# benanil/CLRayTracer

Hardware: AMD Instinct MI355X
Metric: Mrays/s (primary + traced secondary rays), ms/frame at 1920x1080 (higher is better)
Workload: dtype f32

## Files before the change

### clraytracer_amd/_lib.py

```python
import ctypes as C
import os

import numpy as np

os.environ.setdefault("GPU_MAX_HW_QUEUES", "8")

_HERE = os.path.dirname(os.path.abspath(__file__))
ROOT = os.path.dirname(_HERE)
HIP_SO = os.path.join(_HERE, "csrc", "libcrt_hip.so")
HOST_SO = os.path.join(_HERE, "host", "libcrt_host.so")


class CrtTraceArgs(C.Structure):
    _fields_ = [("cameraPos", C.c_float * 3), ("time", C.c_float), ("numMeshes", C.c_uint32), ("sunAngle", C.c_float)]


class CrtFrameStats(C.Structure):
    _fields_ = [("frames", C.c_uint64), ("sumMs", C.c_double * 4), ("extentMs", C.c_double), ("firstFrameMs", C.c_double)]


class CrtCounters(C.Structure):
    _fields_ = [(n, C.c_uint64) for n in ("rays", "primary", "secondary", "hits", "misses", "traversals", "pops",
                                          "innerVisits", "triTests", "capHits", "stackOverflows", "maxStack",
                                          "shadowRays", "shadowHits")]

    def as_dict(self):
        return {n: int(getattr(self, n)) for n, _ in self._fields_}


TRI_DTYPE = np.dtype([("v0", "<f4", 3), ("cx", "<f4"), ("v1", "<f4", 3), ("cy", "<f4"), ("v2", "<f4", 3), ("cz", "<f4"),
                      ("uv", "<u2", 6), ("mat", "<u2"), ("n", "<u2", 9)])
NODE_DTYPE = np.dtype([("min", "<f4", 3), ("leftFirst", "<u4"), ("max", "<f4", 3), ("triCount", "<u4")])
MATERIAL_DTYPE = np.dtype([("color", "<u4"), ("specularColor", "<u4"), ("albedo", "<u2"), ("specular", "<u2"),
                           ("shininess", "<u2"), ("roughness", "<u2")])
TEXTURE_DTYPE = np.dtype([("width", "<i4"), ("height", "<i4"), ("offset", "<i4"), ("padd", "<i4")])
INSTANCE_DTYPE = np.dtype([("inv", "<f4", (4, 4)), ("meshIndex", "<u2"), ("materialStart", "<u2"), ("pad", "u1", 12)])
RAYHIT_DTYPE = np.dtype([("t", "<f4"), ("u", "<f4"), ("v", "<f4"), ("tri", "<u4"), ("instance", "<i4")])
HITRECORD_DTYPE = np.dtype([("normal", "<f4", 3), ("uv", "<f4", 2), ("distance", "<f4"), ("color", "<u4"), ("index", "<u4")])
assert TRI_DTYPE.itemsize == 80 and NODE_DTYPE.itemsize == 32 and MATERIAL_DTYPE.itemsize == 16
assert TEXTURE_DTYPE.itemsize == 16 and INSTANCE_DTYPE.itemsize == 80 and RAYHIT_DTYPE.itemsize == 20
assert HITRECORD_DTYPE.itemsize == 32
CRT_RENDER_GBUFFER = 8192
CRT_GBUFFER_GEOMETRY, CRT_GBUFFER_IDS, CRT_GBUFFER_ALBEDO = 0, 1, 2
GBUFFER_GEOMETRY_DTYPE = np.dtype([("normal", "<f4", 3), ("t", "<f4")])
GBUFFER_IDS_DTYPE = np.dtype([("instance", "<i4"), ("tri", "<u4"), ("u", "<f4"), ("v", "<f4")])
GBUFFER_ALBEDO_DTYPE = np.dtype("<u4")
GBUFFER_PLANE_DTYPES = {"geometry": (CRT_GBUFFER_GEOMETRY, GBUFFER_GEOMETRY_DTYPE), "ids": (CRT_GBUFFER_IDS, GBUFFER_IDS_DTYPE),
                        "albedo": (CRT_GBUFFER_ALBEDO, GBUFFER_ALBEDO_DTYPE)}
GBUFFER_PIXEL_DTYPE = np.dtype([("normal", "<f4", 3), ("t", "<f4"), ("instance", "<i4"), ("tri", "<u4"), ("u", "<f4"), ("v", "<f4"),
                                ("albedo", "<u4")])
assert GBUFFER_GEOMETRY_DTYPE.itemsize == 16 and GBUFFER_IDS_DTYPE.itemsize == 16 and GBUFFER_PIXEL_DTYPE.itemsize == 36

_f = C.c_float
_fp = C.POINTER(C.c_float)
_vp = C.c_void_p
_sz = C.c_size_t

HIP_API = {
    "crt_init": (C.c_int, [C.c_int, C.c_int, C.c_int]),
    "crt_init_devices": (C.c_int, [C.POINTER(C.c_int), C.c_int, C.c_int, C.c_int]),
    "crt_init_gpus": (C.c_int, [C.c_int, C.c_int, C.c_int]),
    "crt_num_devices": (C.c_int, []),
    "crt_peer_access": (C.c_int, [C.c_int]),
    "crt_gather_path": (C.c_char_p, []),
    "crt_get_cull_range": (C.c_int, [_fp, C.c_int, _fp, _fp, C.POINTER(C.c_uint64)]),
    "crt_debug_staggered_frames": (C.c_int, [C.POINTER(C.c_uint64)]),
    "crt_debug_inject_failure": (C.c_int, [C.c_int]),
    "crt_debug_last_kernel": (C.c_int, [C.c_char_p, C.c_size_t]),
    "crt_debug_last_gather": (C.c_int, [C.POINTER(C.c_uint64), C.POINTER(C.c_int)]),
    "crt_debug_build_stats": (C.c_int, [C.POINTER(C.c_uint32), C.POINTER(C.c_uint32)]),
    "crt_debug_tlas_stats": (C.c_int, [C.POINTER(C.c_uint64), C.POINTER(C.c_uint32), C.POINTER(C.c_uint32)]),
    "crt_debug_measure_clock": (C.c_int, [C.c_int, C.POINTER(C.c_double)]),
    "crt_shutdown": (C.c_int, []),
    "crt_resize": (C.c_int, [C.c_int, C.c_int]),
    "crt_set_row_bands": (C.c_int, [C.c_int, C.c_int, C.c_int]),
    "crt_row_owner": (C.c_int, [C.c_int, C.c_int, C.c_int]),
    "crt_band_plan": (C.c_int, [C.c_int, C.c_int, C.c_int, C.c_int, C.POINTER(C.c_int)]),
    "crt_upload_triangles": (C.c_int, [_vp, _sz, _sz]),
    "crt_upload_bvh_nodes": (C.c_int, [_vp, _sz, _sz]),
    "crt_upload_bvh_roots": (C.c_int, [_vp, _sz, _sz]),
    "crt_upload_materials": (C.c_int, [_vp, _sz, _sz]),
    "crt_upload_texture_table": (C.c_int, [_vp, _sz]),
    "crt_upload_texels": (C.c_int, [_vp, _sz, _sz]),
    "crt_upload_instances": (C.c_int, [_vp, _sz, _sz]),
    "crt_build_bvh": (C.c_int, [_sz, _vp, C.c_int, _sz, _sz, C.POINTER(C.c_uint32)]),
    "crt_download_triangles": (C.c_int, [_vp, _sz, _sz]),
    "crt_download_bvh_nodes": (C.c_int, [_vp, _sz, _sz]),
    "crt_download_bvh_roots": (C.c_int, [_vp, _sz, _sz]),
    "crt_render": (C.c_int, [C.POINTER(CrtTraceArgs), _fp, _fp, C.c_int]),
    "crt_sync": (C.c_int, []),
    "crt_query_hits": (C.c_int, [_vp, _vp, C.c_int, C.c_uint32, _vp]),
    "crt_read_output": (C.c_int, [_vp, _sz]),
    "crt_read_output_rows": (C.c_int, [_vp, C.c_int, C.c_int]),
    "crt_read_output_rgba8": (C.c_int, [_vp, _sz]),
    "crt_map_host_frame": (C.c_int, [C.POINTER(C.c_void_p), C.POINTER(C.c_size_t)]),
    "crt_map_host_frame_back": (C.c_int, [C.c_int, C.POINTER(C.c_void_p), C.POINTER(C.c_size_t)]),
    "crt_read_rays": (C.c_int, [_vp, _sz]),
    "crt_output_device_ptr": (_vp, []),
    "crt_read_gbuffer": (C.c_int, [C.c_int, _vp, _sz]),
    "crt_gbuffer_device_ptr": (_vp, [C.c_int]),
    "crt_pick_pixel": (C.c_int, [C.c_int, C.c_int, _vp]),
    "crt_owned_rows": (C.c_int, []),
    "crt_last_kernel_ms": (C.c_float, [C.c_int]),
    "crt_frame_time_stats": (C.c_int, [C.POINTER(CrtFrameStats), C.c_int]),
    "crt_get_counters": (C.c_int, [C.POINTER(CrtCounters)]),
    "crt_get_culled_visits": (C.c_int, [C.POINTER(C.c_uint64)]),
    "crt_debug_read_stamps": (C.c_int, [_vp, _sz, C.POINTER(C.c_size_t)]),
    "crt_debug_read_frame_times": (C.c_int, [_vp, _sz, C.POINTER(C.c_size_t)]),
    "crt_error_string": (C.c_char_p, [C.c_int]),
    "crt_device_name": (C.c_char_p, []),
}

HOST_API = {
    "crth_initialize": (C.c_int, [C.c_int, C.c_int, C.c_int]),
    "crth_initialize_devices": (C.c_int, [C.POINTER(C.c_int), C.c_int, C.c_int, C.c_int]),
    "crth_initialize_host_only": (C.c_int, [C.c_int, C.c_int]),
    "crth_terminate": (None, []),
    "crth_last_error": (C.c_int, []),
    "crth_clear_error": (None, []),
    "crth_prepare_meshes": (None, []),
    "crth_import_texture": (C.c_int, [C.c_char_p]),
    "crth_import_texture_rgb8": (C.c_int, [C.c_char_p, C.c_int, C.c_int, _vp]),
    "crth_import_mesh": (C.c_int, [C.c_char_p]),
    "crth_push_meshes": (None, []),
    "crth_set_device_bvh_build": (None, [C.c_int]),
    "crth_set_mesh_cache": (None, [C.c_int]),
    "crth_qlz_decompress": (C.c_size_t, [_vp, _sz, _vp, _sz]),
    "crth_qlz_store": (C.c_size_t, [_vp, _sz, _vp]),
    "crth_qlz_compress": (C.c_size_t, [_vp, _sz, _vp]),
    "crth_jpeg_decode": (C.c_size_t, [_vp, _sz, _vp, _sz, C.POINTER(C.c_int), C.POINTER(C.c_char_p)]),
    "crth_set_asset_root": (None, [C.c_char_p]),
    "crth_push_textures": (None, []),
    "crth_push_materials": (None, []),
    "crth_create_material": (C.c_int, [C.c_int]),
    "crth_edit_material": (None, [C.c_int, _vp]),
    "crth_begin_instances": (None, []),
    "crth_register_instance": (C.c_uint, [C.c_int, C.c_int, _fp]),
    "crth_end_instances": (None, []),
    "crth_clear_instances": (None, []),
    "crth_set_mesh_matrix": (None, [C.c_uint, _fp]),
    "crth_set_mesh_position": (None, [C.c_uint, _fp]),
    "crth_set_instance_material": (None, [C.c_uint, C.c_int]),
    "crth_set_camera": (None, [_fp, _fp]),
    "crth_get_camera": (None, [_fp, _fp, _fp]),
    "crth_resize": (None, [C.c_int, C.c_int]),
    "crth_set_postprocess": (None, [C.c_int]),
    "crth_set_shadows": (None, [C.c_int]),
    "crth_set_refraction": (None, [C.c_int]),
    "crth_set_fxaa": (None, [C.c_int]),
    "crth_set_supersampling": (None, [C.c_int]),
    "crth_set_gbuffer": (None, [C.c_int]),
    "crth_map_gbuffer": (_vp, [C.c_int]),
    "crth_pick_pixel": (C.c_int, [C.c_int, C.c_int, _vp]),
    "crth_set_unorm8": (None, [C.c_int]),
    "crth_map_output_rgba8": (_vp, []),
    "crth_set_pipelined": (None, [C.c_int]),
    "crth_set_row_bands": (None, [C.c_int, C.c_int, C.c_int]),
    "crth_render": (C.c_uint, [_f]),
    "crth_map_output": (_vp, []),
    "crth_last_frame_ms": (C.c_float, []),
    "crth_cpu_raycast": (None, [_vp, _vp, C.c_int, _vp, C.c_int]),
    "crth_cpu_raycast_sse": (None, [_vp, _vp, C.c_int, _vp, C.c_int]),
    "crth_triangles": (_vp, []), "crth_num_triangles": (_sz, []),
    "crth_nodes": (_vp, []), "crth_num_nodes": (_sz, []),
    "crth_roots": (_vp, []), "crth_num_meshes": (C.c_int, []),
    "crth_materials": (_vp, []), "crth_num_materials": (C.c_int, []),
    "crth_textures": (_vp, []), "crth_num_textures": (C.c_int, []),
    "crth_texels": (_vp, []), "crth_texel_bytes": (_sz, []),
    "crth_instances": (_vp, []), "crth_num_instances": (C.c_uint, []),
    "crth_mesh_info": (None, [C.c_int, _vp]),
    "crth_build_bvh": (C.c_uint32, [_vp, _vp, C.c_int, _vp, _vp]),
    "crth_float_to_half": (C.c_uint16, [_f]),
    "crth_half_to_float": (_f, [C.c_uint16]),
    "crth_inverse_transform": (None, [_fp, _fp]),
    "crth_inverse": (None, [_fp, _fp]),
    "crth_perspective_fov_rh": (None, [_f, _f, _f, _f, _f, _fp]),
    "crth_look_at_rh": (None, [_fp, _fp, _fp, _fp]),
    "crth_write_obj": (C.c_int, [C.c_char_p, _vp, C.c_int, _vp, C.c_int, _vp, C.c_int, _vp, _vp, C.c_int, _vp, C.c_int]),
    "crth_shm_barrier_open": (_vp, [C.c_char_p, C.c_int, C.c_int]),
    "crth_shm_barrier_wait": (C.c_int, [_vp, C.c_int]),
    "crth_shm_barrier_close": (None, [_vp]),
}


def _bind(path, table):
    if not os.path.exists(path):
        raise ImportError(f"{path} has not been built (run `make` at {ROOT} or __graft_entry__.build()); "
                          "the ray-trace path has no fallback without it")
    lib = C.CDLL(path, mode=C.RTLD_GLOBAL)
    for name, (res, args) in table.items():
        fn = getattr(lib, name)
        fn.restype = res
        fn.argtypes = args
    return lib


_hip = None
_host = None


def hip():
    global _hip
    if _hip is None:
        _hip = _bind(HIP_SO, HIP_API)
    return _hip


def host():
    global _host
    if _host is None:
        hip()
        _host = _bind(HOST_SO, HOST_API)
    return _host


CRT_OK, CRT_E_NOT_INITIALIZED, CRT_E_BAD_ARGUMENT, CRT_E_OUT_OF_RANGE, CRT_E_NO_DEVICE, CRT_E_UNSUPPORTED = 0, -1, -2, -3, -4, -5


class CrtError(RuntimeError):
    pass


def check(rc, what="crt call"):
    if rc != 0:
        msg = hip().crt_error_string(rc)
        raise CrtError(f"{what} failed with {rc}: {msg.decode() if msg else '?'}")


def fptr(a):
    a = np.ascontiguousarray(a, dtype=np.float32)
    return a.ctypes.data_as(_fp), a


def as_array(ptr, count, dtype):
    if not ptr or count == 0:
        return np.zeros(0, dtype=dtype)
    nbytes = int(count) * np.dtype(dtype).itemsize
    buf = (C.c_char * nbytes).from_address(ptr)
    return np.frombuffer(buf, dtype=dtype, count=int(count)).copy()
```

### clraytracer_amd/csrc/crt_device.h

```cpp
#pragma once
#include <hip/hip_runtime.h>
#include <hip/hip_fp16.h>
#include <stdint.h>
#include <type_traits>
#include "../../include/crt_types.h"

#define CRT_LEAF_BIT 0x80000000u
#define CRT_TOP_BIT 0x40000000u
#define CRT_BLOCK 64
#ifndef CRT_WAVES_PER_SIMD
#define CRT_WAVES_PER_SIMD 8
#endif
#define CRT_WAVES_PER_SIMD_COUNT 6
typedef uint32_t __attribute__((address_space(3))) * crt_lds_u32_ptr;
typedef float crt_f32x4 __attribute__((ext_vector_type(4)));
typedef const crt_f32x4 __attribute__((address_space(4)))* crt_const_f32x4_ptr;
typedef const crt_f32x4 __attribute__((address_space(3)))* crt_lds_f32x4_ptr;
#ifndef CRT_LDS_SLOTS
#define CRT_LDS_SLOTS 20
#endif
#define CRT_MAX_PARK 5
#define CRT_OVF_SLOTS_MAX (CRT_STACK_DEPTH - (CRT_LDS_SLOTS - CRT_MAX_PARK))
#define CRT_OVF_WORDS_PER_BLOCK ((size_t)CRT_OVF_SLOTS_MAX * CRT_BLOCK)
template <int PARK, int SLOTS = CRT_LDS_SLOTS, bool TOP = false>
struct CrtStackT {
    static constexpr bool kTop = TOP;
    static constexpr int kLds = SLOTS - PARK;
    static_assert(PARK >= 0 && PARK <= CRT_MAX_PARK && kLds >= 1 && kLds <= CRT_STACK_DEPTH && CRT_STACK_DEPTH - kLds <= CRT_OVF_SLOTS_MAX, "LDS slots");
    crt_lds_u32_ptr lds;
    uint32_t* ovf;
    crt_lds_f32x4_ptr top;
    uint32_t vblock;
    __device__ __forceinline__ uint32_t* overflow_slot(int k) const
    {
        uint32_t lane = threadIdx.x & 63;
        asm volatile("" : "+v"(lane));
        return ovf + ((size_t)(TOP ? vblock : blockIdx.x) * CRT_OVF_SLOTS_MAX + (size_t)k) * CRT_BLOCK + lane;
    }
    __device__ __forceinline__ void write(int slot, uint32_t v) const
    {
        const int s = slot & (CRT_STACK_DEPTH - 1);
        if (kLds >= CRT_STACK_DEPTH || __ballot(s >= kLds) == 0) { lds[s * 64] = v; return; }
        if (kLds >= CRT_STACK_DEPTH || s < kLds) lds[s * 64] = v;
        else *overflow_slot(s - kLds) = v;
    }
    __device__ __forceinline__ uint32_t read(int slot) const
    {
        const int s = slot & (CRT_STACK_DEPTH - 1);
        if (kLds >= CRT_STACK_DEPTH || __ballot(s >= kLds) == 0) return lds[s * 64];
        if (kLds >= CRT_STACK_DEPTH || s < kLds) return lds[s * 64];
        return *overflow_slot(s - kLds);
    }
    __device__ __forceinline__ crt_lds_f32x4_ptr top_record(uint32_t k) const { return top + k * 4; }
    __device__ __forceinline__ void park(int k, uint32_t v) const { lds[(kLds + k) * 64] = v; }
    __device__ __forceinline__ uint32_t parked(int k) const { return lds[(kLds + k) * 64]; }
};
typedef CrtStackT<0> CrtStack;
#ifndef CRT_SPLIT_BETA
#define CRT_SPLIT_BETA 1.2f
#endif
#ifndef CRT_SPLIT_BETA_ASYNC
#define CRT_SPLIT_BETA_ASYNC 2.0f
#endif
#define CRT_MAX_SPLIT 96
#ifndef CRT_MAX_SPLIT_PIPELINED
#define CRT_MAX_SPLIT_PIPELINED 8
#endif
#define CRT_TILE 8

struct CrtTlasNode { float4 sphere; uint32_t left, right, pad0, pad1; };
#define CRT_TLAS_LEAF 0x80000000u
#define CRT_TLAS_MIN_INSTANCES 64
#define CRT_TLAS_LIST 8

struct CrtDevScene {
    const float4* __restrict__ pairs;
    const float* __restrict__ triHot;
    const uint4* __restrict__ triCold;
    const uint32_t* __restrict__ bigLeaf;
    const uint32_t* __restrict__ rootRefs;
    uint32_t* stackOverflow;
    const CrtMeshInstance* __restrict__ instances;
    const struct CrtDevInstance* __restrict__ devInstances;
    const float4* __restrict__ instBounds;
    const CrtMaterial* __restrict__ materials;
    const CrtTexture* __restrict__ textures;
    const uint32_t* __restrict__ texels;
    int numTexels;
    uint32_t numInstances;
    const CrtTlasNode* __restrict__ tlas;
    uint32_t tlasNodes;
    const uint32_t* __restrict__ alwaysList;
    uint32_t numAlways;
    const float4* __restrict__ topPairs;
};

struct CrtFrame {
    float invView[16];
    float invProj[16];
    float camPos[3];
    float lightY, lightZ;
    int width, height;
    int tilesX;
    int ownedTileRows;
    int gridBlocks;
    int tileRowsPerBand;
    int rank, nRanks;
    int slotsPerXcd;
    const uint32_t* order;
    const uint32_t* listLen;
    int listCap;
    uint32_t* cost;
    uint32_t epilogue;
    int ss;
    uint32_t* packOut;
};

struct CrtGBuffer {
    char* __restrict__ planes;
    __host__ __device__ char* geometry() const { return planes; }
    __host__ __device__ char* ids(size_t pixels) const { return planes + 16 * pixels; }
    __host__ __device__ char* albedo(size_t pixels) const { return planes + 32 * pixels; }
};

struct v3 { float x, y, z; };

__device__ __forceinline__ v3 mk3(float x, float y, float z) { v3 r; r.x = x; r.y = y; r.z = z; return r; }
__device__ __forceinline__ v3 add3(v3 a, v3 b) { return mk3(a.x + b.x, a.y + b.y, a.z + b.z); }
__device__ __forceinline__ v3 sub3(v3 a, v3 b) { return mk3(a.x - b.x, a.y - b.y, a.z - b.z); }
__device__ __forceinline__ v3 mul3(v3 a, v3 b) { return mk3(a.x * b.x, a.y * b.y, a.z * b.z); }
__device__ __forceinline__ v3 scale3(v3 a, float s) { return mk3(a.x * s, a.y * s, a.z * s); }
__device__ __forceinline__ v3 neg3(v3 a) { return mk3(-a.x, -a.y, -a.z); }
__device__ __forceinline__ float dot3(v3 a, v3 b) { return (a.x * b.x + a.y * b.y) + a.z * b.z; }
__device__ __forceinline__ v3 cross3(v3 a, v3 b)
{
    return mk3(a.y * b.z - a.z * b.y, a.z * b.x - a.x * b.z, a.x * b.y - a.y * b.x);
}
__device__ __forceinline__ v3 normalize3(v3 v)
{
    float inv = 1.0f / sqrtf(dot3(v, v));
    return scale3(v, inv);
}
__device__ __forceinline__ v3 reflect3(v3 v, v3 n)
{
    float d = dot3(n, v);
    return sub3(v, scale3(scale3(n, d), 2.0f));
}
__device__ __forceinline__ int f2i(float x)
{
    if (!(x == x)) return 0;
    if (x >= 2147483648.0f) return 2147483647;
    if (x <= -2147483648.0f) return (-2147483647 - 1);
    return (int)x;
}
__device__ __forceinline__ float h2f(uint32_t bits16) { return __half2float(__ushort_as_half((unsigned short)bits16)); }

struct CrtDevInstance;
struct Triout { float t, u, v; uint32_t tri; };

struct LaneCounters {
    uint32_t rays, primary, secondary, hits, misses;
    uint32_t traversals, pops, innerVisits, triTests, capHits, stackOverflows, maxStack;
    uint32_t shadowRays, shadowHits;
    uint32_t culled;
};
__device__ __forceinline__ void count_culled(LaneCounters& lc, uint32_t n) { lc.traversals += n; lc.pops += n; lc.innerVisits += n; lc.culled += n; }

__device__ __forceinline__ float intersect_aabb(v3 o, v3 inv, float4 bmin, float4 bmax, float minSoFar)
{
// ... 61 lines not shown
__device__ __forceinline__ v3 xform_xyz(const CrtDevInstance& m, float vx, float vy, float vz, float vw)
{
    v3 r;
    r.x = ((m.r0.x * vx + m.r1.x * vy) + m.r2.x * vz) + m.r3.x * vw;
    r.y = ((m.r0.y * vx + m.r1.y * vy) + m.r2.y * vz) + m.r3.y * vw;
    r.z = ((m.r0.z * vx + m.r1.z * vy) + m.r2.z * vz) + m.r3.z * vw;
    return r;
}

__device__ __forceinline__ v3 mat3mul(const CrtDevInstance& m, v3 v)
{
    v3 r;
    r.x = (m.r0.x * v.x + m.r1.x * v.y) + m.r2.x * v.z;
    r.y = (m.r0.y * v.x + m.r1.y * v.y) + m.r2.y * v.z;
    r.z = (m.r0.z * v.x + m.r1.z * v.y) + m.r2.z * v.z;
    return r;
}

__device__ __forceinline__ CrtDevInstance load_instance(const CrtDevInstance* __restrict__ table, uint32_t inst)
{
    CrtDevInstance I;
    const uint32_t inst0 = (uint32_t)__builtin_amdgcn_readfirstlane((int)inst);
    if (__ballot(inst != inst0) == 0) {
        const crt_const_f32x4_ptr p = (crt_const_f32x4_ptr)(table + inst0);
        const crt_f32x4 a = p[0], b = p[1], c = p[2], e = p[3];
        I.r0 = make_float4(a.x, a.y, a.z, a.w); I.r1 = make_float4(b.x, b.y, b.z, b.w);
        I.r2 = make_float4(c.x, c.y, c.z, c.w); I.r3 = make_float4(e.x, e.y, e.z, e.w);
    } else {
        const CrtDevInstance* ip = table + inst;
        I.r0 = ip->r0; I.r1 = ip->r1; I.r2 = ip->r2; I.r3 = ip->r3;
    }
    return I;
}

template <bool COUNT>
struct Traversal {
    v3 mo, md, inv;
    Triout tr;
    int sp, prot, inters;
    uint32_t ref, curInst;
    bool active;

    __device__ __forceinline__ void reset()
    {
        mo = mk3(0.f, 0.f, 0.f); md = mo; inv = mo;
        tr.t = 0.f; tr.u = 0.f; tr.v = 0.f; tr.tri = 0;
        sp = 0; prot = 0; inters = 0; ref = 0; curInst = 0; active = false;
    }
    __device__ __forceinline__ bool at_inner() const { return active && !(ref & CRT_LEAF_BIT); }
    __device__ __forceinline__ bool at_leaf() const { return active && (ref & CRT_LEAF_BIT); }

    __device__ __forceinline__ void finish(Closest& c)
    {
        if (inters) { c.hitInstance = (int)curInst; c.hit = tr; c.distance = tr.t; c.anyHit = 1; }
        active = false;
    }
    template <class STK>
    __device__ __forceinline__ void pop_next(const STK& stack, Closest& c, LaneCounters& lc)
    {
        const bool nonEmpty = sp > 0, canPop = nonEmpty && prot < CRT_MAX_POPS;
        prot += nonEmpty ? 1 : 0;
        if (COUNT) { if (nonEmpty && !canPop) lc.capHits++; if (canPop) lc.pops++; }
        if (canPop) { --sp; ref = stack.read(sp); }
        else {
            const bool keep = inters != 0;
            c.hitInstance = keep ? (int)curInst : c.hitInstance; c.distance = keep ? tr.t : c.distance; c.anyHit = keep ? 1 : c.anyHit;
            c.hit.t = keep ? tr.t : c.hit.t; c.hit.u = keep ? tr.u : c.hit.u; c.hit.v = keep ? tr.v : c.hit.v; c.hit.tri = keep ? tr.tri : c.hit.tri;
            active = false;
        }
    }
    template <bool TOP = false>
    __device__ __forceinline__ void enter(const CrtDevScene& S, uint32_t inst, v3 o, v3 d, float bestSoFar, LaneCounters& lc)
    {
        curInst = inst;
        const CrtDevInstance I = load_instance(S.devInstances, inst);
        mo = xform_xyz(I, o.x, o.y, o.z, 1.0f);
        md = xform_xyz(I, d.x, d.y, d.z, 0.0f);
        inv = mk3(1.0f / md.x, 1.0f / md.y, 1.0f / md.z);
        tr.t = bestSoFar; tr.tri = 0; tr.u = 0.0f; tr.v = 0.0f;
        ref = __float_as_uint(TOP ? I.r2.w : I.r0.w);
        sp = 0; prot = 1; inters = 0; active = true;
        if (COUNT) { lc.traversals++; lc.pops++; }
    }
    template <class STK>
    __device__ __forceinline__ void inner(const CrtDevScene& S, const STK& stack, Closest& c, LaneCounters& lc)
    {
        float dist1, dist2;
        uint32_t nearRef, farRef;
        const uint32_t ref0 = (uint32_t)__builtin_amdgcn_readfirstlane((int)ref);
        if (__ballot(ref != ref0) == 0) {
            const crt_const_f32x4_ptr q = (STK::kTop && (ref0 & CRT_TOP_BIT)) ? (crt_const_f32x4_ptr)(S.topPairs + (size_t)(ref0 & 0xFFFFu) * 4)
                                                                             : (crt_const_f32x4_ptr)(S.pairs + (size_t)ref0 * 4);
            const crt_f32x4 a = q[0], b = q[1], c4 = q[2], e = q[3];
            dist1 = intersect_aabb(mo, inv, make_float4(a.x, a.y, a.z, a.w), make_float4(b.x, b.y, b.z, b.w), tr.t);
            dist2 = intersect_aabb(mo, inv, make_float4(c4.x, c4.y, c4.z, c4.w), make_float4(e.x, e.y, e.z, e.w), tr.t);
            nearRef = __float_as_uint(a.w); farRef = __float_as_uint(c4.w);
#ifndef CRT_TOP_NO_LDS_PATH
#define CRT_TOP_NO_LDS_PATH 0
#endif
        } else if (STK::kTop && !CRT_TOP_NO_LDS_PATH && __ballot(!(ref & CRT_TOP_BIT)) == 0) {
            const auto q = stack.top_record(ref & 0xFFFFu);
            const crt_f32x4 a = q[0], b = q[1], c4 = q[2], e = q[3];
            dist1 = intersect_aabb(mo, inv, make_float4(a.x, a.y, a.z, a.w), make_float4(b.x, b.y, b.z, b.w), tr.t);
            dist2 = intersect_aabb(mo, inv, make_float4(c4.x, c4.y, c4.z, c4.w), make_float4(e.x, e.y, e.z, e.w), tr.t);
            nearRef = __float_as_uint(a.w); farRef = __float_as_uint(c4.w);
        } else {
            const float4* p = (STK::kTop && (ref & CRT_TOP_BIT)) ? S.topPairs + (size_t)(ref & 0xFFFFu) * 4 : S.pairs + (size_t)ref * 4;
            const float4 lmin = p[0], lmax = p[1], rmin = p[2], rmax = p[3];
            dist1 = intersect_aabb(mo, inv, lmin, lmax, tr.t);
            dist2 = intersect_aabb(mo, inv, rmin, rmax, tr.t);
            nearRef = __float_as_uint(lmin.w); farRef = __float_as_uint(rmin.w);
        }
        if (COUNT) lc.innerVisits++;
        {
            const bool sw = dist1 > dist2;
            const float d1 = sw ? dist2 : dist1, d2 = sw ? dist1 : dist2;
            const uint32_t r1 = sw ? farRef : nearRef, r2 = sw ? nearRef : farRef;
            dist1 = d1; dist2 = d2; nearRef = r1; farRef = r2;
        }
        if (dist2 != 1e30f) {
            if (COUNT) { if (sp >= CRT_STACK_DEPTH) lc.stackOverflows++; }
            stack.write(sp, farRef);
            sp++;
            if (COUNT) { if ((uint32_t)sp > lc.maxStack) lc.maxStack = (uint32_t)sp; }
        }
        if (dist1 == 1e30f) pop_next(stack, c, lc);
        else ref = nearRef;
    }
    template <bool ANYHIT, class STK>
    __device__ __forceinline__ void leaf(const CrtDevScene& S, const STK& stack, Closest& c, LaneCounters& lc)
    {
        const uint32_t first = ref & 0x00FFFFFFu;
        uint32_t n = (ref >> 24) & 0x7Fu;
        if (n == 0) n = S.bigLeaf[first];
        for (uint32_t i = first, end = first + n; i < end; ++i) {
            if (COUNT) lc.triTests++;
            const float* __restrict__ hot = S.triHot + (size_t)i * 9;
            inters |= intersect_triangle(mo, md, mk3(hot[0], hot[1], hot[2]), mk3(hot[3], hot[4], hot[5]), mk3(hot[6], hot[7], hot[8]), tr, i);
            if (ANYHIT) { if (inters) break; }
        }
        if (ANYHIT && inters) finish(c);
        else pop_next(stack, c, lc);
    }
};

__device__ __forceinline__ bool sphere_culls(const float4 bs, v3 o, v3 d, float dd)
{
    const v3 oc = mk3(bs.x - o.x, bs.y - o.y, bs.z - o.z);
    const float oc2 = dot3(oc, oc), b = dot3(oc, d);
    const float r2 = bs.w * bs.w * 1.0201f + 4e-6f * oc2;
    return (bs.w >= 0.0f) & ((oc2 * dd - b * b > r2 * dd) | ((b < 0.0f) & (oc2 > r2)));
}

template <bool COUNT, bool DEFER_COUNT = false>
__device__ __forceinline__ unsigned long long candidate_mask(const CrtDevScene& S, v3 o, v3 d, uint32_t base, uint32_t cnt, LaneCounters& lc)
{
    const float dd = dot3(d, d);
    unsigned long long cand = 0;
    const crt_const_f32x4_ptr bounds = (crt_const_f32x4_ptr)S.instBounds;
    for (uint32_t k = 0; k < cnt; ++k) {
        const crt_f32x4 bs = bounds[base + k];
        const v3 oc = mk3(bs.x - o.x, bs.y - o.y, bs.z - o.z);
        const float oc2 = dot3(oc, oc), b = dot3(oc, d);
        const float r2 = bs.w * bs.w * 1.0201f + 4e-6f * oc2;
        const bool cull = (bs.w >= 0.0f) && ((oc2 * dd - b * b > r2 * dd) || (b < 0.0f && oc2 > r2));
        if (!cull) cand |= 1ull << k;
    }
    if (COUNT && !DEFER_COUNT) { const uint32_t culled = cnt - (uint32_t)__popcll(cand); count_culled(lc, culled); }
    return cand;
}

#define CRT_TLAS_PARK (CRT_TLAS_LIST / 2)
template <class STK>
__device__ __forceinline__ bool candidate_list_add(const STK& stack, uint32_t& n, uint32_t idx)
{
    if (n >= (uint32_t)CRT_TLAS_LIST) return false;
    const uint32_t sh = (n & 1u) * 16u, m = ~(0xFFFFu << sh), v = idx << sh;
    const int k = (int)(n >> 1);
    stack.park(k, (stack.parked(k) & m) | v);
    n++;
    return true;
}
template <class STK>
__device__ __forceinline__ uint32_t candidate_list_next(const STK& stack, int after)
{
    uint32_t best = 0xFFFFu;
#pragma unroll
    for (int k = 0; k < CRT_TLAS_PARK; ++k) {
        const uint32_t w = stack.parked(k);
        const uint32_t lo = w & 0xFFFFu, hi = w >> 16;
        if ((int)lo > after && lo < best) best = lo;
        if ((int)hi > after && hi < best) best = hi;
    }
    return best;
}
template <class STK>
__device__ __forceinline__ bool tlas_candidates(const CrtDevScene& S, v3 o, v3 d, const STK& stack, uint32_t& n)
{
#pragma unroll
    for (int k = 0; k < CRT_TLAS_PARK; ++k) stack.park(k, 0xFFFFFFFFu);
    n = 0;
    bool ok = true;
    for (uint32_t k = 0; k < S.numAlways; ++k) { const uint32_t i = S.alwaysList[k]; if (i < S.numInstances) ok = candidate_list_add(stack, n, i) && ok; }
    if (S.tlasNodes == 0) return ok;
    const float dd = dot3(d, d);
    uint32_t node = 0; int sp = 0;
    for (;;) {
        const CrtTlasNode nd = S.tlas[node];
        bool descend = false;
        if (!sphere_culls(nd.sphere, o, d, dd)) {
            if (nd.left & CRT_TLAS_LEAF) {
                const uint32_t i = nd.left & 0xFFFFu;
                if (i < S.numInstances) ok = candidate_list_add(stack, n, i) && ok;
            } else { stack.write(sp, nd.right); sp++; node = nd.left; descend = true; }
        }
        if (!descend) { if (sp == 0) break; --sp; node = stack.read(sp); }
    }
    return ok;
}

template <bool COUNT, bool ITERS, bool ANYHIT, class STK>
__device__ __forceinline__ void trip_steps(const CrtDevScene& S, const STK& stack, Traversal<COUNT>& T, Closest& c, LaneCounters& lc, bool done)
{
    if (!done && T.at_inner()) {
        if (ITERS) { lc.rays++; if (first_active_lane()) lc.innerVisits++; }
        T.inner(S, stack, c, lc);
    }
    if (!done && T.at_leaf()) {
        if (ITERS) {
            if (first_active_lane()) lc.triTests++;
            uint32_t n = (T.ref >> 24) & 0x7Fu; if (n == 0) n = S.bigLeaf[T.ref & 0x00FFFFFFu];
            for (int off = 32; off > 0; off >>= 1) { const uint32_t o2 = (uint32_t)__shfl_xor((int)n, off, 64); n = o2 > n ? o2 : n; }
            if (first_active_lane()) lc.misses += n;
        }
        T.template leaf<ANYHIT>(S, stack, c, lc);
    }
    if (!done && T.at_inner()) {
        if (ITERS) { if (first_active_lane()) lc.hits++; }
        T.inner(S, stack, c, lc);
    }
}

template <bool COUNT, bool ITERS = false, bool ANYHIT = false, bool TLAS = false, class STK = CrtStack>
__device__ __forceinline__ Closest closest_hit(const CrtDevScene& S, v3 o, v3 d, const STK& stack, LaneCounters& lc)
{
    Closest c = no_hit();
    Traversal<COUNT> T; T.reset();

    if constexpr (TLAS) {
        static_assert(!TLAS || STK::kLds <= CRT_LDS_SLOTS - CRT_TLAS_PARK, "the candidate list needs CRT_TLAS_PARK parked slots");
        uint32_t listed = 0;
        const bool fits = tlas_candidates(S, o, d, stack, listed);
        if (__ballot(!fits) == 0) {
            int prev = -1;
            if (COUNT && !ANYHIT) { const uint32_t culled = S.numInstances - listed; count_culled(lc, culled); }
            bool done = false;
            for (;;) {
                const bool wEnter = !done && !T.active;
                const bool wInner = !done && T.at_inner();
                const bool wLeaf = !done && T.at_leaf();
                if (__ballot(wEnter || wInner || wLeaf) == 0) break;
                if (wEnter) {
                    const uint32_t k = (ANYHIT && c.anyHit) ? 0xFFFFu : candidate_list_next(stack, prev);
                    if (k == 0xFFFFu) {
                        done = true;
                        if (COUNT && ANYHIT && !c.anyHit) { const uint32_t n = S.numInstances - (uint32_t)(prev + 1); count_culled(lc, n); }
                    } else {
                        if (COUNT && ANYHIT) { const uint32_t n = k - (uint32_t)(prev + 1); count_culled(lc, n); }
                        prev = (int)k;
                        T.template enter<STK::kTop>(S, k, o, d, c.distance, lc);
                    }
                }
                trip_steps<COUNT, false, ANYHIT>(S, stack, T, c, lc, done);
            }
            return c;
        }
    }

    for (uint32_t base = 0; base < S.numInstances; base += 64) {
        const uint32_t cnt = (S.numInstances - base) < 64u ? (S.numInstances - base) : 64u;
        unsigned long long cand = candidate_mask<COUNT, ANYHIT>(S, o, d, base, cnt, lc);
        unsigned long long culledLeft = (COUNT && ANYHIT) ? (~cand & (cnt == 64u ? ~0ull : ((1ull << cnt) - 1ull))) : 0ull;
        bool done = ANYHIT && c.anyHit;
        for (;;) {
            const bool wEnter = !done && !T.active;
            const bool wInner = !done && T.at_inner();
            const bool wLeaf = !done && T.at_leaf();
            if (__ballot(wEnter || wInner || wLeaf) == 0) break;
            if (ITERS) { if (first_active_lane()) lc.pops++; }
            if (wEnter) {
                if (ANYHIT && c.anyHit) done = true;
                else if (cand == 0) {
                    done = true;
                    if (COUNT && ANYHIT) { const uint32_t n = (uint32_t)__popcll(culledLeft); count_culled(lc, n); culledLeft = 0; }
                } else {
                    if (ITERS) { if (first_active_lane()) lc.traversals++; }
                    const uint32_t k = (uint32_t)__ffsll((long long)cand) - 1u;
                    cand &= cand - 1;
                    if (COUNT && ANYHIT) {
                        const unsigned long long below = culledLeft & ((1ull << k) - 1ull);
                        const uint32_t n = (uint32_t)__popcll(below);
                        count_culled(lc, n); culledLeft &= ~below;
                    }
                    T.template enter<STK::kTop>(S, base + k, o, d, c.distance, lc);
                }
            }
            trip_steps<COUNT, ITERS, ANYHIT>(S, stack, T, c, lc, done);
        }
    }
    return c;
}

__device__ __forceinline__ int clamp_texel(int idx, int n) { return idx < 0 ? 0 : (idx >= n ? n - 1 : idx); }

__device__ __noinline__ int sample_skybox(v3 d, int texW, int texH)
{
    const double PI = 3.14159265358979323846;
    float at = (float)(atan2((double)d.x, (double)(-d.z)) / PI);
    float ac = (float)(acos((double)d.y) / PI);
    int theta = f2i((at * 0.5f) * (float)texW);
    int phi = f2i(ac * (float)texH);
    return (int)((uint32_t)phi * (uint32_t)texW + (uint32_t)(theta + 2));
}

__device__ __forceinline__ int sample_texture(const CrtTexture& tex, float u, float v)
{
    u = u - floorf(u);
    v = v - floorf(v);
    int uS = f2i((float)tex.width * u);
    int vS = f2i((float)tex.height * v);
    return (int)((uint32_t)vS * (uint32_t)tex.width + (uint32_t)tex.offset + (uint32_t)uS);
}

__device__ __forceinline__ v3 raygen_dir(const CrtFrame& F, int i, int j, int width, int height)
{
    float cx = (float)i / (float)width, cy = (float)j / (float)height;
    cx = cx * 2.0f - 1.0f;
    cy = cy * 2.0f - 1.0f;
    v3 t = matmul_xyz(F.invProj, cx, cy, 1.0f, 1.0f);
    float w = matmul_w(F.invProj, cx, cy, 1.0f, 1.0f);
    float tx = t.x / w, ty = t.y / w, tz = t.z / w, tw = w / w;
    v3 wv = matmul_xyz(F.invView, tx, ty, tz, tw);
    return normalize3(wv);
}

__device__ __forceinline__ v3 raygen_dir(const CrtFrame& F, int i, int j) { return raygen_dir(F, i, j, F.width, F.height); }

struct PathState { v3 o, d, result; float energy; };
__device__ __forceinline__ PathState camera_path(const CrtFrame& F, v3 d)
{
    PathState ps;
    ps.o = mk3(F.camPos[0], F.camPos[1], F.camPos[2]);
    ps.d = d;
    ps.result = mk3(0.0f, 0.0f, 0.0f);
    ps.energy = 1.0f;
    return ps;
}

__device__ __forceinline__ float specular_x(float ndl, float shadow)
{
    const float sp = ((1.0f - 0.5f) * ndl) * shadow;
    return (sp * 0.2f) * ndl;
}

struct NoSink { };
template <bool DEFER_ENERGY = false, bool REFRACT = false, class SINK = NoSink>
__device__ __forceinline__ int shade_bounce(const CrtDevScene& S, const Closest& c, PathState& ps, int bounce, float lightY, float lightZ,
                                            float* ndlOut = nullptr, const SINK* sink = nullptr)
{
    constexpr bool kSink = !std::is_same<SINK, NoSink>::value;
    const float UcharToFloat01 = 1.0f / 255.0f;
    if (c.distance > 99998.0f) {
        if constexpr (kSink) { if (bounce == 0) sink->miss(c); }
        const crt_f32x4 skyHdr = ((crt_const_f32x4_ptr)S.textures)[2];
        int idx = clamp_texel(sample_skybox(ps.d, __float_as_int(skyHdr.x), __float_as_int(skyHdr.y)), S.numTexels);
        uint32_t px = S.texels[idx];
        v3 skyc = scale3(mk3((float)(px & 0xffu), (float)((px >> 8) & 0xffu), (float)((px >> 16) & 0xffu)), UcharToFloat01);
        ps.result = add3(ps.result, scale3(skyc, ps.energy));
        return 0;
    }
    const v3 light = bounce == 0 ? mk3(0.0f, lightY, lightZ) : ps.d;
    const v3 atm0 = scale3(mk3(0.255f, 0.25f, 0.27f), 1.0f);
    const v3 atm = bounce == 0 ? atm0 : scale3(atm0, 0.4f);
    const CrtDevInstance I = load_instance(S.devInstances, (uint32_t)c.hitInstance);
    const v3 mo = xform_xyz(I, ps.o.x, ps.o.y, ps.o.z, 1.0f);
    const v3 md = xform_xyz(I, ps.d.x, ps.d.y, ps.d.z, 0.0f);

    const uint4 c0 = S.triCold[(size_t)c.hit.tri * 2], c1 = S.triCold[(size_t)c.hit.tri * 2 + 1];
    const uint32_t matIndex = c0.w & 0xffffu;
    uint32_t mi = __float_as_uint(I.r1.w) + matIndex;
    mi = mi < (uint32_t)CRT_MAX_MATERIALS ? mi : (uint32_t)CRT_MAX_MATERIALS - 1;
    const CrtMaterial mat = S.materials[mi];
    const float bx = (1.0f - c.hit.u) - c.hit.v, by = c.hit.u, bz = c.hit.v;

    const v3 n0 = mat3mul(I, mk3(h2f(c0.w >> 16), h2f(c1.x & 0xffffu), h2f(c1.x >> 16)));
    const v3 n1 = mat3mul(I, mk3(h2f(c1.y & 0xffffu), h2f(c1.y >> 16), h2f(c1.z & 0xffffu)));
    const v3 n2 = mat3mul(I, mk3(h2f(c1.z >> 16), h2f(c1.w & 0xffffu), h2f(c1.w >> 16)));
    const v3 normal = normalize3(add3(add3(scale3(n0, bx), scale3(n1, by)), scale3(n2, bz)));

    const float uvx = (h2f(c0.x & 0xffffu) * bx + h2f(c0.y & 0xffffu) * by) + h2f(c0.z & 0xffffu) * bz;
    const float uvy = (h2f(c0.x >> 16) * bx + h2f(c0.y >> 16) * by) + h2f(c0.z >> 16) * bz;

    uint32_t ti = mat.albedoTextureIndex;
    ti = ti < (uint32_t)CRT_MAX_TEXTURES ? ti : (uint32_t)CRT_MAX_TEXTURES - 1;
    const CrtTexture tex = S.textures[ti];
    const uint32_t px = S.texels[clamp_texel(sample_texture(tex, uvx, uvy), S.numTexels)];
    const uint32_t a = mat.color;
    const uint32_t cr = (((a & 0xffu) * (px & 0xffu)) >> 8) & 0xffu;
    const uint32_t cg = ((((a >> 8) & 0xffu) * ((px >> 8) & 0xffu)) >> 8) & 0xffu;
    const uint32_t cb = ((((a >> 16) & 0xffu) * ((px >> 16) & 0xffu)) >> 8) & 0xffu;
    const v3 color = scale3(mk3((float)cr, (float)cg, (float)cb), UcharToFloat01);
    if constexpr (kSink) { if (bounce == 0) sink->hit(c, normal, 0xFF000000u | (cb << 16) | (cg << 8) | cr); }
    const v3 point = add3(mo, scale3(md, c.hit.t));


    bool transmitted = false;
    float opacity = 1.0f;
    if (REFRACT) {
        if (bounce == 0) {
            opacity = h2f(mat.roughness);
            if (opacity < 1.0f) {
                const float dn = dot3(normal, ps.d);
                const bool entering = dn < 0.0f;
                const v3 nf = entering ? normal : neg3(normal);
                const float cosi = entering ? (0.0f - dn) : dn;
                const float eta = entering ? 0.6666667f : 1.5f;
                const float k = 1.0f - (eta * eta) * (1.0f - cosi * cosi);
                if (k >= 0.0f) {
                    const float w = eta * cosi - sqrtf(k);
                    const v3 refr = add3(scale3(ps.d, eta), scale3(nf, w));
                    ps.o = sub3(point, scale3(nf, 0.01f));
                    ps.d = refr;
                    transmitted = true;
                }
            }
        }
    }
    if (!transmitted) {
        ps.o = add3(point, scale3(normal, 0.01f));
        ps.d = reflect3(ps.d, normal);
    }

    float ndl = dot3(normal, neg3(light));
    const v3 ambient = mul3(scale3(atm, fmaxf(0.0f - ndl, 0.1f)), color);
    ndl = fmaxf(ndl, 0.0f);
    const float sl = (ndl * fmaxf(dot3(reflect3(neg3(light), normal), md), 0.0f)) * 0.2f;

    ps.result = add3(ps.result, add3(add3(scale3(scale3(color, ndl), ps.energy), ambient), mk3(sl, sl, sl)));
    if (REFRACT && transmitted) { ps.energy = ps.energy * (1.0f - opacity); return 2; }
    if (DEFER_ENERGY) *ndlOut = ndl;
    else ps.energy = ps.energy * specular_x(ndl, 1.0f);
    return 1;
}
```

### clraytracer_amd/csrc/crt_frame.h

```cpp
#pragma once
namespace {

static void unpack_counters(const unsigned long long c[CRT_NUM_COUNTERS])
{
    CrtCounters& o = g.lastCounters;
    o.rays = c[0]; o.primary = c[1]; o.secondary = c[2]; o.hits = c[3]; o.misses = c[4]; o.traversals = c[5];
    o.pops = c[6]; o.innerVisits = c[7]; o.triTests = c[8]; o.capHits = c[9]; o.stackOverflows = c[10]; o.maxStack = c[11];
    o.shadowRays = c[12]; o.shadowHits = c[13]; g.lastCulled = c[14];
}

int collect_set(EventSet& es)
{
    if (!es.pending) return CRT_OK;
    hipEvent_t* ev = es.ev;
    hipEvent_t traceStart = es.evRaygen ? ev[1] : ev[0], frameEnd = es.evPost ? ev[3] : ev[2];
    HIPCHK(hipEventSynchronize(frameEnd));
    float ms[4] = { 0, 0, 0, 0 };
    HIPCHK(hipEventElapsedTime(&ms[0], ev[0], frameEnd));
    if (es.evRaygen) HIPCHK(hipEventElapsedTime(&ms[1], ev[0], ev[1]));
    HIPCHK(hipEventElapsedTime(&ms[2], traceStart, ev[2]));
    if (es.evPost) HIPCHK(hipEventElapsedTime(&ms[3], ev[2], ev[3]));
    for (int k = 0; k < 4; ++k) g.msSum[k] += (double)ms[k];
    g.framesTimed++;
    if (g.statStartValid && es.seq >= g.statStartSeq) {
// ... 352 lines not shown

static int launch_passes(FrameCtx& c)
{
    FrameSlot& fs = *c.fs; EventSet& es = *c.es; CrtFrame& F = c.F;
    const bool unorm = (c.flags & CRT_RENDER_UNORM8) != 0, post = (c.flags & CRT_RENDER_POSTPROCESS) != 0, fxaa = (c.flags & CRT_RENDER_FXAA) != 0;
    const bool fxaaLocal = fxaa && g.groupSize <= 1;
    const size_t framePixels = (size_t)g.width * (size_t)g.height;
    if (fxaa && !is_secondary()) RCCHK(grow(fs.aux, fs.auxPixels, framePixels, fs.stream));
    if (c.flags & CRT_RENDER_GBUFFER) RCCHK(grow(fs.gbuf, fs.gbufBytes, framePixels * CRT_GBUFFER_PIXEL_BYTES, fs.stream));
    if (!fxaa) F.epilogue = (unorm ? CRT_EPILOGUE_QUANTIZE : 0u) | (post ? CRT_EPILOGUE_POST : 0u);
    else if (fxaaLocal) F.epilogue = unorm ? CRT_EPILOGUE_QUANTIZE : 0u;
    c.gather8 = frame_gathers_rgba8(c.flags);
    c.packInKernel = unorm && (((c.flags & CRT_RENDER_READBACK) && g.groupSize <= 1) || c.gather8);
    if (c.packInKernel) RCCHK(grow(fs.packBuf, fs.packCap, framePixels, fs.stream));
    if (c.packInKernel && !fxaa) F.packOut = fs.packBuf;
    c.T.epilogue = F.epilogue; c.T.packOut = F.packOut;
    RCCHK(launch_trace(c, fxaaLocal ? fs.aux : fs.out));
    if (is_primary() && !es.evPost) RCCHK(wait_for_parts(c));
    HIPCHK(hipEventRecord(es.ev[2], fs.stream));
    if (!es.evPost) return CRT_OK;
    if (!fxaa) {
        if (!c.fused) {
            if (unorm) crt_quantize_kernel<<<c.grid, CRT_BLOCK, 0, fs.stream>>>(F, fs.out);
            if (post) crt_postprocess_kernel<<<c.grid, CRT_BLOCK, 0, fs.stream>>>(F, fs.out);
            if (unorm && post) crt_quantize_kernel<<<c.grid, CRT_BLOCK, 0, fs.stream>>>(F, fs.out);
            if (c.gather8) crt_pack_owned_kernel<<<(unsigned)F.gridBlocks, CRT_BLOCK, 0, fs.stream>>>(plain_frame(F, false), fs.out, fs.packBuf);
            HIPCHK(hipGetLastError());
        }
        if (is_primary()) RCCHK(wait_for_parts(c));
    } else if (!is_secondary()) {
        if (is_primary()) RCCHK(wait_for_parts(c));
        CrtFrame FF = plain_frame(F, true);
        const unsigned gridAll = (unsigned)FF.gridBlocks;
        if (fxaaLocal) {
            if (unorm && !c.fused) crt_quantize_kernel<<<gridAll, CRT_BLOCK, 0, fs.stream>>>(FF, fs.aux);
        } else {
            if (unorm) crt_quantize_kernel<<<gridAll, CRT_BLOCK, 0, fs.stream>>>(FF, fs.out);
            HIPCHK(hipMemcpyAsync(fs.aux, fs.out, framePixels * sizeof(float4), hipMemcpyDeviceToDevice, fs.stream));
        }
        FF.epilogue = (unorm ? CRT_EPILOGUE_QUANTIZE : 0u) | (post ? CRT_EPILOGUE_POST : 0u);
        FF.packOut = c.packInKernel ? fs.packBuf : nullptr;
        crt_fxaa_kernel<<<gridAll, CRT_BLOCK, 0, fs.stream>>>(FF, fs.aux, fs.out);
        HIPCHK(hipGetLastError());
    }
    HIPCHK(hipEventRecord(es.ev[3], fs.stream));
    return CRT_OK;
}

static int gather_to_primary(const FrameCtx& c)
{
    FrameSlot& fs = *c.fs; FrameSlot& pfs = g.primary->slot[c.slot];
    HIPCHK(hipStreamWaitEvent(fs.stream, pfs.slotDone, 0));
    if (c.gather8) RCCHK(copy_owned_rows_async(pfs.packBuf, fs.packBuf, 4, hipMemcpyDeviceToDevice, fs.stream));
    else RCCHK(copy_owned_rows_async(pfs.out, fs.out, 16, hipMemcpyDeviceToDevice, fs.stream));
    HIPCHK(hipEventRecord(fs.partDone, fs.stream));
    return CRT_OK;
}

static int finish_frame(const FrameCtx& c)
{
    FrameSlot& fs = *c.fs; EventSet& es = *c.es;
    fs.frameIs8 = c.gather8;
    g.cur = c.slot;
    if (c.flags & CRT_RENDER_GBUFFER) g.gbufSlot = c.slot;
    es.pending = true; es.flags = c.flags; es.seq = ++g.frameSeq; fs.frames++;
    if (c.T.order != nullptr && !(c.flags & CRT_RENDER_DIAG_MIX3)) {
        float view[35];
        memcpy(view, c.F.invView, 64); memcpy(view + 16, c.F.invProj, 64); memcpy(view + 32, c.F.camPos, 12);
        g.viewMoved = memcmp(view, g.lastView, sizeof view) != 0 || g.lastViewInst != g.instVersion;
        memcpy(g.lastView, view, sizeof view); g.lastViewInst = g.instVersion;
        RCCHK(sort_for_next_frame(c.T, fs, c.pipelined, g.form != Form::Mega));
    }
    if (c.flags & CRT_RENDER_READBACK) {
        const size_t pixels = (size_t)g.width * (size_t)g.height;
        const bool bytes8 = (c.flags & CRT_RENDER_UNORM8) != 0;
        const size_t bytes = pixels * (bytes8 ? 4 : 16);
        if (bytes > fs.hostCap) {
            if (fs.hostBuf) (void)hipHostFree(fs.hostBuf);
            fs.hostBuf = nullptr; fs.hostCap = 0;
            HIPCHK(hipHostMalloc(&fs.hostBuf, bytes, hipHostMallocDefault));
            fs.hostCap = bytes;
        }
        if (!fs.copied) HIPCHK(hipEventCreateWithFlags(&fs.copied, hipEventDisableTiming));
        const void* src = fs.out;
        if (bytes8) {
            RCCHK(grow(fs.packBuf, fs.packCap, pixels, fs.stream));
            const bool packed = (c.packInKernel && ((c.flags & CRT_RENDER_FXAA) || c.fused)) || c.gather8;
            if (!packed) crt_pack_unorm8_kernel<<<(unsigned)((pixels + 255) / 256), 256, 0, fs.stream>>>(fs.out, fs.packBuf, pixels);
            HIPCHK(hipGetLastError());
            src = fs.packBuf;
        }
        RCCHK(copy_owned_rows_async(fs.hostBuf, src, bytes8 ? 4 : 16, hipMemcpyDeviceToHost, fs.stream, is_primary()));
        HIPCHK(hipEventRecord(fs.copied, fs.stream));
        fs.hostBytes = bytes; g.readbackRing[g.readbackCount++ % CRT_MAX_FRAMES_IN_FLIGHT] = c.slot;
    }
    if (is_primary()) HIPCHK(hipEventRecord(fs.slotDone, fs.stream));
    if (!(c.flags & CRT_RENDER_ASYNC) && !(c.plan && c.plan->noHostWait)) HIPCHK(hipEventSynchronize(es.evPost ? es.ev[3] : es.ev[2]));
    return CRT_OK;
}

int crt1_render(const CrtTraceArgs* args, const float invView[16], const float invProj[16], int flags, const RenderPlan* plan = nullptr)
{
    if (!g.initialized) return CRT_E_NOT_INITIALIZED;
    if (!args || !invView || !invProj) return CRT_E_BAD_ARGUMENT;
    if (args->numMeshes > CRT_MAX_INSTANCES) return CRT_E_OUT_OF_RANGE;
    if (!g.sceneValid) return CRT_E_BAD_ARGUMENT;
    if ((flags & CRT_RENDER_SSAA2) && (flags & CRT_RENDER_SSAA4)) return CRT_E_BAD_ARGUMENT;
    FrameCtx c;
    c.flags = flags; c.plan = plan;
    fill_frame(c.F, args, invView, invProj, ssaa_factor(flags));
    if (c.F.gridBlocks == 0) return record_empty_share(plan);
    RCCHK(refuse_unsupported(flags, args->numMeshes));
    RCCHK(choose_slot(c));
    RCCHK(prepare_lists(c));
    RCCHK(begin_frame(c, args));
    RCCHK(launch_passes(c));
    if (is_secondary()) RCCHK(gather_to_primary(c));
    return finish_frame(c);
}

__global__ void crt_clock_probe_kernel(unsigned long long ticks, double* __restrict__ out)
{
    const unsigned long long r0 = __builtin_amdgcn_s_memrealtime(), c0 = __builtin_amdgcn_s_memtime();
    unsigned long long r1 = r0, guard = 0;
    while (r1 - r0 < ticks && guard < (1ull << 24)) { __builtin_amdgcn_s_sleep(8); r1 = __builtin_amdgcn_s_memrealtime(); ++guard; }
    const unsigned long long c1 = __builtin_amdgcn_s_memtime();
    r1 = __builtin_amdgcn_s_memrealtime();
    if (threadIdx.x == 0) out[blockIdx.x] = r1 > r0 ? (double)(c1 - c0) / (double)(r1 - r0) * 0.1 : 0.0;
}

int crt1_debug_measure_clock(int micros, double* ghz)
{
    if (!g.initialized) return CRT_E_NOT_INITIALIZED;
    if (!ghz || micros < 1 || micros > 100000) return CRT_E_BAD_ARGUMENT;
    double* d = nullptr; hipStream_t st = nullptr;
    HIPCHK(hipMalloc(&d, 8 * sizeof(double)));
    hipError_t e = hipStreamCreateWithFlags(&st, hipStreamNonBlocking);
    double h[8] = { 0 };
    if (e == hipSuccess) {
        crt_clock_probe_kernel<<<8, 64, 0, st>>>((unsigned long long)micros * 100ull, d);
        e = hipGetLastError();
        if (e == hipSuccess) e = hipMemcpyAsync(h, d, sizeof h, hipMemcpyDeviceToHost, st);
        if (e == hipSuccess) e = hipStreamSynchronize(st);
    }
    if (st) (void)hipStreamDestroy(st);
    (void)hipFree(d);
    if (e != hipSuccess) return (int)e;
    double sum = 0; int n = 0;
    for (double v : h) if (v > 0.0) { sum += v; ++n; }
    *ghz = n ? sum / n : 0.0;
    return CRT_OK;
}

int crt1_sync(void)
{
    if (!g.initialized) return CRT_E_NOT_INITIALIZED;
    return sync_all();
}

int crt1_query_hits(const float* origins, const float* dirs, int n, uint32_t numInstances, CrtRayHit* out)
{
    if (!g.initialized) return CRT_E_NOT_INITIALIZED;
    if (n <= 0) return CRT_OK;
    if (!origins || !dirs || !out || numInstances > CRT_MAX_INSTANCES) return CRT_E_BAD_ARGUMENT;
    if (!g.sceneValid) return CRT_E_BAD_ARGUMENT;
    RCCHK(collect_timing());
    RCCHK(quiesce());
    const size_t rayBytes = sizeof(float) * 3 * (size_t)n, need = rayBytes * 2 + sizeof(CrtRayHit) * (size_t)n;
    RCCHK(grow(g.queryBuf, g.queryBytes, need, g.stream));
    float* dO = reinterpret_cast<float*>(g.queryBuf);
    float* dD = dO + 3 * (size_t)n;
    CrtRayHit* dH = reinterpret_cast<CrtRayHit*>(dD + 3 * (size_t)n);
    HIPCHK(hipMemcpyAsync(dO, origins, rayBytes, hipMemcpyHostToDevice, g.stream));
    HIPCHK(hipMemcpyAsync(dD, dirs, rayBytes, hipMemcpyHostToDevice, g.stream));
    HIPCHK(hipMemsetAsync(g.counters, 0, CRT_NUM_COUNTERS * sizeof(unsigned long long), g.stream));
    FrameSlot& fs = g.slot[0];
    RCCHK(ensure_slot_instances(fs));
    RCCHK(ensure_overflow(fs, (size_t)((n + CRT_BLOCK - 1) / CRT_BLOCK)));
    double farthest2 = 0.0;
    for (int k = 0; k < n; ++k) {
        const double x = origins[3 * k], y = origins[3 * k + 1], z = origins[3 * k + 2], d2 = x * x + y * y + z * z;
        if (!(d2 <= farthest2)) farthest2 = d2;
    }
    CrtDevScene S; fill_scene(S, numInstances, fs, beyond_cull_range(sqrt(farthest2)));
    with_bools([&](auto Tl) { crt_query_kernel<decltype(Tl)::value><<<(unsigned)((n + CRT_BLOCK - 1) / CRT_BLOCK), CRT_BLOCK, 0, g.stream>>>(S, dO, dD, n, dH, g.counters); }, use_tlas(S));
    HIPCHK(hipGetLastError());
    HIPCHK(hipMemcpyAsync(out, dH, sizeof(CrtRayHit) * (size_t)n, hipMemcpyDeviceToHost, g.stream));
    unsigned long long c[CRT_NUM_COUNTERS];
    HIPCHK(hipMemcpyAsync(c, g.counters, sizeof c, hipMemcpyDeviceToHost, g.stream));
    HIPCHK(hipStreamSynchronize(g.stream));
    unpack_counters(c);
    return CRT_OK;
}

int crt1_read_output(float* dst, size_t floats)
{
    if (!g.initialized) return CRT_E_NOT_INITIALIZED;
    if (!dst || floats != (size_t)g.width * (size_t)g.height * 4) return CRT_E_BAD_ARGUMENT;
    RCCHK(sync_all());
    RCCHK(expand_rgba8_frame(g.slot[g.cur]));
    HIPCHK(hipMemcpy(dst, g.slot[g.cur].out, floats * sizeof(float), hipMemcpyDeviceToHost));
    return CRT_OK;
}

int crt1_read_output_rows(float* dst, int row0, int rows)
{
    if (!g.initialized) return CRT_E_NOT_INITIALIZED;
    if (!dst || row0 < 0 || rows < 0 || row0 + rows > g.height) return CRT_E_BAD_ARGUMENT;
    RCCHK(sync_all());
    RCCHK(expand_rgba8_frame(g.slot[g.cur]));
    HIPCHK(hipMemcpy(dst, g.slot[g.cur].out + (size_t)row0 * (size_t)g.width, (size_t)rows * (size_t)g.width * sizeof(float4), hipMemcpyDeviceToHost));
    return CRT_OK;
}

int crt1_read_output_rgba8(uint8_t* dst, size_t bytes)
{
    if (!g.initialized) return CRT_E_NOT_INITIALIZED;
    const size_t pixels = (size_t)g.width * (size_t)g.height;
    if (!dst || bytes != pixels * 4) return CRT_E_BAD_ARGUMENT;
    RCCHK(sync_all());
    if (g.slot[g.cur].frameIs8) {
        HIPCHK(hipMemcpy(dst, g.slot[g.cur].packBuf, pixels * 4, hipMemcpyDeviceToHost));
        return CRT_OK;
    }
    RCCHK(grow(g.queryBuf, g.queryBytes, pixels * 4, g.stream));
    crt_pack_unorm8_kernel<<<(unsigned)((pixels + 255) / 256), 256, 0, g.stream>>>(g.slot[g.cur].out, reinterpret_cast<uint32_t*>(g.queryBuf), pixels);
    HIPCHK(hipGetLastError());
    HIPCHK(hipMemcpyAsync(dst, g.queryBuf, pixels * 4, hipMemcpyDeviceToHost, g.stream));
    HIPCHK(hipStreamSynchronize(g.stream));
    return CRT_OK;
}

int crt1_map_host_frame_back(int framesBack, const void** ptr, size_t* bytes)
{
    if (!g.initialized) return CRT_E_NOT_INITIALIZED;
    if (!ptr || framesBack < 0 || (unsigned)framesBack >= g.readbackCount || framesBack >= g.nSlots) return CRT_E_BAD_ARGUMENT;
    const int slot = g.readbackRing[(g.readbackCount - 1u - (unsigned)framesBack) % CRT_MAX_FRAMES_IN_FLIGHT];
    for (int k = 0; k < framesBack; ++k)
        if (g.readbackRing[(g.readbackCount - 1u - (unsigned)k) % CRT_MAX_FRAMES_IN_FLIGHT] == slot) return CRT_E_BAD_ARGUMENT;
    FrameSlot& fs = g.slot[slot];
    HIPCHK(hipEventSynchronize(fs.copied));
    *ptr = fs.hostBuf;
    if (bytes) *bytes = fs.hostBytes;
    return CRT_OK;
}

int crt1_map_host_frame(const void** ptr, size_t* bytes) { return crt1_map_host_frame_back(0, ptr, bytes); }

int crt1_read_rays(float* dst, size_t floats)
{
    if (!g.initialized) return CRT_E_NOT_INITIALIZED;
    if (!dst || floats != (size_t)g.width * (size_t)g.height * 3) return CRT_E_BAD_ARGUMENT;
    RCCHK(sync_all());
    HIPCHK(hipMemcpy(dst, g.rays, floats * sizeof(float), hipMemcpyDeviceToHost));
    return CRT_OK;
}

static char* gbuffer_plane(int plane)
{
    if (g.gbufSlot < 0 || !g.slot[g.gbufSlot].gbuf || gbuffer_plane_pixel_bytes(plane) == 0) return nullptr;
    const CrtGBuffer gb = slot_gbuffer(g.slot[g.gbufSlot]);
    const size_t pixels = (size_t)g.width * (size_t)g.height;
    return plane == CRT_GBUFFER_GEOMETRY ? gb.geometry() : plane == CRT_GBUFFER_IDS ? gb.ids(pixels) : gb.albedo(pixels);
}

int crt1_read_gbuffer(int plane, void* dst, size_t bytes)
{
    if (!g.initialized) return CRT_E_NOT_INITIALIZED;
    const char* src = gbuffer_plane(plane);
    if (!dst || !src || bytes != (size_t)g.width * (size_t)g.height * gbuffer_plane_pixel_bytes(plane)) return CRT_E_BAD_ARGUMENT;
    RCCHK(sync_all());
    HIPCHK(hipMemcpy(dst, src, bytes, hipMemcpyDeviceToHost));
    return CRT_OK;
}

void* crt1_gbuffer_device_ptr(int plane) { return g.initialized ? (void*)gbuffer_plane(plane) : nullptr; }

int crt1_pick_pixel(int x, int y, CrtGBufferPixel* out)
{
    if (!g.initialized) return CRT_E_NOT_INITIALIZED;
    if (!out || !gbuffer_plane(CRT_GBUFFER_GEOMETRY)) return CRT_E_BAD_ARGUMENT;
    if (x < 0 || y < 0 || x >= g.width || y >= g.height) return CRT_E_OUT_OF_RANGE;
    RCCHK(sync_all());
    const size_t idx = (size_t)y * (size_t)g.width + (size_t)x;
    HIPCHK(hipMemcpy(out->normal, gbuffer_plane(CRT_GBUFFER_GEOMETRY) + idx * 16, 16, hipMemcpyDeviceToHost));
    HIPCHK(hipMemcpy(&out->instance, gbuffer_plane(CRT_GBUFFER_IDS) + idx * 16, 16, hipMemcpyDeviceToHost));
    HIPCHK(hipMemcpy(&out->albedo, gbuffer_plane(CRT_GBUFFER_ALBEDO) + idx * 4, 4, hipMemcpyDeviceToHost));
    return CRT_OK;
}

void* crt1_output_device_ptr(void)
{
    if (!g.initialized) return nullptr;
    if (g.slot[g.cur].frameIs8 && (sync_all() != CRT_OK || expand_rgba8_frame(g.slot[g.cur]) != CRT_OK)) return nullptr;
    return (void*)g.slot[g.cur].out;
}

float crt1_last_kernel_ms(int which)
{
    if (!g.initialized || which < 0 || which > 3) return -1.0f;
    if (collect_timing() != CRT_OK) return -1.0f;
    return g.ms[which];
}

int crt1_frame_time_stats(CrtFrameStats* out, int reset)
{
    if (!g.initialized) return CRT_E_NOT_INITIALIZED;
    RCCHK(collect_timing());
    if (out) {
        out->frames = g.framesTimed;
        for (int k = 0; k < 4; ++k) out->sumMs[k] = g.msSum[k];
        out->extentMs = g.statExtent;
        out->firstFrameMs = g.statFirstMs;
    }
    if (reset) {
        for (int k = 0; k < 4; ++k) g.msSum[k] = 0.0;
        g.framesTimed = 0; g.statExtent = 0; g.statFirstMs = 0; g.statStartArmed = true; g.statStartValid = false;
    }
    return CRT_OK;
}

int crt1_debug_read_frame_times(double* dst, size_t maxFrames, size_t* numFrames)
{
    if (!g.initialized) return CRT_E_NOT_INITIALIZED;
    if (!numFrames) return CRT_E_BAD_ARGUMENT;
    RCCHK(collect_timing());
    *numFrames = g.frameLogN;
    if (dst) memcpy(dst, g.frameLog, sizeof(double) * 2 * (maxFrames < g.frameLogN ? maxFrames : g.frameLogN));
    return CRT_OK;
}

int crt1_debug_read_stamps(uint64_t* dst, size_t maxWaves, size_t* numWaves)
{
    if (!g.initialized) return CRT_E_NOT_INITIALIZED;
    if (!numWaves) return CRT_E_BAD_ARGUMENT;
    *numWaves = g.stampWaves;
    if (!dst || !g.stamps) return CRT_OK;
    const size_t n = maxWaves < g.stampWaves ? maxWaves : g.stampWaves;
    RCCHK(sync_all());
    HIPCHK(hipMemcpy(dst, g.stamps + 16, n * 8 * sizeof(unsigned long long), hipMemcpyDeviceToHost));
    return CRT_OK;
}

int crt1_get_culled_visits(uint64_t* out)
{
    if (!g.initialized) return CRT_E_NOT_INITIALIZED;
    if (!out) return CRT_E_BAD_ARGUMENT;
    RCCHK(collect_timing());
    *out = g.lastCulled;
    return CRT_OK;
}

int crt1_get_cull_range(float* limits, int n, float* sceneLimit, float* bounceReach, uint64_t* noCullFrames)
{
    if (!g.initialized) return CRT_E_NOT_INITIALIZED;
    if (n < 0 || n > CRT_MAX_INSTANCES || (n > 0 && !limits)) return CRT_E_BAD_ARGUMENT;
    for (int i = 0; i < n; ++i) limits[i] = g.hCullOriginLimit[i];
    if (sceneLimit) *sceneLimit = g.cullOriginLimit;
    if (bounceReach) *bounceReach = g.bounceOriginReach;
    if (noCullFrames) *noCullFrames = g.noCullFrames;
    return CRT_OK;
}

int crt1_get_counters(CrtCounters* out)
{
    if (!g.initialized) return CRT_E_NOT_INITIALIZED;
    if (!out) return CRT_E_BAD_ARGUMENT;
    RCCHK(collect_timing());
    *out = g.lastCounters;
    return CRT_OK;
}

}
```

### clraytracer_amd/csrc/crt_instances.h

```cpp
#pragma once
namespace {

bool invert4(const double m[16], double out[16])
{
    double a[4][8];
    for (int r = 0; r < 4; ++r) for (int c = 0; c < 4; ++c) { a[r][c] = m[r * 4 + c]; a[r][4 + c] = (r == c) ? 1.0 : 0.0; }
    for (int col = 0; col < 4; ++col) {
        int piv = col;
        for (int r = col + 1; r < 4; ++r) if (fabs(a[r][col]) > fabs(a[piv][col])) piv = r;
        if (!(fabs(a[piv][col]) > 1e-300)) return false;
        if (piv != col) for (int c = 0; c < 8; ++c) { double t = a[col][c]; a[col][c] = a[piv][c]; a[piv][c] = t; }
        const double inv = 1.0 / a[col][col];
        for (int c = 0; c < 8; ++c) a[col][c] *= inv;
        for (int r = 0; r < 4; ++r) if (r != col) { const double f = a[r][col]; if (f != 0.0) for (int c = 0; c < 8; ++c) a[r][c] -= f * a[col][c]; }
    }
    for (int r = 0; r < 4; ++r) for (int c = 0; c < 4; ++c) out[r * 4 + c] = a[r][4 + c];
    return true;
}

int cache_root_nodes()
{
    for (uint32_t m = 0; m < CRT_MAX_MESHES; ++m) {
        g.hHaveRoot[m] = m < g.numRoots && g.hRoots[m] < g.nodeCount;
        if (g.hHaveRoot[m]) HIPCHK(hipMemcpyAsync(&g.hRootNodes[m], g.rawNodes + g.hRoots[m], sizeof(CrtBVHNode), hipMemcpyDeviceToHost, g.stream));
// ... 79 lines not shown
    for (int a = 0; a < 3; ++a) { lo[a] = c[a] - b.w; hi[a] = c[a] + b.w; }
}

double debug_cull_range_scale()
{
    const char* h = getenv("CRT_DEBUG_HOOKS"); const char* k = getenv("CRT_DEBUG_CULL_RANGE_SCALE");
    return (h && atoi(h) != 0 && k && atof(k) > 0.0) ? atof(k) : 1.0;
}


void update_bounce_reach()
{
    g.hReach = 0.0;
    auto widen = [](double far) { if (far > g.hReach || !(far == far)) g.hReach = far; };
    for (uint32_t m = 0; m < CRT_MAX_MESHES; ++m) {
        if (!g.hHaveRoot[m]) continue;
        widen(box_reach(g.hRootNodes[m]));
        if (g.hHaveKids[m]) { widen(box_reach(g.hRootKids[m][0])); widen(box_reach(g.hRootKids[m][1])); }
    }
    widen(reach_of(g.triReach2));
    g.bounceOriginReach = g.hReach < 3.0e38 ? (float)g.hReach : 3.0e38f;
}

void recompute_cull_records(uint32_t first, uint32_t count)
{
    const uint32_t end = first + count < (uint32_t)CRT_MAX_INSTANCES ? first + count : (uint32_t)CRT_MAX_INSTANCES;
    const double rangeScale = debug_cull_range_scale();
    for (uint32_t i = first; i < end; ++i) {
        g.hBounds[i] = make_float4(0.f, 0.f, 0.f, -1.0f);
        g.hCullOriginLimit[i] = 0.0f;
        if (i >= g.instHigh) continue;
        const CrtMeshInstance& inst = g.hInstances[i];
        if (inst.meshIndex >= CRT_MAX_MESHES || !g.hHaveRoot[inst.meshIndex] || g.hRootNodes[inst.meshIndex].triCount > 0 || !g.hHaveKids[inst.meshIndex]) continue;
        double inv[16], fwd[16], lo[3], hi[3], cw[3];
        if (!forward_transform(inst, inv, fwd)) continue;
        const CrtBVHNode* kid = g.hRootKids[inst.meshIndex];
        for (int a = 0; a < 3; ++a) { lo[a] = fmin((double)kid[0].aabbMin[a], (double)kid[1].aabbMin[a]); hi[a] = fmax((double)kid[0].aabbMax[a], (double)kid[1].aabbMax[a]); }
        const double r = image_sphere(lo, hi, fwd, cw);
        const float4 b = fp32_sphere(cw, r, 1.0 + 1e-4);
        if (!(isfinite(b.x) && isfinite(b.y) && isfinite(b.z) && isfinite(b.w)) || !(b.w < 1e18f) || !(b.w > 1e-18f)) continue;
        const double limit = cull_origin_limit(inv, fwd, b.w) * rangeScale;
        if (!(limit >= g.hReach)) continue;
        g.hCullOriginLimit[i] = (float)fmin(limit * (1.0 - 1e-6), 3e38);
        g.hBounds[i] = b;
    }
}

void recompute_scene_limit()
{
    float lo = (float)fmin(1e30 * (1.0 - 1e-6), 3e38);
    for (uint32_t i = 0; i < g.instHigh; ++i) if (g.hBounds[i].w >= 0.0f && g.hCullOriginLimit[i] < lo) lo = g.hCullOriginLimit[i];
    g.cullOriginLimit = lo;
}

bool tlas_refit()
{
    bool sameSet = g.hTlasBuilt && g.hTlasBuiltHigh == g.instHigh && g.hTlasRefits < 256u;
    for (uint32_t k = 0; sameSet && k < g.instHigh; ++k) sameSet = g.hTlasMember[k] == (uint8_t)(g.hBounds[k].w >= 0.0f);
    if (!sameSet) return false;
    if (g.hTlasNodes == 0) return true;
    double blo[2 * CRT_MAX_INSTANCES][3], bhi[2 * CRT_MAX_INSTANCES][3], sumR = 0.0;
    for (uint32_t n = g.hTlasNodes; n-- > 0;) {
        CrtTlasNode& nd = g.hTlas[n];
        if (nd.left & CRT_TLAS_LEAF) {
            nd.sphere = g.hBounds[nd.left & 0xFFFFu];
            sphere_box(blo[n], bhi[n], nd.sphere);
        } else {
            for (int a = 0; a < 3; ++a) { blo[n][a] = fmin(blo[nd.left][a], blo[nd.right][a]); bhi[n][a] = fmax(bhi[nd.left][a], bhi[nd.right][a]); }
            nd.sphere = node_sphere(blo[n], bhi[n]);
            sumR += (double)nd.sphere.w;
        }
    }
    if (!(sumR <= 1.25 * g.hTlasBuiltRadii)) return false;
    g.hTlasRefits++;
    return true;
}

void tlas_build()
{
    uint32_t nAlways = 0, nLeaves = 0, nNodes = 0, leaves[CRT_MAX_INSTANCES];
    for (uint32_t k = 0; k < g.instHigh; ++k) { const bool cullable = g.hBounds[k].w >= 0.0f; g.hTlasMember[k] = (uint8_t)cullable; if (!cullable) g.hAlways[nAlways++] = k; else leaves[nLeaves++] = k; }
    struct Range { uint32_t lo, hi, node; };
    double sumR = 0.0;
    Range stack[64]; int sp = 0;
    if (nLeaves) stack[sp++] = Range{ 0, nLeaves, nNodes++ };
    while (sp) {
        const Range r = stack[--sp];
        double lo[3] = { 1e300, 1e300, 1e300 }, hi[3] = { -1e300, -1e300, -1e300 }, clo[3] = { 1e300, 1e300, 1e300 }, chi[3] = { -1e300, -1e300, -1e300 };
        for (uint32_t k = r.lo; k < r.hi; ++k) {
            const float4 b = g.hBounds[leaves[k]]; const double c[3] = { b.x, b.y, b.z };
            double slo[3], shi[3];
            sphere_box(slo, shi, b);
            for (int a = 0; a < 3; ++a) {
                if (slo[a] < lo[a]) lo[a] = slo[a];
                if (shi[a] > hi[a]) hi[a] = shi[a];
                if (c[a] < clo[a]) clo[a] = c[a];
                if (c[a] > chi[a]) chi[a] = c[a];
            }
        }
        CrtTlasNode& n = g.hTlas[r.node];
        n.pad0 = n.pad1 = 0;
        if (r.hi - r.lo == 1) { n.sphere = g.hBounds[leaves[r.lo]]; n.left = CRT_TLAS_LEAF | leaves[r.lo]; n.right = 0; continue; }
        n.sphere = node_sphere(lo, hi);
        sumR += (double)n.sphere.w;
        int axis = 0;
        if (chi[1] - clo[1] > chi[axis] - clo[axis]) axis = 1;
        if (chi[2] - clo[2] > chi[axis] - clo[axis]) axis = 2;
        const uint32_t mid = (r.lo + r.hi) / 2;
        auto key = [&](uint32_t idx) { const float4 b = g.hBounds[idx]; return axis == 0 ? b.x : (axis == 1 ? b.y : b.z); };
        std::nth_element(leaves + r.lo, leaves + mid, leaves + r.hi, [&](uint32_t p, uint32_t q) { return key(p) < key(q) || (key(p) == key(q) && p < q); });
        n.left = nNodes++; n.right = nNodes++;
        stack[sp++] = Range{ mid, r.hi, n.right };
        stack[sp++] = Range{ r.lo, mid, n.left };
    }
    g.hTlasNodes = nNodes; g.hNumAlways = nAlways;
    g.hTlasBuilt = true; g.hTlasBuiltHigh = g.instHigh; g.hTlasBuiltRadii = sumR; g.hTlasRefits = 0; g.hTlasBuilds++;
}

void rebuild_instance_master(uint32_t dirtyFirst = 0, uint32_t dirtyCount = CRT_MAX_INSTANCES, bool everything = true)
{
    if (everything) update_bounce_reach();
    recompute_cull_records(everything ? 0u : dirtyFirst, everything ? (uint32_t)CRT_MAX_INSTANCES : dirtyCount);
    recompute_scene_limit();
    if (!tlas_refit()) tlas_build();
    g.instVersion++;
}

int rebuild_bvh_layout()
{
    HIPCHK(hipMemsetAsync(g.err, 0, sizeof(int), g.stream));
    if (g.nodeCount) {
        crt_relayout_nodes<<<(g.nodeCount + 255) / 256, 256, 0, g.stream>>>(g.rawNodes, g.nodeCount, (uint32_t)g.triCap, g.pairs, g.bigLeaf, g.err);
        HIPCHK(hipGetLastError());
    }
    crt_make_root_refs<<<(CRT_MAX_MESHES + 255) / 256, 256, 0, g.stream>>>(g.rawNodes, g.nodeCount, (uint32_t)g.triCap, g.roots, g.numRoots, g.rootRefs, g.bigLeaf, g.err);
    HIPCHK(hipGetLastError());
    {
        const uint32_t perMesh = g.numRoots ? (uint32_t)CRT_TOP_PAIRS / g.numRoots : 0u;
        crt_build_top_kernel<<<1, CRT_MAX_MESHES, 0, g.stream>>>(g.pairs, g.rootRefs, g.numRoots, perMesh, g.topPairs, g.topRootRefs);
        HIPCHK(hipGetLastError());
    }
    int err = 0;
    HIPCHK(hipMemcpyAsync(&err, g.err, sizeof(int), hipMemcpyDeviceToHost, g.stream));
    HIPCHK(hipStreamSynchronize(g.stream));
    g.sceneValid = (err == 0);
    if (err) return CRT_E_BAD_ARGUMENT;
    RCCHK(cache_root_nodes());
    rebuild_instance_master();
    return CRT_OK;
}

constexpr size_t kStageInst = 0;
constexpr size_t kStageBounds = (kStageInst + CRT_MAX_INSTANCES * sizeof(CrtMeshInstance) + 255) & ~(size_t)255;
constexpr size_t kStageAlways = (kStageBounds + CRT_MAX_INSTANCES * sizeof(float4) + 255) & ~(size_t)255;
constexpr size_t kStageTlas = (kStageAlways + CRT_MAX_INSTANCES * sizeof(uint32_t) + 255) & ~(size_t)255;
constexpr size_t kStageBytes = kStageTlas + 2 * CRT_MAX_INSTANCES * sizeof(CrtTlasNode);

int ensure_slot_instances(FrameSlot& fs)
{
    if (fs.instVersion == g.instVersion) return CRT_OK;
    HIPCHK(hipEventSynchronize(fs.staged));
    memcpy(fs.staging + kStageInst, g.hInstances, CRT_MAX_INSTANCES * sizeof(CrtMeshInstance));
    memcpy(fs.staging + kStageBounds, g.hBounds, CRT_MAX_INSTANCES * sizeof(float4));
    if (g.hNumAlways) memcpy(fs.staging + kStageAlways, g.hAlways, g.hNumAlways * sizeof(uint32_t));
    if (g.hTlasNodes) memcpy(fs.staging + kStageTlas, g.hTlas, g.hTlasNodes * sizeof(CrtTlasNode));
    static_assert(kStageInst == 0 && kStageBytes % 16 == 0 && kStageTlas % 16 == 0 && sizeof(CrtTlasNode) % 16 == 0, "copied as 16-byte words");
    const uint32_t words16 = (uint32_t)((kStageTlas + g.hTlasNodes * sizeof(CrtTlasNode)) / 16);
    crt_refresh_instances_kernel<<<16, 256, 0, fs.stream>>>(reinterpret_cast<const uint4*>(fs.stagingDev), reinterpret_cast<uint4*>(fs.instBlock), words16,
                                                             g.rootRefs, g.topRootRefs, CRT_MAX_INSTANCES, fs.devInstances);
    HIPCHK(hipGetLastError());
    HIPCHK(hipEventRecord(fs.staged, fs.stream));
    fs.tlasNodes = g.hTlasNodes; fs.numAlways = g.hNumAlways; fs.instVersion = g.instVersion;
    return CRT_OK;
}

}
```

### clraytracer_amd/csrc/crt_kernels.h

```cpp
#pragma once
#include "crt_device.h"

__device__ __forceinline__ uint32_t wave_sum(uint32_t v)
{
    for (int off = 32; off > 0; off >>= 1) v += __shfl_xor(v, off, 64);
    return v;
}
__device__ __forceinline__ uint32_t wave_max(uint32_t v)
{
    for (int off = 32; off > 0; off >>= 1) { uint32_t o = __shfl_xor(v, off, 64); v = o > v ? o : v; }
    return v;
}

__device__ __forceinline__ void flush_counters(const LaneCounters& lc, unsigned long long* g)
{
    uint32_t s[14] = { lc.rays, lc.primary, lc.secondary, lc.hits, lc.misses, lc.traversals, lc.pops,
                       lc.innerVisits, lc.triTests, lc.capHits, lc.stackOverflows, lc.shadowRays, lc.shadowHits, lc.culled };
    uint32_t mx = wave_max(lc.maxStack);
#pragma unroll
    for (int k = 0; k < 14; ++k) {
        uint32_t t = wave_sum(s[k]);
        if ((threadIdx.x & 63) == 0 && t) atomicAdd(&g[k < 11 ? k : k + 1], (unsigned long long)t);
    }
    if ((threadIdx.x & 63) == 0) atomicMax(&g[11], (unsigned long long)mx);
// ... 113 lines not shown
    __syncthreads();
    const uint32_t nSplit = s_nSplit;
    for (int i = tid; i < slotsPerXcd; i += 1024) {
        int bin = 1023 - (int)((float)c[i] * scale);
        bin = bin < 0 ? 0 : (bin > 1023 ? 1023 : bin);
        const uint32_t pos = atomicAdd(&s_bins[bin], 1u);
        if (pos < nSplit) { for (uint32_t q = 0; q < 4; ++q) o[4 * pos + q] = (uint32_t)i | (q << 28) | 0x80000000u; }
        else o[3 * nSplit + pos] = (uint32_t)i;
    }
    __syncthreads();
    for (int i = tid; i < slotsPerXcd; i += 1024) cost[(size_t)x * slotsPerXcd + i] = 0;
}

__global__ void crt_identity_order_kernel(uint32_t* __restrict__ order, uint32_t* __restrict__ listLen, int slotsPerXcd, int listCap)
{
    const int i = blockIdx.x * blockDim.x + threadIdx.x;
    if (i < 8) listLen[i] = (uint32_t)slotsPerXcd;
    if (i < 8 * slotsPerXcd) order[(i / slotsPerXcd) * listCap + (i % slotsPerXcd)] = (uint32_t)(i % slotsPerXcd);
}

__device__ __forceinline__ v3 post_pixel(v3 rgb, int px, int py, int width, int height)
{
    const float uvx = (float)px / (float)width, uvy = (float)py / (float)height;
    const float P = sqrtf((rgb.x * rgb.x) * 0.299f + ((rgb.y * rgb.y) * 0.587f) + ((rgb.z * rgb.z) * 0.114f));
    const v3 Pv = mk3(P, P, P);
    rgb = add3(Pv, scale3(sub3(rgb, Pv), 1.2f));
    const v3 lw = mk3(0.2126f, 0.7152f, 0.0722f);
    const float max_white_l = 0.8f;
    const float l_old = dot3(rgb, lw);
    const float numerator = l_old * (1.0f + (l_old / (max_white_l * max_white_l)));
    const float l_new = numerator / (1.0f + l_old);
    const float l_in = dot3(rgb, lw);
    rgb = scale3(rgb, l_new / l_in);
    const float ig = 1.0f / 1.55f;
    rgb = mk3(powf(rgb.x, ig), powf(rgb.y, ig), powf(rgb.z, ig));
    const float oneDivGamma = 1.0f / 1.2f;
    rgb = mk3(powf(rgb.x, oneDivGamma), powf(rgb.y, oneDivGamma), powf(rgb.z, oneDivGamma));
    const float vx = uvx * (1.0f - uvy), vy = uvy * (1.0f - uvx);
    float vig = (vx * vy) * 15.0f;
    vig = powf(vig, 0.15f);
    return scale3(rgb, vig);
}
__device__ __forceinline__ uint32_t unorm8(float x)
{
    const float v = x * 255.0f;
    if (!(v == v) || v <= 0.0f) return 0u;
    if (v >= 255.0f) return 255u;
    return (uint32_t)rintf(v);
}
__device__ __forceinline__ float quantize1(float x) { return (float)unorm8(x) / 255.0f; }
#define CRT_EPILOGUE_QUANTIZE 1
#define CRT_EPILOGUE_POST 2

__device__ __forceinline__ v3 quantize3(v3 c) { return mk3(quantize1(c.x), quantize1(c.y), quantize1(c.z)); }
__device__ __forceinline__ uint32_t pack_rgba8(float4 p) { return unorm8(p.x) | (unorm8(p.y) << 8) | (unorm8(p.z) << 16) | (unorm8(p.w) << 24); }
__device__ __forceinline__ uint32_t pack_rgba8(v3 c) { return unorm8(c.x) | (unorm8(c.y) << 8) | (unorm8(c.z) << 16) | 0xFF000000u; }

__device__ __forceinline__ void finish_pixel(const CrtFrame& F, v3 rgb, int x, int y, int width, int height, float4* __restrict__ out, bool always = true)
{
    if (F.epilogue & CRT_EPILOGUE_QUANTIZE) rgb = quantize3(rgb);
    if (F.epilogue & CRT_EPILOGUE_POST) {
        rgb = post_pixel(rgb, x, y, width, height);
        if (F.epilogue & CRT_EPILOGUE_QUANTIZE) rgb = quantize3(rgb);
    }
    const size_t idx = (size_t)y * (size_t)width + (size_t)x;
    if (always || F.epilogue != 0) out[idx] = make_float4(rgb.x, rgb.y, rgb.z, 1.0f);
    if (F.packOut) F.packOut[idx] = pack_rgba8(rgb);
}
__device__ __forceinline__ void finish_block_pixels(const CrtFrame& F, int tx0, int tileRow, uint32_t pixels, float4* __restrict__ out)
{
    if (F.epilogue == 0 && F.packOut == nullptr) return;
    __builtin_amdgcn_fence(__ATOMIC_RELEASE, "workgroup");
    __builtin_amdgcn_fence(__ATOMIC_ACQUIRE, "workgroup");
    for (uint32_t p = threadIdx.x & 63u; p < pixels; p += 64u) {
        int qx, qy;
        tile_pixel(tx0 + (int)(p >> 6), tileRow, (int)(p & 63u), qx, qy);
        if (qx >= F.width || qy >= F.height) continue;
        const float4 v = out[(size_t)qy * (size_t)F.width + (size_t)qx];
        finish_pixel(F, mk3(v.x, v.y, v.z), qx, qy, F.width, F.height, out, false);
    }
}

__device__ __forceinline__ unsigned long long tile_cost_start(const CrtFrame& F) { return F.cost ? __builtin_amdgcn_s_memtime() : 0ull; }
__device__ __forceinline__ void add_tile_cost(const CrtFrame& F, int costSlot, unsigned long long tc0, bool halve = false)
{
    if (F.cost && costSlot >= 0) {
        unsigned long long dt = __builtin_amdgcn_s_memtime() - tc0;
        if (halve) dt >>= 1;
        if ((threadIdx.x & 63) == 0) atomicAdd(&F.cost[costSlot], dt > 0x0FFFFFFFull ? 0x0FFFFFFFu : (uint32_t)dt);
    }
}

struct WaveStampStart { unsigned long long rt, c; };
__device__ __forceinline__ WaveStampStart wave_stamp_start() { return { __builtin_amdgcn_s_memrealtime(), __builtin_amdgcn_s_memtime() }; }
__device__ __forceinline__ void write_wave_stamp(unsigned long long* __restrict__ counters, const LaneCounters& lc, WaveStampStart t0, uint32_t wService = 0)
{
    const unsigned long long t1c = __builtin_amdgcn_s_memtime(), t1rt = __builtin_amdgcn_s_memrealtime();
    const uint32_t wOuter = wave_sum(lc.pops), wEnter = wave_sum(lc.traversals), wDescent = wave_sum(lc.innerVisits),
                   wLeaf = wave_sum(lc.triTests), laneVisits = wave_sum(lc.rays), wInner2 = wave_sum(lc.hits), wLeafIters = wave_sum(lc.misses);
    if ((threadIdx.x & 63) == 0) {
        unsigned long long* st = counters + 16 + (size_t)blockIdx.x * 8;
        st[4] = wOuter | ((unsigned long long)wInner2 << 32); st[5] = wEnter | ((unsigned long long)wLeafIters << 32);
        st[6] = wDescent | ((unsigned long long)wService << 32); st[7] = ((unsigned long long)wLeaf << 32) | laneVisits;
        st[0] = t0.rt; st[1] = t1rt; st[2] = t1c - t0.c;
        st[3] = (unsigned long long)__builtin_amdgcn_s_getreg((31 << 11) | 20) | ((unsigned long long)__builtin_amdgcn_s_getreg((31 << 11) | 4) << 32);
    }
}

template <int M> __device__ __forceinline__ float xor_add(float v) { return v + __int_as_float(__builtin_amdgcn_ds_swizzle(__float_as_int(v), 0x1F | (M << 10))); }
template <int M> __device__ __forceinline__ v3 xor_add3(v3 v) { return mk3(xor_add<M>(v.x), xor_add<M>(v.y), xor_add<M>(v.z)); }

__device__ __forceinline__ void lane_pixel_again(const CrtFrame& F, int b, int lane, int& qx, int& qy)
{
    asm volatile("" : "+s"(b), "+v"(lane));
    (void)lane_pixel(F, qx, qy, nullptr, nullptr, b, lane);
}

struct GBufferSink {
    const CrtGBuffer* gb; const CrtFrame* F; int b, lane;
    __device__ __forceinline__ uint32_t pixel_offset() const
    {
        int gx, gy;
        lane_pixel_again(*F, b, lane, gx, gy);
        return ((uint32_t)gy * (uint32_t)F->width + (uint32_t)gx) << 2;
    }
    template <class T> static __device__ __forceinline__ void store(char* plane, uint32_t byteOffset, T v) { *reinterpret_cast<T*>(plane + byteOffset) = v; }
    __device__ __forceinline__ size_t pixels() const { return (size_t)((uint32_t)F->width * (uint32_t)F->height); }
    __device__ __forceinline__ void hit(const Closest& c, v3 normal, uint32_t albedo) const
    {
        const uint32_t off = pixel_offset();
        store(gb->geometry(), off << 2, make_float4(normal.x, normal.y, normal.z, c.hit.t));
        store(gb->ids(pixels()), off << 2, make_uint4((uint32_t)c.hitInstance, c.hit.tri, __float_as_uint(c.hit.u), __float_as_uint(c.hit.v)));
        store(gb->albedo(pixels()), off, albedo);
    }
    __device__ __forceinline__ void miss(const Closest& c) const
    {
        const uint32_t off = pixel_offset();
        const bool anyHit = c.distance < no_hit().distance;
        store(gb->geometry(), off << 2, make_float4(0.0f, 0.0f, 0.0f, c.distance));
        store(gb->ids(pixels()), off << 2, anyHit ? make_uint4((uint32_t)c.hitInstance, c.hit.tri, __float_as_uint(c.hit.u), __float_as_uint(c.hit.v)) : make_uint4(0xFFFFFFFFu, 0u, 0u, 0u));
        store(gb->albedo(pixels()), off, 0u);
    }
};
#define CRT_TRACE_PLAIN 0
#define CRT_TRACE_SSAA 1
#define CRT_TRACE_GBUFFER 2
template <bool SHADOW, bool TLAS> using CrtTraceStack = CrtStackT<(TLAS ? CRT_TLAS_PARK : 0) + (SHADOW ? 1 : 0)>;
template <bool COUNT, bool STAMP, bool SHADOW, bool TLAS, bool REFRACT, int CASE, class STK>
__device__ __forceinline__ void trace_body(const CrtDevScene& S, const CrtFrame& F, float4* __restrict__ out, unsigned long long* __restrict__ counters,
                                           const STK& stack, int b, int lane, const CrtGBuffer* gb = nullptr)
{
    constexpr bool SSAA = CASE == CRT_TRACE_SSAA, GBUFFER = CASE == CRT_TRACE_GBUFFER;
    constexpr int kParkNdl = TLAS ? CRT_TLAS_PARK : 0;
    LaneCounters lc; zero_counters(lc);
    WaveStampStart t0 = { 0, 0 };
    if (STAMP) t0 = wave_stamp_start();
    int px, py, costSlot = -1;
    bool isQuadrant = false;
    const unsigned long long tc0 = tile_cost_start(F);
    const bool active = lane_pixel(F, px, py, &costSlot, &isQuadrant, b, lane);
    if (active) {
        PathState ps = camera_path(F, raygen_dir(F, px, py));
        for (int bounce = 0; bounce < 2; ++bounce) {
            if (COUNT) { lc.rays++; if (bounce == 0) lc.primary++; else lc.secondary++; }
            if (SHADOW || GBUFFER) stack.park(kParkNdl, __float_as_uint(ps.energy));
            Closest c = closest_hit<COUNT, STAMP, false, TLAS>(S, ps.o, ps.d, stack, lc);
            if (SHADOW || GBUFFER) ps.energy = __uint_as_float(stack.parked(kParkNdl));
            float ndl = 0.0f;
            int cont;
            if constexpr (!GBUFFER) cont = shade_bounce<SHADOW, REFRACT>(S, c, ps, bounce, F.lightY, F.lightZ, &ndl);
            else {
                const GBufferSink sink = { gb, &F, b, lane };
                cont = shade_bounce<SHADOW, REFRACT, GBufferSink>(S, c, ps, bounce, F.lightY, F.lightZ, &ndl, &sink);
            }
            if (COUNT) { if (cont) lc.hits++; else lc.misses++; }
            if (!cont) break;
            if (SHADOW && cont == 1) {
                if (bounce == 0) {
                    float shadow = 1.0f;
                    if (ndl > 0.0f) {
                        if (COUNT) { lc.rays++; lc.shadowRays++; }
                        stack.park(kParkNdl, __float_as_uint(ndl));
                        const Closest sc = closest_hit<COUNT, false, true, TLAS>(S, ps.o, neg3(mk3(0.0f, F.lightY, F.lightZ)), stack, lc);
                        if (sc.anyHit) { shadow = 0.0f; if (COUNT) lc.shadowHits++; }
                        ndl = __uint_as_float(stack.parked(kParkNdl));
                    }
                    ps.energy = specular_x(ndl, shadow);
                } else ps.energy = ps.energy * specular_x(ndl, 1.0f);
            }
        }
        int qx, qy;
        if constexpr (SSAA) {
            const int k = F.ss;
            v3 rgb = xor_add3<2>(xor_add3<1>(ps.result));
            if (k == 4) rgb = xor_add3<8>(xor_add3<4>(rgb));
            rgb = scale3(rgb, k == 4 ? 1.0f / 16.0f : 0.25f);
            lane_pixel_again(F, b, lane, qx, qy);
            if ((lane & (k * k - 1)) == 0) {
                const int sh = k == 4 ? 2 : 1;
                int w2 = F.width >> sh, h2 = F.height >> sh;
                asm volatile("" : "+s"(w2), "+s"(h2));
                finish_pixel(F, rgb, qx >> sh, qy >> sh, w2, h2, out);
            }
        } else {
            lane_pixel_again(F, b, lane, qx, qy);
            int w2 = F.width, h2 = F.height;
            asm volatile("" : "+s"(w2), "+s"(h2));
            finish_pixel(F, ps.result, qx, qy, w2, h2, out);
        }
    }
    add_tile_cost(F, costSlot, tc0, isQuadrant);
    if (COUNT) flush_counters(lc, counters);
    if (STAMP) write_wave_stamp(counters, lc, t0);
}

template <bool COUNT, bool STAMP = false, bool SHADOW = false, bool TLAS = false, bool REFRACT = false>
__global__ __launch_bounds__(CRT_BLOCK, (COUNT || STAMP) ? CRT_WAVES_PER_SIMD_COUNT : CRT_WAVES_PER_SIMD)
void crt_trace_kernel(CrtDevScene S, CrtFrame F, float4* __restrict__ out, unsigned long long* __restrict__ counters)
{
    __shared__ uint32_t s_stack[CRT_LDS_SLOTS * CRT_BLOCK];
    const CrtTraceStack<SHADOW, TLAS> stack = { (crt_lds_u32_ptr)s_stack + threadIdx.x, S.stackOverflow };
    trace_body<COUNT, STAMP, SHADOW, TLAS, REFRACT, CRT_TRACE_PLAIN>(S, F, out, counters, stack, blockIdx.x, (int)(threadIdx.x & 63));
}

template <bool COUNT, bool SHADOW, bool TLAS, bool REFRACT>
__global__ __launch_bounds__(CRT_BLOCK, COUNT ? CRT_WAVES_PER_SIMD_COUNT - 1 : CRT_WAVES_PER_SIMD)
void crt_trace_ssaa_kernel(CrtDevScene S, CrtFrame F, float4* __restrict__ out, unsigned long long* __restrict__ counters)
{
    __shared__ uint32_t s_stack[CRT_LDS_SLOTS * CRT_BLOCK];
    const CrtTraceStack<SHADOW, TLAS> stack = { (crt_lds_u32_ptr)s_stack + threadIdx.x, S.stackOverflow };
    trace_body<COUNT, false, SHADOW, TLAS, REFRACT, CRT_TRACE_SSAA>(S, F, out, counters, stack, blockIdx.x, (int)(threadIdx.x & 63));
}

template <bool SHADOW, bool TLAS, bool REFRACT>
__global__ __launch_bounds__(CRT_BLOCK, (SHADOW && TLAS && REFRACT) ? CRT_WAVES_PER_SIMD - 1 : CRT_WAVES_PER_SIMD)
void crt_trace_gbuffer_kernel(CrtDevScene S, CrtFrame F, float4* __restrict__ out, CrtGBuffer gb)
{
    __shared__ uint32_t s_stack[CRT_LDS_SLOTS * CRT_BLOCK];
    const CrtTraceStack<true, TLAS> stack = { (crt_lds_u32_ptr)s_stack + threadIdx.x, S.stackOverflow };
    trace_body<false, false, SHADOW, TLAS, REFRACT, CRT_TRACE_GBUFFER>(S, F, out, nullptr, stack, blockIdx.x, (int)(threadIdx.x & 63), &gb);
}

struct CrtBounceRay { float ox, oy, oz, energy, dx, dy, dz; uint32_t pixel; };
__device__ __forceinline__ CrtBounceRay pack_bounce(const PathState& ps, uint32_t pixel)
{
    CrtBounceRay r;
    r.ox = ps.o.x; r.oy = ps.o.y; r.oz = ps.o.z; r.energy = ps.energy;
    r.dx = ps.d.x; r.dy = ps.d.y; r.dz = ps.d.z; r.pixel = pixel;
    return r;
}
__device__ __forceinline__ PathState unpack_bounce(const CrtBounceRay& r, v3 result = mk3(0.0f, 0.0f, 0.0f))
{
    PathState ps;
    ps.o = mk3(r.ox, r.oy, r.oz); ps.d = mk3(r.dx, r.dy, r.dz); ps.result = result; ps.energy = r.energy;
    return ps;
}

template <bool COUNT>
__global__ __launch_bounds__(CRT_BLOCK, COUNT ? CRT_WAVES_PER_SIMD_COUNT : CRT_WAVES_PER_SIMD) void crt_primary_kernel(CrtDevScene S, CrtFrame F, float4* __restrict__ out,
                                                                unsigned long long* __restrict__ counters,
                                                                CrtBounceRay* __restrict__ queue, uint32_t* __restrict__ waveCount)
{
    __shared__ uint32_t s_stack[CRT_LDS_SLOTS * CRT_BLOCK];
    const CrtStack stack = { (crt_lds_u32_ptr)s_stack + threadIdx.x, S.stackOverflow };
    LaneCounters lc; zero_counters(lc);
    int px, py;
    const bool active = lane_pixel(F, px, py);
    bool cont = false;
    PathState ps = camera_path(F, mk3(0.f, 0.f, 0.f));
    if (active) {
        ps.d = raygen_dir(F, px, py);
        if (COUNT) { lc.rays++; lc.primary++; }
        Closest c = closest_hit<COUNT>(S, ps.o, ps.d, stack, lc);
        cont = shade_bounce(S, c, ps, 0, F.lightY, F.lightZ) != 0;
        if (COUNT) { if (cont) lc.hits++; else lc.misses++; }
        out[(size_t)py * (size_t)F.width + (size_t)px] = make_float4(ps.result.x, ps.result.y, ps.result.z, 1.0f);
    }
    const uint32_t entry = (blockIdx.x & 7u) * (uint32_t)F.slotsPerXcd + (blockIdx.x >> 3);
    const unsigned long long m = __ballot(cont);
    if (cont) {
        const uint32_t rank = __builtin_amdgcn_mbcnt_hi((uint32_t)(m >> 32), __builtin_amdgcn_mbcnt_lo((uint32_t)m, 0u));
        queue[(size_t)entry * 64 + rank] = pack_bounce(ps, (uint32_t)py * (uint32_t)F.width + (uint32_t)px);
    }
    if ((threadIdx.x & 63) == 0) waveCount[entry] = (uint32_t)__popcll(m);
    if (COUNT) flush_counters(lc, counters);
}

__global__ __launch_bounds__(1024) void crt_wavefront_scan_kernel(const uint32_t* __restrict__ waveCount, uint32_t* __restrict__ offs, uint32_t* __restrict__ total, int slotsPerXcd)
{
    __shared__ uint32_t s_wave[16];
    const int x = blockIdx.x, tid = threadIdx.x;
    const uint32_t* c = waveCount + (size_t)x * slotsPerXcd;
    uint32_t* o = offs + (size_t)x * slotsPerXcd;
    const int per = (slotsPerXcd + 1023) / 1024, i0 = tid * per, i1 = (i0 + per < slotsPerXcd) ? i0 + per : slotsPerXcd;
    uint32_t sum = 0;
    for (int i = i0; i < i1; ++i) sum += c[i];
    uint32_t incl = sum;
    for (int off = 1; off < 64; off <<= 1) { const uint32_t v = (uint32_t)__shfl_up((int)incl, off, 64); if ((tid & 63) >= off) incl += v; }
    if ((tid & 63) == 63) s_wave[tid >> 6] = incl;
    __syncthreads();
    uint32_t base = incl - sum;
    for (int w = 0; w < (tid >> 6); ++w) base += s_wave[w];
    for (int i = i0; i < i1; ++i) { o[i] = base; base += c[i]; }
    if (tid == 1023) total[x] = base;
}

template <bool COUNT>
__global__ __launch_bounds__(CRT_BLOCK, COUNT ? CRT_WAVES_PER_SIMD_COUNT : CRT_WAVES_PER_SIMD) void crt_bounce_kernel(CrtDevScene S, CrtFrame F, float4* __restrict__ out,
                                                               unsigned long long* __restrict__ counters,
                                                               const CrtBounceRay* __restrict__ queue, const uint32_t* __restrict__ offs,
                                                               const uint32_t* __restrict__ total)
{
    __shared__ uint32_t s_stack[CRT_LDS_SLOTS * CRT_BLOCK];
    const CrtStack stack = { (crt_lds_u32_ptr)s_stack + threadIdx.x, S.stackOverflow };
    LaneCounters lc; zero_counters(lc);
    const uint32_t xcd = blockIdx.x & 7u;
    const uint32_t n = total[xcd];
    const uint32_t k = (blockIdx.x >> 3) * CRT_BLOCK + threadIdx.x;
    if (k < n) {
        const uint32_t* o = offs + (size_t)xcd * (uint32_t)F.slotsPerXcd;
        uint32_t lo = 0, hi = (uint32_t)F.slotsPerXcd;
        while (hi - lo > 1) { const uint32_t mid = (lo + hi) >> 1; if (o[mid] <= k) lo = mid; else hi = mid; }
        const CrtBounceRay r = queue[((size_t)xcd * (uint32_t)F.slotsPerXcd + lo) * 64 + (k - o[lo])];
        const float4 partial = out[r.pixel];
        PathState ps = unpack_bounce(r, mk3(partial.x, partial.y, partial.z));
        if (COUNT) { lc.rays++; lc.secondary++; }
        Closest c = closest_hit<COUNT>(S, ps.o, ps.d, stack, lc);
        const bool cont = shade_bounce(S, c, ps, 1, F.lightY, F.lightZ) != 0;
        if (COUNT) { if (cont) lc.hits++; else lc.misses++; }
        out[r.pixel] = make_float4(ps.result.x, ps.result.y, ps.result.z, 1.0f);
    }
    if (COUNT) flush_counters(lc, counters);
}

__global__ __launch_bounds__(CRT_BLOCK) void crt_raygen_kernel(CrtFrame F, float* __restrict__ rays)
{
    int px, py;
    if (!lane_pixel(F, px, py)) return;
    v3 d = raygen_dir(F, px, py);
    float* o = rays + 3 * ((size_t)px + (size_t)py * (size_t)F.width);
    o[0] = d.x; o[1] = d.y; o[2] = d.z;
}

// ... 118 lines not shown
```

### clraytracer_amd/csrc/crt_shim.hip

```cpp
#include <hip/hip_runtime.h>
#include <math.h>
#include <stdio.h>
#include <string.h>
#include <stdlib.h>
#include "../../include/crt_api.h"
#include "../../include/crt_debug.h"
#include "crt_kernels.h"
#include "crt_refill.h"
#include "crt_ldstop.h"
#include "crt_relayout.h"
#include "crt_bvh_build.h"
#include <vector>
#include <algorithm>
#include <utility>
#include <thread>
#include <mutex>
#include <condition_variable>
#include <functional>
#include <atomic>
#include "crt_state.h"
#include "crt_instances.h"
#include "crt_upload.h"
#include "crt_bvh_driver.h"
#include "crt_frame.h"

#include "crt_multidev.h"

extern "C" {

const char* crt_error_string(int code)
{
    switch (code) {
    case CRT_OK: return "ok";
    case CRT_E_NOT_INITIALIZED: return "crt: not initialized (crt_init failed or was not called)";
    case CRT_E_BAD_ARGUMENT: return "crt: bad argument or invalid scene data";
    case CRT_E_OUT_OF_RANGE: return "crt: out of range (an upload beyond a fixed device pool, a pixel outside the frame)";
    case CRT_E_NO_DEVICE: return "crt: no usable HIP device";
    case CRT_E_UNSUPPORTED: return "crt: unsupported";
    default: return code > 0 ? hipGetErrorString((hipError_t)code) : "crt: unknown error";
    }
}

int crt_row_owner(int row, int bandRows, int nRanks)
{
    if (row < 0 || !valid_bands(bandRows, 0, nRanks)) return CRT_E_BAD_ARGUMENT;
    return (row / bandRows) % nRanks;
}

int crt_band_plan(int height, int bandRows, int rank, int nRanks, int out[4])
{
    if (!out || height < 0 || !valid_bands(bandRows, rank, nRanks)) return CRT_E_BAD_ARGUMENT;
    const BandPlan p = band_plan(height, bandRows, rank, nRanks);
    out[0] = p.firstRow; out[1] = p.fullBands; out[2] = p.tailRow; out[3] = p.tailRows;
    return CRT_OK;
}

static void raise_hw_queues()
{
    (void)setenv("GPU_MAX_HW_QUEUES", "8", 0);
}

int crt_init_devices(const int* devices, int numDevices, int width, int height)
{
    if (M.n != 0) return CRT_E_BAD_ARGUMENT;
    if (!devices || numDevices < 1 || numDevices > CRT_MAX_DEVICES) return CRT_E_BAD_ARGUMENT;
    raise_hw_queues();
    int rc = CRT_OK;
    M.n = numDevices;
    for (int d = 0; d < numDevices && rc == CRT_OK; ++d) {
        M.hipDevice[d] = devices[d];
        M.dev[d] = new State();
        G = M.dev[d];
        rc = init_impl(devices[d], width, height);
        M.peer[d] = 2;
        if (rc == CRT_OK && numDevices > 1) {
            g.bandRows = 16; g.rank = d; g.nRanks = numDevices;
            g.primary = M.dev[0]; g.groupSize = numDevices;
            if (d > 0 && devices[d] != devices[0]) {
                int can = 0;
                (void)hipDeviceCanAccessPeer(&can, devices[d], devices[0]);
                M.peer[d] = 0;
                if (can) {
                    const hipError_t e = hipDeviceEnablePeerAccess(devices[0], 0);
                    if (e == hipSuccess || e == hipErrorPeerAccessAlreadyEnabled) M.peer[d] = 1; else rc = (int)e;
                    (void)hipGetLastError();
                }
                if (M.peer[d] == 0 && rc == CRT_OK)
                    fprintf(stderr, "crt_init_devices: device %d has no peer access to device %d: its bands are gathered through host memory\n", devices[d], devices[0]);
            }
        }
    }
    if (rc == CRT_OK && numDevices > 1) {
        for (int d = 0; d < numDevices; ++d) for (int k = 0; k < numDevices; ++k) M.dev[d]->group[k] = M.dev[k];
        for (int d = 1; d < numDevices; ++d) { M.worker[d] = new Worker(); M.worker[d]->start(M.dev[d], devices[d]); }
    }
    if (rc != CRT_OK) { destroy_group(); return rc; }
    Use::select(0);
    return CRT_OK;
}

int crt_init(int device, int width, int height) { return crt_init_devices(&device, 1, width, height); }

int crt_init_gpus(int numGpus, int width, int height)
{
    raise_hw_queues();
    int have = 0;
    if (hipGetDeviceCount(&have) != hipSuccess || have <= 0) return CRT_E_NO_DEVICE;
    if (numGpus < 1 || numGpus > have || numGpus > CRT_MAX_DEVICES) return CRT_E_BAD_ARGUMENT;
    int ids[CRT_MAX_DEVICES];
    for (int d = 0; d < numGpus; ++d) ids[d] = d;
    return crt_init_devices(ids, numGpus, width, height);
}

int crt_num_devices(void) { return M.n; }
int crt_peer_access(int device) { if (M.n == 0) return CRT_E_NOT_INITIALIZED; if (device < 0 || device >= M.n) return CRT_E_BAD_ARGUMENT; return M.peer[device]; }
const char* crt_gather_path(void)
{
    if (M.n <= 1) return "none (one device)";
    int lo = 2;
    for (int d = 1; d < M.n; ++d) if (M.peer[d] < lo) lo = M.peer[d];
    return lo == 2 ? "same-device copies (rehearsal: one GPU listed several times)" : (lo == 1 ? "xgmi-peer" : "host-staged");
}
int crt_debug_inject_failure(int device)
{
    NEED_SESSION();
    { const char* e = getenv("CRT_DEBUG_HOOKS"); if (!e || atoi(e) == 0) return CRT_E_UNSUPPORTED; }
    if (device < 0 || device >= M.n) return CRT_E_BAD_ARGUMENT;
    M.injectFailure = device;
    return CRT_OK;
}
int crt_debug_staggered_frames(uint64_t* out) { NEED_SESSION(); if (!out) return CRT_E_BAD_ARGUMENT; Use u_(0); *out = g.staggeredFrames; return CRT_OK; }
int crt_debug_tlas_stats(uint64_t* builds, uint32_t* refitsSinceBuild, uint32_t* nodes)
{
    NEED_SESSION();
    Use u_(0);
    if (builds) *builds = g.hTlasBuilds;
    if (refitsSinceBuild) *refitsSinceBuild = g.hTlasRefits;
    if (nodes) *nodes = g.hTlasNodes;
    return CRT_OK;
}
int crt_debug_build_stats(uint32_t* levels, uint32_t* launches)
{
    NEED_SESSION();
    Use u_(0);
    if (levels) *levels = g.buildLevels;
    if (launches) *launches = g.buildLaunches;
    return CRT_OK;
}
int crt_debug_last_gather(uint64_t* bytes, int* bytesPerPixel)
{
    NEED_SESSION();
    if (bytes) *bytes = M.n > 1 ? M.lastGatherBytes : 0;
    if (bytesPerPixel) *bytesPerPixel = M.n > 1 ? M.lastGatherBpp : 0;
    return CRT_OK;
}
int crt_debug_last_kernel(char* dst, size_t cap)
{
    NEED_SESSION();
    if (!dst || cap == 0) return CRT_E_BAD_ARGUMENT;
    Use u_(0);
    snprintf(dst, cap, "%s", g.lastKernel);
    return CRT_OK;
}
int crt_debug_measure_clock(int micros, double* ghz) { ON_PRIMARY(crt1_debug_measure_clock(micros, ghz)); }

int crt_shutdown(void)
{
    NEED_SESSION();
    destroy_group();
    return CRT_OK;
}

const char* crt_device_name(void) { if (M.n == 0) return ""; Use u(0); return crt1_device_name(); }

int crt_resize(int width, int height)
{
    NEED_SESSION();
    if (M.n == 1) { Use u(0); return crt1_resize(width, height); }
    int oldW, oldH;
    { Use u(0); oldW = g.width; oldH = g.height; }
    int rc = CRT_OK, done = 0;
    for (; done < M.n && rc == CRT_OK; ++done) { Use u(done); rc = (done == M.injectFailure) ? (int)CRT_E_UNSUPPORTED : crt1_resize(width, height); }
    if (M.injectFailure >= 0) M.injectFailure = -1;
    if (rc == CRT_OK) return CRT_OK;
    for (int d = 0; d < done - 1; ++d) { Use u(d); if (crt1_resize(oldW, oldH) != CRT_OK) M.broken = true; }
    return rc;
}
int crt_set_row_bands(int bandRows, int rank, int nRanks)
{
    NEED_SESSION();
    if (M.n > 1) return CRT_E_UNSUPPORTED;
    ON_PRIMARY(crt1_set_row_bands(bandRows, rank, nRanks));
}
int crt_owned_rows(void) { if (M.n == 0) return 0; Use u(0); return M.n > 1 ? g.height : crt1_owned_rows(); }

int crt_upload_triangles(const void* tris, size_t byteOffset, size_t bytes) { ON_ALL(crt1_upload_triangles(tris, byteOffset, bytes)); }
int crt_upload_bvh_nodes(const void* nodes, size_t byteOffset, size_t bytes) { ON_ALL(crt1_upload_bvh_nodes(nodes, byteOffset, bytes)); }
int crt_upload_bvh_roots(const uint32_t* roots, size_t firstMesh, size_t count) { ON_ALL(crt1_upload_bvh_roots(roots, firstMesh, count)); }
int crt_upload_materials(const void* materials, size_t first, size_t count) { ON_ALL(crt1_upload_materials(materials, first, count)); }
int crt_upload_texture_table(const void* textures, size_t count) { ON_ALL(crt1_upload_texture_table(textures, count)); }
int crt_upload_texels(const void* rgb8, size_t byteOffset, size_t bytes) { ON_ALL(crt1_upload_texels(rgb8, byteOffset, bytes)); }
int crt_upload_instances(const void* instances, size_t first, size_t count) { ON_ALL(crt1_upload_instances(instances, first, count)); }
int crt_build_bvh(size_t firstTri, const uint32_t* meshTriCounts, int numMeshes, size_t firstNode, size_t firstMesh, uint32_t* nodesUsedOut)
{ ON_ALL(crt1_build_bvh(firstTri, meshTriCounts, numMeshes, firstNode, firstMesh, nodesUsedOut)); }
int crt_download_triangles(void* dst, size_t byteOffset, size_t bytes) { ON_PRIMARY(crt1_download_triangles(dst, byteOffset, bytes)); }
int crt_download_bvh_nodes(void* dst, size_t byteOffset, size_t bytes) { ON_PRIMARY(crt1_download_bvh_nodes(dst, byteOffset, bytes)); }
int crt_download_bvh_roots(uint32_t* dst, size_t firstMesh, size_t count) { ON_PRIMARY(crt1_download_bvh_roots(dst, firstMesh, count)); }

int crt_render(const CrtTraceArgs* args, const float invView[16], const float invProj[16], int flags)
{
    NEED_SESSION();
    if (M.n == 1) { Use u(0); return crt1_render(args, invView, invProj, flags); }
    if (M.broken) return CRT_E_BAD_ARGUMENT;
    if (!args || !invView || !invProj) return CRT_E_BAD_ARGUMENT;
    if (flags & (CRT_RENDER_WRITE_RAYS | CRT_RENDER_STAMPS)) return CRT_E_UNSUPPORTED;
    if ((flags & CRT_RENDER_SSAA2) && (flags & CRT_RENDER_SSAA4)) return CRT_E_BAD_ARGUMENT;
    { Use u(0); RCCHK(refuse_ssaa(flags)); RCCHK(refuse_gbuffer(flags)); }
    RenderPlan plan;
    { Use u(0); plan.slot = frame_is_pipelined(flags) ? (int)(M.seq++ % (unsigned)g.nSlots) : 0; }
    plan.noHostWait = true;
    bool gather8 = false;
    { Use u(0); gather8 = frame_gathers_rgba8(flags); }
    if (gather8) {
        int w, h;
        { Use u(0); w = g.width; h = g.height; }
        if (M.pack8W != w || M.pack8H != h) {
            for (int d = 0; d < M.n; ++d) { Use u(d); RCCHK(crt1_prepare_gather8()); }
            M.pack8W = w; M.pack8H = h;
        }
    }
    {
        Use u(0);
        unsigned long long rows = 0;
        for (int d = 1; d < M.n; ++d) { const BandPlan p = band_plan(g.height, g.bandRows, d, M.n); rows += (unsigned long long)p.fullBands * (unsigned)g.bandRows + (unsigned)p.tailRows; }
        M.lastGatherBpp = gather8 ? 4 : 16; M.lastGatherBytes = rows * (unsigned long long)g.width * (unsigned)M.lastGatherBpp;
    }
    struct Job { CrtTraceArgs a; float iv[16], ip[16]; int flags; RenderPlan plan; } job;
    job.a = *args; memcpy(job.iv, invView, 64); memcpy(job.ip, invProj, 64); job.flags = flags & ~CRT_RENDER_READBACK; job.plan = plan;
    const int failDevice = M.injectFailure;
    M.injectFailure = -1;
    for (int d = 1; d < M.n; ++d) {
        if (d == failDevice) M.worker[d]->post([]() { return (int)CRT_E_UNSUPPORTED; });
        else M.worker[d]->post([job]() { return crt1_render(&job.a, job.iv, job.ip, job.flags, &job.plan); });
    }
    int rc = CRT_OK;
    for (int d = 1; d < M.n; ++d) { const int r = M.worker[d]->wait(); if (r != CRT_OK && rc == CRT_OK) rc = r; }
    if (rc != CRT_OK) return rc;
    if (failDevice == 0) return CRT_E_UNSUPPORTED;
    Use u(0);
    plan.noHostWait = false;
    return crt1_render(args, invView, invProj, flags, &plan);
}

int crt_sync(void) { ON_ALL(crt1_sync()); }

static int drain_secondaries() { for (int d = 1; d < M.n; ++d) { Use u(d); const int r = crt1_sync(); if (r != CRT_OK) return r; } return CRT_OK; }
int crt_query_hits(const float* origins, const float* dirs, int n, uint32_t numInstances, CrtRayHit* out) { ON_PRIMARY(crt1_query_hits(origins, dirs, n, numInstances, out)); }
int crt_read_output(float* dst, size_t floats) { NEED_SESSION(); RCCHK(drain_secondaries()); ON_PRIMARY(crt1_read_output(dst, floats)); }
int crt_read_output_rows(float* dst, int row0, int rows) { NEED_SESSION(); RCCHK(drain_secondaries()); ON_PRIMARY(crt1_read_output_rows(dst, row0, rows)); }
int crt_read_output_rgba8(uint8_t* dst, size_t bytes) { NEED_SESSION(); RCCHK(drain_secondaries()); ON_PRIMARY(crt1_read_output_rgba8(dst, bytes)); }
int crt_map_host_frame_back(int framesBack, const void** ptr, size_t* bytes) { ON_PRIMARY(crt1_map_host_frame_back(framesBack, ptr, bytes)); }
int crt_map_host_frame(const void** ptr, size_t* bytes) { return crt_map_host_frame_back(0, ptr, bytes); }
int crt_read_rays(float* dst, size_t floats) { NEED_SESSION(); if (M.n > 1) return CRT_E_UNSUPPORTED; ON_PRIMARY(crt1_read_rays(dst, floats)); }
int crt_read_gbuffer(int plane, void* dst, size_t bytes) { ON_PRIMARY(crt1_read_gbuffer(plane, dst, bytes)); }
void* crt_gbuffer_device_ptr(int plane) { if (M.n == 0) return nullptr; Use u(0); return crt1_gbuffer_device_ptr(plane); }
int crt_pick_pixel(int x, int y, CrtGBufferPixel* out) { ON_PRIMARY(crt1_pick_pixel(x, y, out)); }
void* crt_output_device_ptr(void) { if (M.n == 0) return nullptr; Use u(0); return crt1_output_device_ptr(); }
float crt_last_kernel_ms(int which) { if (M.n == 0) return -1.0f; Use u(0); return crt1_last_kernel_ms(which); }
int crt_frame_time_stats(CrtFrameStats* out, int reset)
{
    NEED_SESSION();
    for (int d = 1; d < M.n; ++d) { Use u(d); RCCHK(crt1_frame_time_stats(nullptr, reset)); }
    ON_PRIMARY(crt1_frame_time_stats(out, reset));
}
int crt_debug_read_stamps(uint64_t* dst, size_t maxWaves, size_t* numWaves) { ON_PRIMARY(crt1_debug_read_stamps(dst, maxWaves, numWaves)); }
int crt_debug_read_frame_times(double* dst, size_t maxFrames, size_t* numFrames) { ON_PRIMARY(crt1_debug_read_frame_times(dst, maxFrames, numFrames)); }

int crt_get_counters(CrtCounters* out)
{
    NEED_SESSION();
    if (!out) return CRT_E_BAD_ARGUMENT;
    CrtCounters total; memset(&total, 0, sizeof total);
    unsigned long long maxStack = 0;
    for (int d = 0; d < M.n; ++d) {
        Use u(d);
        CrtCounters c;
        RCCHK(crt1_get_counters(&c));
        const unsigned long long* src = reinterpret_cast<const unsigned long long*>(&c);
        unsigned long long* dst = reinterpret_cast<unsigned long long*>(&total);
        for (size_t k = 0; k < sizeof(CrtCounters) / sizeof(unsigned long long); ++k) dst[k] += src[k];
        if (c.maxStack > maxStack) maxStack = c.maxStack;
    }
    total.maxStack = maxStack;
    *out = total;
    return CRT_OK;
}
int crt_get_cull_range(float* limits, int n, float* sceneLimit, float* bounceReach, uint64_t* noCullFrames) { ON_PRIMARY(crt1_get_cull_range(limits, n, sceneLimit, bounceReach, noCullFrames)); }
int crt_get_culled_visits(uint64_t* out)
{
    NEED_SESSION();
    if (!out) return CRT_E_BAD_ARGUMENT;
    uint64_t total = 0;
    for (int d = 0; d < M.n; ++d) { Use u(d); uint64_t c = 0; RCCHK(crt1_get_culled_visits(&c)); total += c; }
    *out = total;
    return CRT_OK;
}
}
```

### clraytracer_amd/csrc/crt_upload.h

```cpp
#pragma once
namespace {


const char* crt1_device_name(void) { return g.deviceName; }

int crt1_upload_texels(const void* rgb8, size_t byteOffset, size_t bytes);

int env_int(const char* name, int dflt) { const char* e = getenv(name); return e ? atoi(e) : dflt; }
float env_float(const char* name, float dflt) { const char* e = getenv(name); return e ? (float)atof(e) : dflt; }
bool env_on(const char* name, bool dflt) { const char* e = getenv(name); return e ? atoi(e) != 0 : dflt; }

const struct { const char* name; Form form; } kKernelForms[] = {
    { "default", Form::Mega }, { "wavefront", Form::Wavefront }, { "refill", Form::Refill }, { "block", Form::Block }, { "ldstop", Form::LdsTop } };


int open_device(int device)
{
    int n = 0;
    if (hipGetDeviceCount(&n) != hipSuccess || n <= 0) return CRT_E_NO_DEVICE;
    if (device < 0 || device >= n) return CRT_E_BAD_ARGUMENT;
    HIPCHK(hipSetDevice(device));
    hipDeviceProp_t prop;
    HIPCHK(hipGetDeviceProperties(&prop, device));
    snprintf(g.deviceName, sizeof g.deviceName, "%s (%s, %d CUs)", prop.name, prop.gcnArchName, prop.multiProcessorCount);
    g.device = device;
    g.numCUs = prop.multiProcessorCount;
    return CRT_OK;
}

int create_frame_slots()
{
    g.nSlots = std::min(std::max(env_int("CRT_FRAMES_IN_FLIGHT", 3), 1), CRT_MAX_FRAMES_IN_FLIGHT);
    for (int si = 0; si < g.nSlots; ++si) {
        FrameSlot& fs = g.slot[si];
        HIPCHK(hipStreamCreateWithFlags(&fs.stream, hipStreamNonBlocking));
        for (EventSet& es : fs.es) for (int i = 0; i < 4; ++i) HIPCHK(hipEventCreate(&es.ev[i]));
        HIPCHK(hipMalloc(&fs.instBlock, kStageBytes));
        fs.instances = reinterpret_cast<CrtMeshInstance*>(fs.instBlock + kStageInst); fs.instBounds = reinterpret_cast<float4*>(fs.instBlock + kStageBounds);
        fs.alwaysList = reinterpret_cast<uint32_t*>(fs.instBlock + kStageAlways); fs.tlas = reinterpret_cast<CrtTlasNode*>(fs.instBlock + kStageTlas);
        HIPCHK(hipMalloc(&fs.devInstances, CRT_MAX_INSTANCES * sizeof(CrtDevInstance)));
        HIPCHK(hipHostMalloc(reinterpret_cast<void**>(&fs.staging), kStageBytes, hipHostMallocDefault));
        HIPCHK(hipHostGetDevicePointer(reinterpret_cast<void**>(&fs.stagingDev), fs.staging, 0));
        for (hipEvent_t* ev : { &fs.staged, &fs.partDone, &fs.slotDone }) HIPCHK(hipEventCreateWithFlags(ev, hipEventDisableTiming));
        HIPCHK(hipEventRecord(fs.staged, fs.stream));
        fs.instVersion = 0;
    }
    HIPCHK(hipEventCreate(&g.statStart));
    g.stream = g.slot[0].stream; g.cur = 0; g.asyncSeq = 0; g.othersBusy = false;
    return CRT_OK;
}

int alloc_pools()
{
    g.triCap = (size_t)CRT_MAX_TRIANGLES * 2;
    g.nodeCap = (size_t)CRT_MAX_TRIANGLES * 2;
    g.texelByteCap = CRT_MAX_TEXTURE_BYTES * 2;
    HIPCHK(hipMalloc(&g.rawTris, g.triCap * sizeof(CrtTri)));
    HIPCHK(hipMemsetAsync(g.rawTris, 0, g.triCap * sizeof(CrtTri), g.stream));
    HIPCHK(hipMalloc(&g.rawNodes, g.nodeCap * sizeof(CrtBVHNode)));
    HIPCHK(hipMalloc(&g.roots, CRT_MAX_MESHES * sizeof(uint32_t)));
    HIPCHK(hipMalloc(&g.rawTexels, g.texelByteCap + 16));
    HIPCHK(hipMalloc(&g.pairs, (g.nodeCap / 2 + 1) * 4 * sizeof(float4)));
    HIPCHK(hipMalloc(&g.triHot, g.triCap * 9 * sizeof(float)));
    HIPCHK(hipMalloc(&g.triCold, g.triCap * 2 * sizeof(uint4)));
    HIPCHK(hipMalloc(&g.bigLeaf, (g.triCap + 1) * sizeof(uint32_t)));
    HIPCHK(hipMemset(g.bigLeaf + g.triCap, 0, sizeof(uint32_t)));
    HIPCHK(hipMalloc(&g.rootRefs, CRT_MAX_MESHES * sizeof(uint32_t)));
    HIPCHK(hipMalloc(&g.topRootRefs, CRT_MAX_MESHES * sizeof(uint32_t)));
    HIPCHK(hipMalloc(&g.topPairs, CRT_TOP_PAIRS * 4 * sizeof(float4)));
    HIPCHK(hipMemset(g.topPairs, 0, CRT_TOP_PAIRS * 4 * sizeof(float4)));
    HIPCHK(hipMalloc(&g.texels, (g.texelByteCap / 3 + 2) * sizeof(uint32_t)));
    HIPCHK(hipMalloc(&g.materials, CRT_MAX_MATERIALS * sizeof(CrtMaterial)));
    HIPCHK(hipMalloc(&g.textures, CRT_MAX_TEXTURES * sizeof(CrtTexture)));
    HIPCHK(hipMalloc(&g.counters, CRT_NUM_COUNTERS * sizeof(unsigned long long)));
    HIPCHK(hipMalloc(&g.err, sizeof(int)));
    HIPCHK(hipMalloc(&g.triReachBits, sizeof(uint32_t)));
    HIPCHK(hipMemset(g.triReachBits, 0, sizeof(uint32_t)));
    static float4 never[CRT_MAX_INSTANCES];
    for (float4& b : never) b = make_float4(0.f, 0.f, 0.f, -1.0f);
    HIPCHK(hipMalloc(&g.noCullBounds, sizeof never));
    HIPCHK(hipMemcpy(g.noCullBounds, never, sizeof never, hipMemcpyHostToDevice));
    return CRT_OK;
}

int read_environment()
{
    const char* e = getenv("CRT_KERNEL");
    const auto* form = std::begin(kKernelForms);
    while (e && *e && form != std::end(kKernelForms) && strcmp(e, form->name) != 0) ++form;
    if (form == std::end(kKernelForms)) {
        fprintf(stderr, "crt_init: CRT_KERNEL=%s is not one of ", e);
        for (const auto& k : kKernelForms) fprintf(stderr, "%s%s", k.name, &k + 1 == std::end(kKernelForms) ? "\n" : ", ");
        return CRT_E_BAD_ARGUMENT;
    }
    g.form = form->form;
    g.splitBeta = env_float("CRT_SPLIT_BETA", CRT_SPLIT_BETA);
    g.splitBetaAsync = env_float("CRT_SPLIT_BETA_ASYNC", CRT_SPLIT_BETA_ASYNC);
    g.costSpread = env_float("CRT_COST_SPREAD", 0.8f);
    const char* split = getenv("CRT_SPLIT");
    g.maxSplit = split ? std::min(std::max(atoi(split), 0), CRT_MAX_SPLIT) : CRT_MAX_SPLIT; g.maxSplitPipelined = split ? g.maxSplit : CRT_MAX_SPLIT_PIPELINED;
    g.gather8 = env_on("CRT_GATHER_RGBA8", true);
    { const char* e = getenv("CRT_TLAS"); g.forceTlas = e ? (atoi(e) != 0 ? 1 : 0) : -1; }
    g.staggerUs = env_int("CRT_STAGGER_US", -1);
    g.feedback = env_on("CRT_FEEDBACK", true);
    g.feedbackAsync = env_on("CRT_FEEDBACK_ASYNC", false);
    return CRT_OK;
}

int reset_scene()
{
    HIPCHK(hipMemset(g.roots, 0, CRT_MAX_MESHES * sizeof(uint32_t)));
    { std::vector<uint32_t> e(CRT_MAX_MESHES, crt_empty_ref((uint32_t)g.triCap)); HIPCHK(hipMemcpy(g.rootRefs, e.data(), e.size() * sizeof(uint32_t), hipMemcpyHostToDevice));
      HIPCHK(hipMemcpy(g.topRootRefs, e.data(), e.size() * sizeof(uint32_t), hipMemcpyHostToDevice)); }
    HIPCHK(hipMemset(g.materials, 0, CRT_MAX_MATERIALS * sizeof(CrtMaterial)));
    HIPCHK(hipMemset(g.textures, 0, CRT_MAX_TEXTURES * sizeof(CrtTexture)));
    HIPCHK(hipMemset(g.texels, 0, 64));
    g.nodeCount = 0; g.numRoots = 0; g.texelBytesHigh = 0; g.trisHigh = 0; g.sceneValid = true; g.instHigh = 0;
    memset(g.hInstances, 0, sizeof g.hInstances); memset(g.hRoots, 0, sizeof g.hRoots);
    memset(g.hHaveRoot, 0, sizeof g.hHaveRoot); g.instVersion = 1;
    rebuild_instance_master();
    return CRT_OK;
}

static int init_impl(int device, int width, int height)
{
    if (g.initialized) return CRT_E_BAD_ARGUMENT;
    if (width < 16 || height < 16) return CRT_E_BAD_ARGUMENT;
    RCCHK(open_device(device));
    RCCHK(create_frame_slots());
    RCCHK(alloc_pools());
    RCCHK(read_environment());
    RCCHK(reset_scene());
    g.bandRows = 16; g.rank = 0; g.nRanks = 1;
    RCCHK(alloc_frame_buffers(width, height));
    g.initialized = true;
    const unsigned char def[6] = { 0xFF, 0xFF, 0xFF, 0, 0, 0 };
    return crt1_upload_texels(def, 0, 6);
}

static void release_all()
{
    for (FrameSlot& fs : g.slot) if (fs.stream) (void)hipStreamSynchronize(fs.stream);
    void* ptrs[] = { g.rawTris, g.rawNodes, g.roots, g.rawTexels, g.pairs, g.triHot, g.triCold, g.bigLeaf, g.rootRefs,
                     g.texels, g.materials, g.textures, g.rays, g.counters, g.err, g.triReachBits, g.topPairs, g.topRootRefs,
                     g.queryBuf, g.buildBuf, g.buildTris, g.stamps, g.noCullBounds };
    for (FrameSlot& fs : g.slot) {
        void* q[] = { fs.out, fs.aux, fs.blockQueue, fs.wfCount, fs.ovf, fs.lists, fs.mixOrder, fs.packBuf, fs.instBlock, fs.devInstances, fs.gbuf };
        for (void* p : q) if (p) (void)hipFree(p);
        if (fs.staging) (void)hipHostFree(fs.staging);
        if (fs.staged) (void)hipEventDestroy(fs.staged);
        if (fs.partDone) (void)hipEventDestroy(fs.partDone);
        if (fs.slotDone) (void)hipEventDestroy(fs.slotDone);
        if (fs.hostBuf) (void)hipHostFree(fs.hostBuf);
        if (fs.copied) (void)hipEventDestroy(fs.copied);
    }
    for (void* p : ptrs) if (p) (void)hipFree(p);
    if (g.statStart) (void)hipEventDestroy(g.statStart);
    if (g.buildCtlHost) (void)hipHostFree(g.buildCtlHost);
    for (FrameSlot& fs : g.slot) {
        for (EventSet& es : fs.es) for (int i = 0; i < 4; ++i) if (es.ev[i]) (void)hipEventDestroy(es.ev[i]);
        if (fs.stream) (void)hipStreamDestroy(fs.stream);
    }
    { State* me = G; *me = State(); }
}

int crt1_resize(int width, int height)
{
    if (!g.initialized) return CRT_E_NOT_INITIALIZED;
    if (width < 16 || height < 16) return CRT_OK;
    RCCHK(sync_all());
    return alloc_frame_buffers(width, height);
}

int crt1_set_row_bands(int bandRows, int rank, int nRanks)
{
    if (!g.initialized) return CRT_E_NOT_INITIALIZED;
    if (!valid_bands(bandRows, rank, nRanks)) return CRT_E_BAD_ARGUMENT;
    RCCHK(sync_all());
    g.bandRows = bandRows; g.rank = rank; g.nRanks = nRanks;
    return CRT_OK;
}

int crt1_owned_rows(void)
{
    if (!g.initialized) return 0;
    const BandPlan p = band_plan(g.height, g.bandRows, g.rank, g.nRanks);
    return p.fullBands * g.bandRows + p.tailRows;
}

#define SPANCHK(p, first, count, unit, cap) do { \
    if (!g.initialized) return CRT_E_NOT_INITIALIZED; \
    if ((count) == 0) return CRT_OK; \
    if (!(p) || (first) % (unit) || (count) % (unit)) return CRT_E_BAD_ARGUMENT; \
    if ((first) + (count) > (cap)) return CRT_E_OUT_OF_RANGE; } while (0)

int crt1_upload_triangles(const void* tris, size_t byteOffset, size_t bytes)
{
    SPANCHK(tris, byteOffset, bytes, sizeof(CrtTri), g.triCap * sizeof(CrtTri));
    RCCHK(quiesce());
    HIPCHK(hipMemcpyAsync(reinterpret_cast<char*>(g.rawTris) + byteOffset, tris, bytes, hipMemcpyHostToDevice, g.stream));
    const size_t first = byteOffset / sizeof(CrtTri), count = bytes / sizeof(CrtTri);
    crt_relayout_tris<<<(unsigned)((count + 255) / 256), 256, 0, g.stream>>>(g.rawTris, first, count, g.triHot, g.triCold);
    HIPCHK(hipGetLastError());
    HIPCHK(hipStreamSynchronize(g.stream));
    const bool overwrites = first < g.trisHigh;
    if (first + count > g.trisHigh) g.trisHigh = first + count;
    if (overwrites) HIPCHK(hipMemsetAsync(g.triReachBits, 0, sizeof(uint32_t), g.stream));
    {
        const size_t f0 = overwrites ? 0 : first, n0 = overwrites ? g.trisHigh : count;
        crt_tri_reach_kernel<<<(unsigned)((n0 + 255) / 256), 256, 0, g.stream>>>(g.rawTris, f0, n0, g.triReachBits);
        HIPCHK(hipGetLastError());
    }
    uint32_t bitsHost = 0;
    HIPCHK(hipMemcpyAsync(&bitsHost, g.triReachBits, sizeof bitsHost, hipMemcpyDeviceToHost, g.stream));
    HIPCHK(hipStreamSynchronize(g.stream));
    {
        float f; memcpy(&f, &bitsHost, sizeof f);
        const double far2 = (f == f && f < 3.0e38f) ? (double)f * (1.0 + 1e-6) : 1e300;
        if (far2 != g.triReach2) { g.triReach2 = far2; rebuild_instance_master(); }
    }
    return CRT_OK;
}

int crt1_upload_bvh_nodes(const void* nodes, size_t byteOffset, size_t bytes)
{
    SPANCHK(nodes, byteOffset, bytes, sizeof(CrtBVHNode), g.nodeCap * sizeof(CrtBVHNode));
    RCCHK(quiesce());
    HIPCHK(hipMemcpyAsync(reinterpret_cast<char*>(g.rawNodes) + byteOffset, nodes, bytes, hipMemcpyHostToDevice, g.stream));
    const uint32_t high = (uint32_t)((byteOffset + bytes) / sizeof(CrtBVHNode));
    if (high > g.nodeCount) g.nodeCount = high;
    return rebuild_bvh_layout();
// ... 71 lines not shown
```

### clraytracer_amd/host/crt_host_c.cpp

```cpp
#include "../../include/crt_host.h"
#include "../../include/crt_api.h"
#include "AssetManager.hpp"
#include "CPURayTrace.hpp"
#include "JpegDecode.hpp"
#include "Renderer.hpp"
#include <cstdio>
#include <cstring>
#include <thread>
#include <vector>

namespace ResourceManager { size_t TexelBytesUsed(); int NumMaterials(); int NumTextures(); size_t NumTriangles(); size_t NumNodes(); }

namespace { bool hostOnly = false; int hostOnlyError = 0; }

extern "C" {

int crth_initialize(int device, int width, int height) { hostOnly = false; hostOnlyError = 0; return Renderer::Initialize(device, width, height); }
int crth_initialize_devices(const int* devices, int numDevices, int width, int height) { hostOnly = false; hostOnlyError = 0; return Renderer::InitializeDevices(devices, numDevices, width, height); }

int crth_initialize_host_only(int width, int height)
{
    hostOnly = true; hostOnlyError = 0;
    ResourceManager::Initialize(false);
    g_NumMeshInstances = 0;
    Renderer::ClearAllInstances();
    Camera& cam = Renderer::EditCamera();
    cam = Camera();
    cam.RecalculateProjection(width, height);
    cam.RecalculateView();
    return 1;
}

void crth_terminate(void) { if (hostOnly) ResourceManager::Finalize(); else Renderer::Terminate(); hostOnly = false; }
int crth_last_error(void) { return hostOnlyError ? hostOnlyError : Renderer::LastError(); }
void crth_clear_error(void) { hostOnlyError = 0; Renderer::ClearError(); }

void crth_prepare_meshes(void) { ResourceManager::PrepareMeshes(); }
int crth_import_texture(const char* path) { return ResourceManager::ImportTexture(path); }
int crth_import_texture_rgb8(const char* name, int w, int h, const unsigned char* rgb) { return ResourceManager::ImportTextureRGB8(name, w, h, rgb); }
int crth_import_mesh(const char* path) { return ResourceManager::ImportMesh(path); }
void crth_push_meshes(void) { ResourceManager::PushMeshesToGPU(); }
void crth_set_mesh_cache(int enabled) { AssetManager_SetMeshCache(enabled != 0); }
size_t crth_qlz_decompress(const unsigned char* src, size_t srcLen, unsigned char* dst, size_t dstCap) { return MeshCache_QlzDecompress(src, srcLen, dst, dstCap); }
size_t crth_jpeg_decode(const unsigned char* data, size_t size, unsigned char* dst, size_t dstCap, int info[4], const char** error)
{
    std::vector<unsigned char> rgb;
    JpegInfo ji;
    if (!JpegDecodeRGB8(data, size, &ji, rgb, error)) return 0;
    if (info) { info[0] = ji.width; info[1] = ji.height; info[2] = ji.components; info[3] = ji.progressive ? 1 : 0; }
    if (dst) { if (dstCap < rgb.size()) return 0; std::memcpy(dst, rgb.data(), rgb.size()); }
    return rgb.size();
}
void crth_set_asset_root(const char* dir) { ResourceManager::SetAssetRoot(dir); }
size_t crth_qlz_store(const unsigned char* src, size_t size, unsigned char* dst) { return MeshCache_QlzStore(src, size, dst); }
size_t crth_qlz_compress(const unsigned char* src, size_t size, unsigned char* dst) { return MeshCache_QlzCompress(src, size, dst); }
void crth_set_device_bvh_build(int enabled) { ResourceManager::SetDeviceBVHBuild(enabled != 0); }
void crth_push_textures(void) { ResourceManager::PushTexturesToGPU(); }
void crth_push_materials(void) { ResourceManager::PushMaterialsToGPU(); }
int crth_create_material(int count) { MaterialHandle h = 0; return ResourceManager::CreateMaterial(&h, count) ? (int)h : -1; }
void crth_edit_material(int handle, const CrtMaterial* value) { if (value && handle >= 0 && handle < CRT_MAX_MATERIALS) ResourceManager::EditMaterial((MaterialHandle)handle) = *value; }

void crth_begin_instances(void) { Renderer::BeginInstanceRegister(); }
unsigned crth_register_instance(int mesh, int material, const float matrix[16])
{
    Matrix4 m; std::memcpy(&m, matrix, 64);
    return Renderer::RegisterMeshInstance((MeshHandle)mesh, (MaterialHandle)material, m);
}
void crth_end_instances(void) { Renderer::EndInstanceRegister(); }
void crth_clear_instances(void) { Renderer::ClearAllInstances(); }
void crth_set_mesh_matrix(unsigned instance, const float matrix[16]) { Matrix4 m; std::memcpy(&m, matrix, 64); Renderer::SetMeshMatrix(instance, m); }
void crth_set_mesh_position(unsigned instance, const float p[3]) { Renderer::SetMeshPosition(instance, float3(p[0], p[1], p[2])); }
void crth_set_instance_material(unsigned instance, int material) { Renderer::SetMeshInstanceMaterial(instance, (MaterialHandle)material); }

void crth_set_camera(const float position[3], const float front[3])
{
    Camera& cam = Renderer::EditCamera();
    cam.position = Vector3f(position[0], position[1], position[2]);
    cam.Front = Vector3f(front[0], front[1], front[2]);
    cam.RecalculateView();
}
void crth_get_camera(float invView[16], float invProj[16], float position[3])
{
    const Camera& cam = Renderer::GetCamera();
    std::memcpy(invView, &cam.inverseView, 64);
    std::memcpy(invProj, &cam.inverseProjection, 64);
    position[0] = cam.position.x; position[1] = cam.position.y; position[2] = cam.position.z;
}
void crth_resize(int width, int height)
{
    if (hostOnly) { if (width >= 16 && height >= 16) Renderer::EditCamera().RecalculateProjection(width, height); }
    else Renderer::OnWindowResize(width, height);
}
void crth_set_postprocess(int enabled) { Renderer::SetPostProcess(enabled != 0); }
void crth_set_shadows(int enabled) { Renderer::SetShadows(enabled != 0); }
void crth_set_refraction(int enabled) { Renderer::SetRefraction(enabled != 0); }
void crth_set_fxaa(int enabled) { Renderer::SetFXAA(enabled != 0); }
void crth_set_supersampling(int factor) { Renderer::SetSupersampling(factor); }
void crth_set_gbuffer(int enabled) { Renderer::SetGBuffer(enabled != 0); }
const void* crth_map_gbuffer(int plane) { if (hostOnly) { hostOnlyError = CRT_E_NOT_INITIALIZED; return nullptr; } return Renderer::MapGBuffer(plane); }
int crth_pick_pixel(int x, int y, CrtGBufferPixel* out)
{
    if (hostOnly) { hostOnlyError = CRT_E_NOT_INITIALIZED; return 0; }
    return (out && Renderer::PickPixel(x, y, *out)) ? 1 : 0;
}
void crth_set_unorm8(int enabled) { Renderer::SetUnorm8(enabled != 0); }
const unsigned char* crth_map_output_rgba8(void) { return hostOnly ? nullptr : Renderer::MapOutputRGBA8(); }
void crth_set_pipelined(int enabled) { Renderer::SetPipelined(enabled != 0); }
void crth_set_row_bands(int bandRows, int rank, int nRanks) { Renderer::SetRowBands(bandRows, rank, nRanks); }
unsigned crth_render(float sunAngle)
{
    if (hostOnly) { hostOnlyError = CRT_E_NOT_INITIALIZED; std::fprintf(stderr, "[crth] render requested in a host-only session: there is no CPU render path\n"); return 0; }
    return Renderer::Render(sunAngle);
}
const float* crth_map_output(void) { return hostOnly ? nullptr : Renderer::MapOutput(); }
float crth_last_frame_ms(void) { return hostOnly ? -1.0f : Renderer::LastFrameMs(); }

static void cpu_raycast_many(HitRecord (*cast)(RaySSE), const float* origins, const float* dirs, int n, CrtHitRecord* out, int nthreads)
{
    if (nthreads < 1) nthreads = 1;
    auto work = [&](int t) {
        for (int base = t * 4096; base < n; base += nthreads * 4096) {
            const int end = base + 4096 < n ? base + 4096 : n;
            for (int k = base; k < end; ++k) {
                RaySSE r;
                r.origin[0] = origins[3 * k]; r.origin[1] = origins[3 * k + 1]; r.origin[2] = origins[3 * k + 2]; r.origin[3] = 1.0f;
                r.direction[0] = dirs[3 * k]; r.direction[1] = dirs[3 * k + 1]; r.direction[2] = dirs[3 * k + 2]; r.direction[3] = 0.0f;
                out[k] = cast(r);
            }
        }
    };
    if (nthreads == 1) { work(0); return; }
    std::vector<std::thread> pool;
    for (int t = 0; t < nthreads; ++t) pool.emplace_back(work, t);
    for (auto& th : pool) th.join();
}
void crth_cpu_raycast(const float* origins, const float* dirs, int n, CrtHitRecord* out, int nthreads) { cpu_raycast_many(CPU_RayCast, origins, dirs, n, out, nthreads); }
void crth_cpu_raycast_sse(const float* origins, const float* dirs, int n, CrtHitRecord* out, int nthreads) { cpu_raycast_many(CPU_RayCastSSE, origins, dirs, n, out, nthreads); }

const CrtTri* crth_triangles(void) { return g_Triangles; }
size_t crth_num_triangles(void) { return ResourceManager::NumTriangles(); }
const CrtBVHNode* crth_nodes(void) { return g_BVHNodes; }
size_t crth_num_nodes(void) { return ResourceManager::NumNodes(); }
const uint32_t* crth_roots(void) { return g_BVHIndices; }
int crth_num_meshes(void) { return ResourceManager::GetNumMeshes(); }
const CrtMaterial* crth_materials(void) { return g_Materials; }
int crth_num_materials(void) { return ResourceManager::NumMaterials(); }
const CrtTexture* crth_textures(void) { return g_Textures; }
int crth_num_textures(void) { return ResourceManager::NumTextures(); }
const CrtRGB8* crth_texels(void) { return g_TexturePixels; }
size_t crth_texel_bytes(void) { return ResourceManager::TexelBytesUsed(); }
const CrtMeshInstance* crth_instances(void) { return g_MeshInstances; }
unsigned crth_num_instances(void) { return g_NumMeshInstances; }
void crth_mesh_info(int mesh, uint32_t out[4])
{
    MeshInfo mi = ResourceManager::GetMeshInfo((MeshHandle)mesh);
    out[0] = mi.numTriangles; out[1] = mi.triangleStart; out[2] = mi.materialStart; out[3] = mi.numMaterials;
}

uint32_t crth_build_bvh(CrtTri* tris, const uint32_t* meshTriCounts, int numMeshes, CrtBVHNode* nodes, uint32_t* roots)
{
    std::vector<MeshInfo> infos((size_t)numMeshes);
    uint32_t start = 0;
    for (int i = 0; i < numMeshes; ++i) { infos[i] = MeshInfo{ meshTriCounts[i], start, 0, 0, nullptr }; start += meshTriCounts[i]; }
    ResetBVHNodeCounter();
    uint32_t n = BuildBVH(tris, infos.data(), numMeshes, nodes, roots);
    ResetBVHNodeCounter();
    return n;
}
uint16_t crth_float_to_half(float v) { return crtmath::ConvertFloatToHalf(v); }
float crth_half_to_float(uint16_t h) { return crtmath::ConvertHalfToFloat(h); }
void crth_inverse_transform(const float in[16], float out[16]) { Matrix4 m; std::memcpy(&m, in, 64); m = Matrix4::InverseTransform(m); std::memcpy(out, &m, 64); }
void crth_inverse(const float in[16], float out[16]) { Matrix4 m; std::memcpy(&m, in, 64); m = Matrix4::Inverse(m); std::memcpy(out, &m, 64); }
void crth_perspective_fov_rh(float fov, float w, float h, float zn, float zf, float out[16]) { Matrix4 m = Matrix4::PerspectiveFovRH(fov, w, h, zn, zf); std::memcpy(out, &m, 64); }
void crth_look_at_rh(const float eye[3], const float front[3], const float up[3], float out[16])
{
    Matrix4 m = Matrix4::LookAtRH(Vector3f(eye[0], eye[1], eye[2]), Vector3f(front[0], front[1], front[2]), Vector3f(up[0], up[1], up[2]));
    std::memcpy(out, &m, 64);
}
int crth_write_obj(const char* path, const float* positions, int numPositions, const float* uvs, int numUvs,
                   const float* normals, int numNormals, const int* faces, const int* faceMaterial, int numFaces,
                   const char* const* materialNames, int numMaterials)
{
    return AssetManager_WriteObj(path, positions, numPositions, uvs, numUvs, normals, numNormals, faces, faceMaterial, numFaces, materialNames, numMaterials);
}

}
```

### include/crt_debug.h

```cpp
#ifndef CRT_DEBUG_H
#define CRT_DEBUG_H
#include "crt_api.h"
#ifdef __cplusplus
extern "C" {
#endif

int crt_debug_read_stamps(uint64_t* dst, size_t maxWaves, size_t* numWaves);
int crt_debug_read_frame_times(double* dst, size_t maxFrames, size_t* numFrames);
int crt_debug_measure_clock(int micros, double* ghz);
int crt_debug_inject_failure(int device);
int crt_debug_staggered_frames(uint64_t* out);

int crt_debug_last_kernel(char* dst, size_t cap);
int crt_debug_last_gather(uint64_t* bytes, int* bytesPerPixel);
int crt_debug_build_stats(uint32_t* levels, uint32_t* launches);
int crt_debug_tlas_stats(uint64_t* builds, uint32_t* refitsSinceBuild, uint32_t* nodes);

#ifdef __cplusplus
}
#endif
#endif
```

### include/crt_host.h

```cpp
#ifndef CRT_HOST_H
#define CRT_HOST_H
#include <stddef.h>
#include <stdint.h>
#include "crt_types.h"
#ifdef __cplusplus
extern "C" {
#endif

int crth_initialize(int device, int width, int height);
int crth_initialize_devices(const int* devices, int numDevices, int width, int height);
int crth_initialize_host_only(int width, int height);
void crth_terminate(void);
int crth_last_error(void);
void crth_clear_error(void);

void crth_prepare_meshes(void);
int crth_import_texture(const char* path);
int crth_import_texture_rgb8(const char* name, int width, int height, const unsigned char* rgb);
int crth_import_mesh(const char* path);
void crth_push_meshes(void);
void crth_set_device_bvh_build(int enabled);
void crth_set_mesh_cache(int enabled);
size_t crth_qlz_decompress(const unsigned char* src, size_t srcLen, unsigned char* dst, size_t dstCap);
size_t crth_qlz_store(const unsigned char* src, size_t size, unsigned char* dst);
size_t crth_qlz_compress(const unsigned char* src, size_t size, unsigned char* dst);
size_t crth_jpeg_decode(const unsigned char* data, size_t size, unsigned char* dst, size_t dstCap, int info[4], const char** error);
void crth_set_asset_root(const char* dir);
void crth_push_textures(void);
void crth_push_materials(void);
int crth_create_material(int count);
void crth_edit_material(int handle, const CrtMaterial* value);

void crth_begin_instances(void);
unsigned crth_register_instance(int mesh, int material, const float matrix[16]);
void crth_end_instances(void);
void crth_clear_instances(void);
void crth_set_mesh_matrix(unsigned instance, const float matrix[16]);
void crth_set_mesh_position(unsigned instance, const float position[3]);
void crth_set_instance_material(unsigned instance, int material);

void crth_set_camera(const float position[3], const float front[3]);
void crth_get_camera(float invView[16], float invProj[16], float position[3]);
void crth_resize(int width, int height);
void crth_set_postprocess(int enabled);
void crth_set_shadows(int enabled);
void crth_set_fxaa(int enabled);
void crth_set_supersampling(int factor);
void crth_set_gbuffer(int enabled);
const void* crth_map_gbuffer(int plane);
int crth_pick_pixel(int x, int y, CrtGBufferPixel* out);
void crth_set_refraction(int enabled);
void crth_set_unorm8(int enabled);
const unsigned char* crth_map_output_rgba8(void);
void crth_set_pipelined(int enabled);
void crth_set_row_bands(int bandRows, int rank, int nRanks);
unsigned crth_render(float sunAngle);
const float* crth_map_output(void);
float crth_last_frame_ms(void);

void crth_cpu_raycast(const float* origins, const float* dirs, int n, CrtHitRecord* out, int nthreads);
void crth_cpu_raycast_sse(const float* origins, const float* dirs, int n, CrtHitRecord* out, int nthreads);

const CrtTri* crth_triangles(void);         size_t crth_num_triangles(void);
const CrtBVHNode* crth_nodes(void);         size_t crth_num_nodes(void);
const uint32_t* crth_roots(void);           int crth_num_meshes(void);
const CrtMaterial* crth_materials(void);    int crth_num_materials(void);
const CrtTexture* crth_textures(void);      int crth_num_textures(void);
const CrtRGB8* crth_texels(void);           size_t crth_texel_bytes(void);
const CrtMeshInstance* crth_instances(void); unsigned crth_num_instances(void);
void crth_mesh_info(int mesh, uint32_t out[4]);

uint32_t crth_build_bvh(CrtTri* tris, const uint32_t* meshTriCounts, int numMeshes, CrtBVHNode* nodes, uint32_t* roots);
uint16_t crth_float_to_half(float v);
float crth_half_to_float(uint16_t h);
void crth_inverse_transform(const float in[16], float out[16]);
void crth_inverse(const float in[16], float out[16]);
void crth_perspective_fov_rh(float fovRad, float width, float height, float zNear, float zFar, float out[16]);
void crth_look_at_rh(const float eye[3], const float front[3], const float up[3], float out[16]);
int crth_write_obj(const char* path, const float* positions, int numPositions, const float* uvs, int numUvs,
                   const float* normals, int numNormals, const int* faces, const int* faceMaterial, int numFaces,
                   const char* const* materialNames, int numMaterials);

void* crth_shm_barrier_open(const char* name, int nRanks, int create);
int crth_shm_barrier_wait(void* handle, int timeoutMs);
void crth_shm_barrier_close(void* handle);

#ifdef __cplusplus
}
#endif
#endif
```

Before: 10600.

## Add fast float skybox indexing, deferred sky merge, and paired-bounds culling

Result: faster. 10840, median of 6 (+2.3%).

```diff
diff --git a/clraytracer_amd/_lib.py b/clraytracer_amd/_lib.py
--- a/clraytracer_amd/_lib.py
+++ b/clraytracer_amd/_lib.py
@@ -71,6 +71,9 @@
     "crt_debug_build_stats": (C.c_int, [C.POINTER(C.c_uint32), C.POINTER(C.c_uint32)]),
     "crt_debug_tlas_stats": (C.c_int, [C.POINTER(C.c_uint64), C.POINTER(C.c_uint32), C.POINTER(C.c_uint32)]),
     "crt_debug_measure_clock": (C.c_int, [C.c_int, C.POINTER(C.c_double)]),
+    "crt_debug_cull_counts": (C.c_int, [_fp, _fp, C.c_int, C.c_uint32, _vp]),
+    "crt_debug_instance_bounds": (C.c_int, [_fp, C.c_int]),
+    "crt_debug_skybox_indices": (C.c_int, [_fp, C.c_int, C.c_int, C.c_int, _vp, _vp, _vp, _vp]),
     "crt_shutdown": (C.c_int, []),
     "crt_resize": (C.c_int, [C.c_int, C.c_int]),
     "crt_set_row_bands": (C.c_int, [C.c_int, C.c_int, C.c_int]),
@@ -173,6 +176,8 @@
     "crth_float_to_half": (C.c_uint16, [_f]),
     "crth_half_to_float": (_f, [C.c_uint16]),
     "crth_inverse_transform": (None, [_fp, _fp]),
+    "crth_skybox_indices": (None, [_fp, _sz, C.c_int, C.c_int, _vp, _vp, _vp, _vp, _vp, _vp]),
+    "crth_skybox_bounds": (None, [_fp]),
     "crth_inverse": (None, [_fp, _fp]),
     "crth_perspective_fov_rh": (None, [_f, _f, _f, _f, _f, _fp]),
     "crth_look_at_rh": (None, [_fp, _fp, _fp, _fp]),
diff --git a/clraytracer_amd/csrc/crt_debug_kernels.hip b/clraytracer_amd/csrc/crt_debug_kernels.hip
--- /dev/null
+++ b/clraytracer_amd/csrc/crt_debug_kernels.hip
@@ -0,0 +1,74 @@
+#include <hip/hip_runtime.h>
+#include "crt_device.h"
+
+__global__ void crt_skybox_indices_kernel(const float* __restrict__ dirs, int n, int texW, int texH, int* __restrict__ idxFinal,
+                                          int* __restrict__ idxDouble, int* __restrict__ decided, int* __restrict__ idxFast)
+{
+    const int i = (int)(blockIdx.x * blockDim.x + threadIdx.x);
+    if (i >= n) return;
+    const v3 d = mk3(dirs[3 * (size_t)i], dirs[3 * (size_t)i + 1], dirs[3 * (size_t)i + 2]);
+    const CrtSkyIndex f = crt_skybox_index_fast(d.x, d.y, d.z, texW, texH);
+    idxFinal[i] = skybox_index(d, texW, texH);
+    idxDouble[i] = sample_skybox(d, texW, texH);
+    decided[i] = f.decided;
+    idxFast[i] = f.index;
+}
+
+int crt_skybox_indices_on_device(const float* dirs, int n, int texW, int texH, int* idxFinal, int* idxDouble, int* decided, int* idxFast)
+{
+    const size_t dirBytes = sizeof(float) * 3 * (size_t)n, outBytes = sizeof(int) * (size_t)n;
+    char* d = nullptr;
+    hipError_t e = hipMalloc(&d, dirBytes + 4 * outBytes);
+    if (e != hipSuccess) return (int)e;
+    int* o = reinterpret_cast<int*>(d + dirBytes);
+    e = hipMemcpy(d, dirs, dirBytes, hipMemcpyHostToDevice);
+    if (e == hipSuccess) {
+        crt_skybox_indices_kernel<<<(unsigned)(((size_t)n + 255) / 256), 256>>>(reinterpret_cast<const float*>(d), n, texW, texH, o, o + (size_t)n,
+                                                                              o + 2 * (size_t)n, o + 3 * (size_t)n);
+        e = hipGetLastError();
+    }
+    int* dst[4] = { idxFinal, idxDouble, decided, idxFast };
+    for (int k = 0; k < 4 && e == hipSuccess; ++k) e = hipMemcpy(dst[k], o + (size_t)k * (size_t)n, outBytes, hipMemcpyDeviceToHost);
+    (void)hipFree(d);
+    return (int)e;
+}
+
+__global__ void crt_cull_counts_kernel(const float4* __restrict__ bounds, uint32_t numInstances, const float* __restrict__ origins,
+                                       const float* __restrict__ dirs, int n, uint32_t* __restrict__ culled)
+{
+    const int i = (int)(blockIdx.x * blockDim.x + threadIdx.x);
+    if (i >= n) return;
+    CrtDevScene S;
+    memset(&S, 0, sizeof S);
+    S.instBounds = bounds; S.numInstances = numInstances;
+    const v3 o = mk3(origins[3 * (size_t)i], origins[3 * (size_t)i + 1], origins[3 * (size_t)i + 2]);
+    const v3 d = mk3(dirs[3 * (size_t)i], dirs[3 * (size_t)i + 1], dirs[3 * (size_t)i + 2]);
+    LaneCounters lc;
+    memset(&lc, 0, sizeof lc);
+    for (uint32_t base = 0; base < numInstances; base += 64) {
+        const uint32_t cnt = (numInstances - base) < 64u ? (numInstances - base) : 64u;
+        (void)candidate_mask<true, false, true>(S, o, d, base, cnt, lc);
+    }
+    culled[i] = lc.culled;
+}
+
+int crt_cull_counts_on_device(const float* bounds, uint32_t numInstances, const float* origins, const float* dirs, int n, uint32_t* culled)
+{
+    const size_t bBytes = sizeof(float4) * CRT_BOUNDS_ENTRIES, rayBytes = sizeof(float) * 3 * (size_t)n, outBytes = sizeof(uint32_t) * (size_t)n;
+    char* d = nullptr;
+    hipError_t e = hipMalloc(&d, bBytes + 2 * rayBytes + outBytes);
+    if (e != hipSuccess) return (int)e;
+    float* dO = reinterpret_cast<float*>(d + bBytes);
+    float* dD = reinterpret_cast<float*>(d + bBytes + rayBytes);
+    uint32_t* dC = reinterpret_cast<uint32_t*>(d + bBytes + 2 * rayBytes);
+    e = hipMemcpy(d, bounds, bBytes, hipMemcpyHostToDevice);
+    if (e == hipSuccess) e = hipMemcpy(dO, origins, rayBytes, hipMemcpyHostToDevice);
+    if (e == hipSuccess) e = hipMemcpy(dD, dirs, rayBytes, hipMemcpyHostToDevice);
+    if (e == hipSuccess) {
+        crt_cull_counts_kernel<<<(unsigned)(((size_t)n + 63) / 64), 64>>>(reinterpret_cast<const float4*>(d), numInstances, dO, dD, n, dC);
+        e = hipGetLastError();
+    }
+    if (e == hipSuccess) e = hipMemcpy(culled, dC, outBytes, hipMemcpyDeviceToHost);
+    (void)hipFree(d);
+    return (int)e;
+}
diff --git a/clraytracer_amd/csrc/crt_device.h b/clraytracer_amd/csrc/crt_device.h
--- a/clraytracer_amd/csrc/crt_device.h
+++ b/clraytracer_amd/csrc/crt_device.h
@@ -4,6 +4,7 @@
 #include <stdint.h>
 #include <type_traits>
 #include "../../include/crt_types.h"
+#include "../../include/crt_skybox_index.h"
 
 #define CRT_LEAF_BIT 0x80000000u
 #define CRT_TOP_BIT 0x40000000u
@@ -15,6 +16,9 @@
 typedef uint32_t __attribute__((address_space(3))) * crt_lds_u32_ptr;
 typedef float crt_f32x4 __attribute__((ext_vector_type(4)));
 typedef const crt_f32x4 __attribute__((address_space(4)))* crt_const_f32x4_ptr;
+typedef float crt_f32x8 __attribute__((ext_vector_type(8)));
+typedef const crt_f32x8 __attribute__((address_space(4)))* crt_const_f32x8_ptr;
+#define CRT_BOUNDS_ENTRIES ((CRT_MAX_INSTANCES + 3) & ~3)
 typedef const crt_f32x4 __attribute__((address_space(3)))* crt_lds_f32x4_ptr;
 #ifndef CRT_LDS_SLOTS
 #define CRT_LDS_SLOTS 20
@@ -382,19 +386,38 @@
     return (bs.w >= 0.0f) & ((oc2 * dd - b * b > r2 * dd) | ((b < 0.0f) & (oc2 > r2)));
 }
 
-template <bool COUNT, bool DEFER_COUNT = false>
+template <bool COUNT, bool DEFER_COUNT = false, bool BATCH = false>
 __device__ __forceinline__ unsigned long long candidate_mask(const CrtDevScene& S, v3 o, v3 d, uint32_t base, uint32_t cnt, LaneCounters& lc)
 {
     const float dd = dot3(d, d);
     unsigned long long cand = 0;
-    const crt_const_f32x4_ptr bounds = (crt_const_f32x4_ptr)S.instBounds;
-    for (uint32_t k = 0; k < cnt; ++k) {
-        const crt_f32x4 bs = bounds[base + k];
-        const v3 oc = mk3(bs.x - o.x, bs.y - o.y, bs.z - o.z);
-        const float oc2 = dot3(oc, oc), b = dot3(oc, d);
-        const float r2 = bs.w * bs.w * 1.0201f + 4e-6f * oc2;
-        const bool cull = (bs.w >= 0.0f) && ((oc2 * dd - b * b > r2 * dd) || (b < 0.0f && oc2 > r2));
-        if (!cull) cand |= 1ull << k;
+    if constexpr (BATCH) {
+        const crt_const_f32x8_ptr bounds2 = (crt_const_f32x8_ptr)S.instBounds + (base >> 1);
+        for (uint32_t k2 = 0; k2 < cnt; k2 += 2) {
+            const crt_f32x8 q = bounds2[k2 >> 1];
+            uint32_t nib = 0;
+#pragma unroll
+            for (int j = 0; j < 2; ++j) {
+                const float bx = q[4 * j], by = q[4 * j + 1], bz = q[4 * j + 2], bw = q[4 * j + 3];
+                const v3 oc = mk3(bx - o.x, by - o.y, bz - o.z);
+                const float oc2 = dot3(oc, oc), b = dot3(oc, d);
+                const float r2 = bw * bw * 1.0201f + 4e-6f * oc2;
+                const bool cull = (bw >= 0.0f) & ((oc2 * dd - b * b > r2 * dd) | ((b < 0.0f) & (oc2 > r2)));
+                nib |= cull ? 0u : (1u << j);
+            }
+            cand |= (unsigned long long)nib << k2;
+        }
+        cand &= cnt >= 64u ? ~0ull : ((1ull << cnt) - 1ull);
+    } else {
+        const crt_const_f32x4_ptr bounds = (crt_const_f32x4_ptr)S.instBounds;
+        for (uint32_t k = 0; k < cnt; ++k) {
+            const crt_f32x4 bs = bounds[base + k];
+            const v3 oc = mk3(bs.x - o.x, bs.y - o.y, bs.z - o.z);
+            const float oc2 = dot3(oc, oc), b = dot3(oc, d);
+            const float r2 = bs.w * bs.w * 1.0201f + 4e-6f * oc2;
+            const bool cull = (bs.w >= 0.0f) && ((oc2 * dd - b * b > r2 * dd) || (b < 0.0f && oc2 > r2));
+            if (!cull) cand |= 1ull << k;
+        }
     }
     if (COUNT && !DEFER_COUNT) { const uint32_t culled = cnt - (uint32_t)__popcll(cand); count_culled(lc, culled); }
     return cand;
@@ -471,7 +494,7 @@
     }
 }
 
-template <bool COUNT, bool ITERS = false, bool ANYHIT = false, bool TLAS = false, class STK = CrtStack>
+template <bool COUNT, bool ITERS = false, bool ANYHIT = false, bool TLAS = false, bool BATCH = false, class STK = CrtStack>
 __device__ __forceinline__ Closest closest_hit(const CrtDevScene& S, v3 o, v3 d, const STK& stack, LaneCounters& lc)
 {
     Closest c = no_hit();
@@ -509,7 +532,7 @@
 
     for (uint32_t base = 0; base < S.numInstances; base += 64) {
         const uint32_t cnt = (S.numInstances - base) < 64u ? (S.numInstances - base) : 64u;
-        unsigned long long cand = candidate_mask<COUNT, ANYHIT>(S, o, d, base, cnt, lc);
+        unsigned long long cand = candidate_mask<COUNT, ANYHIT, BATCH>(S, o, d, base, cnt, lc);
         unsigned long long culledLeft = (COUNT && ANYHIT) ? (~cand & (cnt == 64u ? ~0ull : ((1ull << cnt) - 1ull))) : 0ull;
         bool done = ANYHIT && c.anyHit;
         for (;;) {
@@ -553,6 +576,18 @@
     return (int)((uint32_t)phi * (uint32_t)texW + (uint32_t)(theta + 2));
 }
 
+template <bool FAST = true>
+__device__ __forceinline__ int skybox_index(v3 d, int texW, int texH)
+{
+    if constexpr (!FAST) return sample_skybox(d, texW, texH);
+    const CrtSkyIndex f = crt_skybox_index_fast(d.x, d.y, d.z, texW, texH);
+    int idx = f.index;
+    if (__ballot(!f.decided) != 0) {
+        if (!f.decided) idx = sample_skybox(d, texW, texH);
+    }
+    return idx;
+}
+
 __device__ __forceinline__ int sample_texture(const CrtTexture& tex, float u, float v)
 {
     u = u - floorf(u);
@@ -593,20 +628,38 @@
     return (sp * 0.2f) * ndl;
 }
 
+#ifndef CRT_SKY_FAST
+#define CRT_SKY_FAST 1
+#endif
+#ifndef CRT_SKY_MERGE
+#define CRT_SKY_MERGE 1
+#endif
+#ifndef CRT_CULL_BATCH
+#define CRT_CULL_BATCH 1
+#endif
+#define CRT_BOUNCES 2
+#define CRT_SKYMODE_DOUBLE 0
+#define CRT_SKYMODE_FAST 1
+#define CRT_SKYMODE_DEFER 2
 struct NoSink { };
-template <bool DEFER_ENERGY = false, bool REFRACT = false, class SINK = NoSink>
+template <bool FAST = true>
+__device__ __forceinline__ v3 sky_radiance(const CrtDevScene& S, v3 d)
+{
+    const crt_f32x4 skyHdr = ((crt_const_f32x4_ptr)S.textures)[2];
+    const int idx = clamp_texel(skybox_index<FAST>(d, __float_as_int(skyHdr.x), __float_as_int(skyHdr.y)), S.numTexels);
+    const uint32_t px = S.texels[idx];
+    return scale3(mk3((float)(px & 0xffu), (float)((px >> 8) & 0xffu), (float)((px >> 16) & 0xffu)), 1.0f / 255.0f);
+}
+template <bool DEFER_ENERGY = false, bool REFRACT = false, class SINK = NoSink, int SKY = CRT_SKYMODE_DOUBLE>
 __device__ __forceinline__ int shade_bounce(const CrtDevScene& S, const Closest& c, PathState& ps, int bounce, float lightY, float lightZ,
                                             float* ndlOut = nullptr, const SINK* sink = nullptr)
 {
     constexpr bool kSink = !std::is_same<SINK, NoSink>::value;
+    static_assert(SKY != CRT_SKYMODE_DEFER || CRT_BOUNCES == 2, "the deferred sky lookup is argued for two bounces: revisit the energy's sign-bit mark");
     const float UcharToFloat01 = 1.0f / 255.0f;
     if (c.distance > 99998.0f) {
         if constexpr (kSink) { if (bounce == 0) sink->miss(c); }
-        const crt_f32x4 skyHdr = ((crt_const_f32x4_ptr)S.textures)[2];
-        int idx = clamp_texel(sample_skybox(ps.d, __float_as_int(skyHdr.x), __float_as_int(skyHdr.y)), S.numTexels);
-        uint32_t px = S.texels[idx];
-        v3 skyc = scale3(mk3((float)(px & 0xffu), (float)((px >> 8) & 0xffu), (float)((px >> 16) & 0xffu)), UcharToFloat01);
-        ps.result = add3(ps.result, scale3(skyc, ps.energy));
+        if constexpr (SKY != CRT_SKYMODE_DEFER) ps.result = add3(ps.result, scale3(sky_radiance<SKY == CRT_SKYMODE_FAST>(S, ps.d), ps.energy));
         return 0;
     }
     const v3 light = bounce == 0 ? mk3(0.0f, lightY, lightZ) : ps.d;
@@ -679,6 +732,6 @@
     ps.result = add3(ps.result, add3(add3(scale3(scale3(color, ndl), ps.energy), ambient), mk3(sl, sl, sl)));
     if (REFRACT && transmitted) { ps.energy = ps.energy * (1.0f - opacity); return 2; }
     if (DEFER_ENERGY) *ndlOut = ndl;
-    else ps.energy = ps.energy * specular_x(ndl, 1.0f);
+    else if (SKY != CRT_SKYMODE_DEFER || bounce < CRT_BOUNCES - 1) ps.energy = ps.energy * specular_x(ndl, 1.0f);
     return 1;
 }
diff --git a/clraytracer_amd/csrc/crt_frame.h b/clraytracer_amd/csrc/crt_frame.h
--- a/clraytracer_amd/csrc/crt_frame.h
+++ b/clraytracer_amd/csrc/crt_frame.h
@@ -528,6 +528,15 @@
     return CRT_OK;
 }
 
+int crt1_debug_skybox_indices(const float* dirs, int n, int texW, int texH, int* idxFinal, int* idxDouble, int* decided, int* idxFast)
+{
+    if (!g.initialized) return CRT_E_NOT_INITIALIZED;
+    if (n <= 0) return CRT_OK;
+    if (!dirs || !idxFinal || !idxDouble || !decided || !idxFast) return CRT_E_BAD_ARGUMENT;
+    RCCHK(sync_all());
+    return ::crt_skybox_indices_on_device(dirs, n, texW, texH, idxFinal, idxDouble, decided, idxFast);
+}
+
 int crt1_sync(void)
 {
     if (!g.initialized) return CRT_E_NOT_INITIALIZED;
@@ -738,6 +747,25 @@
     return CRT_OK;
 }
 
+int crt1_debug_instance_bounds(float* dst, int n)
+{
+    if (!g.initialized) return CRT_E_NOT_INITIALIZED;
+    if (n < 0 || n > CRT_MAX_INSTANCES || (n > 0 && !dst)) return CRT_E_BAD_ARGUMENT;
+    for (int i = 0; i < n; ++i) { dst[4 * i] = g.hBounds[i].x; dst[4 * i + 1] = g.hBounds[i].y; dst[4 * i + 2] = g.hBounds[i].z; dst[4 * i + 3] = g.hBounds[i].w; }
+    return CRT_OK;
+}
+
+int crt1_debug_cull_counts(const float* origins, const float* dirs, int n, uint32_t numInstances, uint32_t* culledPerRay)
+{
+    if (!g.initialized) return CRT_E_NOT_INITIALIZED;
+    if (n <= 0) return CRT_OK;
+    if (!origins || !dirs || !culledPerRay || numInstances > CRT_MAX_INSTANCES) return CRT_E_BAD_ARGUMENT;
+    static float4 padded[CRT_BOUNDS_ENTRIES];
+    for (int k = 0; k < CRT_BOUNDS_ENTRIES; ++k) padded[k] = k < CRT_MAX_INSTANCES ? g.hBounds[k] : make_float4(0.f, 0.f, 0.f, -1.0f);
+    RCCHK(sync_all());
+    return ::crt_cull_counts_on_device(reinterpret_cast<const float*>(padded), numInstances, origins, dirs, n, culledPerRay);
+}
+
 int crt1_get_counters(CrtCounters* out)
 {
     if (!g.initialized) return CRT_E_NOT_INITIALIZED;
diff --git a/clraytracer_amd/csrc/crt_instances.h b/clraytracer_amd/csrc/crt_instances.h
--- a/clraytracer_amd/csrc/crt_instances.h
+++ b/clraytracer_amd/csrc/crt_instances.h
@@ -255,7 +255,7 @@
 
 constexpr size_t kStageInst = 0;
 constexpr size_t kStageBounds = (kStageInst + CRT_MAX_INSTANCES * sizeof(CrtMeshInstance) + 255) & ~(size_t)255;
-constexpr size_t kStageAlways = (kStageBounds + CRT_MAX_INSTANCES * sizeof(float4) + 255) & ~(size_t)255;
+constexpr size_t kStageAlways = (kStageBounds + CRT_BOUNDS_ENTRIES * sizeof(float4) + 255) & ~(size_t)255;
 constexpr size_t kStageTlas = (kStageAlways + CRT_MAX_INSTANCES * sizeof(uint32_t) + 255) & ~(size_t)255;
 constexpr size_t kStageBytes = kStageTlas + 2 * CRT_MAX_INSTANCES * sizeof(CrtTlasNode);
 
@@ -265,6 +265,7 @@
     HIPCHK(hipEventSynchronize(fs.staged));
     memcpy(fs.staging + kStageInst, g.hInstances, CRT_MAX_INSTANCES * sizeof(CrtMeshInstance));
     memcpy(fs.staging + kStageBounds, g.hBounds, CRT_MAX_INSTANCES * sizeof(float4));
+    for (int k = CRT_MAX_INSTANCES; k < CRT_BOUNDS_ENTRIES; ++k) reinterpret_cast<float4*>(fs.staging + kStageBounds)[k] = make_float4(0.f, 0.f, 0.f, -1.0f);
     if (g.hNumAlways) memcpy(fs.staging + kStageAlways, g.hAlways, g.hNumAlways * sizeof(uint32_t));
     if (g.hTlasNodes) memcpy(fs.staging + kStageTlas, g.hTlas, g.hTlasNodes * sizeof(CrtTlasNode));
     static_assert(kStageInst == 0 && kStageBytes % 16 == 0 && kStageTlas % 16 == 0 && sizeof(CrtTlasNode) % 16 == 0, "copied as 16-byte words");
diff --git a/clraytracer_amd/csrc/crt_kernels.h b/clraytracer_amd/csrc/crt_kernels.h
--- a/clraytracer_amd/csrc/crt_kernels.h
+++ b/clraytracer_amd/csrc/crt_kernels.h
@@ -289,6 +289,10 @@
 {
     constexpr bool SSAA = CASE == CRT_TRACE_SSAA, GBUFFER = CASE == CRT_TRACE_GBUFFER;
     constexpr int kParkNdl = TLAS ? CRT_TLAS_PARK : 0;
+    constexpr bool kDeferSky = CRT_SKY_MERGE != 0 && CASE == CRT_TRACE_PLAIN && !(COUNT && TLAS);
+    constexpr int kSky = kDeferSky ? CRT_SKYMODE_DEFER : (CRT_SKY_FAST != 0 ? CRT_SKYMODE_FAST : CRT_SKYMODE_DOUBLE);
+    constexpr bool kCullBatch = CRT_CULL_BATCH != 0;
+    static_assert(CRT_BOUNCES == 2, "the sign-bit mark below is argued for the camera ray and one bounce");
     LaneCounters lc; zero_counters(lc);
     WaveStampStart t0 = { 0, 0 };
     if (STAMP) t0 = wave_stamp_start();
@@ -298,34 +302,35 @@
     const bool active = lane_pixel(F, px, py, &costSlot, &isQuadrant, b, lane);
     if (active) {
         PathState ps = camera_path(F, raygen_dir(F, px, py));
-        for (int bounce = 0; bounce < 2; ++bounce) {
+        for (int bounce = 0; bounce < CRT_BOUNCES; ++bounce) {
             if (COUNT) { lc.rays++; if (bounce == 0) lc.primary++; else lc.secondary++; }
             if (SHADOW || GBUFFER) stack.park(kParkNdl, __float_as_uint(ps.energy));
-            Closest c = closest_hit<COUNT, STAMP, false, TLAS>(S, ps.o, ps.d, stack, lc);
+            Closest c = closest_hit<COUNT, STAMP, false, TLAS, kCullBatch>(S, ps.o, ps.d, stack, lc);
             if (SHADOW || GBUFFER) ps.energy = __uint_as_float(stack.parked(kParkNdl));
             float ndl = 0.0f;
             int cont;
-            if constexpr (!GBUFFER) cont = shade_bounce<SHADOW, REFRACT>(S, c, ps, bounce, F.lightY, F.lightZ, &ndl);
+            if constexpr (!GBUFFER) cont = shade_bounce<SHADOW, REFRACT, NoSink, kSky>(S, c, ps, bounce, F.lightY, F.lightZ, &ndl);
             else {
                 const GBufferSink sink = { gb, &F, b, lane };
-                cont = shade_bounce<SHADOW, REFRACT, GBufferSink>(S, c, ps, bounce, F.lightY, F.lightZ, &ndl, &sink);
+                cont = shade_bounce<SHADOW, REFRACT, GBufferSink, kSky>(S, c, ps, bounce, F.lightY, F.lightZ, &ndl, &sink);
             }
             if (COUNT) { if (cont) lc.hits++; else lc.misses++; }
-            if (!cont) break;
+            if (!cont) { if (kDeferSky) ps.energy = -ps.energy; break; }
             if (SHADOW && cont == 1) {
                 if (bounce == 0) {
                     float shadow = 1.0f;
                     if (ndl > 0.0f) {
                         if (COUNT) { lc.rays++; lc.shadowRays++; }
                         stack.park(kParkNdl, __float_as_uint(ndl));
-                        const Closest sc = closest_hit<COUNT, false, true, TLAS>(S, ps.o, neg3(mk3(0.0f, F.lightY, F.lightZ)), stack, lc);
+                        const Closest sc = closest_hit<COUNT, false, true, TLAS, kCullBatch>(S, ps.o, neg3(mk3(0.0f, F.lightY, F.lightZ)), stack, lc);
                         if (sc.anyHit) { shadow = 0.0f; if (COUNT) lc.shadowHits++; }
                         ndl = __uint_as_float(stack.parked(kParkNdl));
                     }
                     ps.energy = specular_x(ndl, shadow);
-                } else ps.energy = ps.energy * specular_x(ndl, 1.0f);
+                } else if (!kDeferSky) ps.energy = ps.energy * specular_x(ndl, 1.0f);
             }
         }
+        if (kDeferSky && __float_as_int(ps.energy) < 0) ps.result = add3(ps.result, scale3(sky_radiance<CRT_SKY_FAST != 0>(S, ps.d), -ps.energy));
         int qx, qy;
         if constexpr (SSAA) {
             const int k = F.ss;
diff --git a/clraytracer_amd/csrc/crt_shim.hip b/clraytracer_amd/csrc/crt_shim.hip
--- a/clraytracer_amd/csrc/crt_shim.hip
+++ b/clraytracer_amd/csrc/crt_shim.hip
@@ -5,6 +5,8 @@
 #include <stdlib.h>
 #include "../../include/crt_api.h"
 #include "../../include/crt_debug.h"
+int crt_skybox_indices_on_device(const float* dirs, int n, int texW, int texH, int* idxFinal, int* idxDouble, int* decided, int* idxFast);
+int crt_cull_counts_on_device(const float* bounds, uint32_t numInstances, const float* origins, const float* dirs, int n, uint32_t* culled);
 #include "crt_kernels.h"
 #include "crt_refill.h"
 #include "crt_ldstop.h"
@@ -163,6 +165,12 @@
     return CRT_OK;
 }
 int crt_debug_measure_clock(int micros, double* ghz) { ON_PRIMARY(crt1_debug_measure_clock(micros, ghz)); }
+int crt_debug_instance_bounds(float* dst, int n) { ON_PRIMARY(crt1_debug_instance_bounds(dst, n)); }
+int crt_debug_cull_counts(const float* origins, const float* dirs, int n, uint32_t numInstances, uint32_t* culledPerRay) { ON_PRIMARY(crt1_debug_cull_counts(origins, dirs, n, numInstances, culledPerRay)); }
+int crt_debug_skybox_indices(const float* dirs, int n, int texW, int texH, int* idxFinal, int* idxDouble, int* decided, int* idxFast)
+{
+    ON_PRIMARY(crt1_debug_skybox_indices(dirs, n, texW, texH, idxFinal, idxDouble, decided, idxFast));
+}
 
 int crt_shutdown(void)
 {
diff --git a/clraytracer_amd/csrc/crt_upload.h b/clraytracer_amd/csrc/crt_upload.h
--- a/clraytracer_amd/csrc/crt_upload.h
+++ b/clraytracer_amd/csrc/crt_upload.h
@@ -76,7 +76,7 @@
     HIPCHK(hipMalloc(&g.err, sizeof(int)));
     HIPCHK(hipMalloc(&g.triReachBits, sizeof(uint32_t)));
     HIPCHK(hipMemset(g.triReachBits, 0, sizeof(uint32_t)));
-    static float4 never[CRT_MAX_INSTANCES];
+    static float4 never[CRT_BOUNDS_ENTRIES];
     for (float4& b : never) b = make_float4(0.f, 0.f, 0.f, -1.0f);
     HIPCHK(hipMalloc(&g.noCullBounds, sizeof never));
     HIPCHK(hipMemcpy(g.noCullBounds, never, sizeof never, hipMemcpyHostToDevice));
diff --git a/clraytracer_amd/host/crt_host_c.cpp b/clraytracer_amd/host/crt_host_c.cpp
--- a/clraytracer_amd/host/crt_host_c.cpp
+++ b/clraytracer_amd/host/crt_host_c.cpp
@@ -1,5 +1,7 @@
 #include "../../include/crt_host.h"
 #include "../../include/crt_api.h"
+#include "../../include/crt_skybox_index.h"
+#include <cmath>
 #include "AssetManager.hpp"
 #include "CPURayTrace.hpp"
 #include "JpegDecode.hpp"
@@ -170,6 +172,26 @@
 uint16_t crth_float_to_half(float v) { return crtmath::ConvertFloatToHalf(v); }
 float crth_half_to_float(uint16_t h) { return crtmath::ConvertHalfToFloat(h); }
 void crth_inverse_transform(const float in[16], float out[16]) { Matrix4 m; std::memcpy(&m, in, 64); m = Matrix4::InverseTransform(m); std::memcpy(out, &m, 64); }
+void crth_skybox_indices(const float* dirs, size_t n, int texW, int texH, int* idxFinal, int* idxDouble, int* decided, int* idxFast,
+                         float* aHat, float* cHat)
+{
+    const double PI = 3.14159265358979323846;
+    for (size_t i = 0; i < n; ++i) {
+        const float x = dirs[3 * i], y = dirs[3 * i + 1], z = dirs[3 * i + 2];
+        const float at = (float)(atan2((double)x, (double)(-z)) / PI);
+        const float ac = (float)(acos((double)y) / PI);
+        const int theta = crt_sky_f2i((at * 0.5f) * (float)texW), phi = crt_sky_f2i(ac * (float)texH);
+        const int dbl = (int)((uint32_t)phi * (uint32_t)texW + (uint32_t)(theta + 2));
+        const CrtSkyIndex f = crt_skybox_index_fast(x, y, z, texW, texH);
+        idxDouble[i] = dbl;
+        idxFast[i] = f.index;
+        decided[i] = f.decided;
+        idxFinal[i] = f.decided ? f.index : dbl;
+        if (aHat) aHat[i] = crt_sky_azimuth(x, z);
+        if (cHat) cHat[i] = crt_sky_polar(y);
+    }
+}
+void crth_skybox_bounds(float out[4]) { out[0] = CRT_SKY_EPS_A; out[1] = CRT_SKY_EPS_C; out[2] = CRT_SKY_DELTA; out[3] = CRT_SKY_MIN_XZ; }
 void crth_inverse(const float in[16], float out[16]) { Matrix4 m; std::memcpy(&m, in, 64); m = Matrix4::Inverse(m); std::memcpy(out, &m, 64); }
 void crth_perspective_fov_rh(float fov, float w, float h, float zn, float zf, float out[16]) { Matrix4 m = Matrix4::PerspectiveFovRH(fov, w, h, zn, zf); std::memcpy(out, &m, 64); }
 void crth_look_at_rh(const float eye[3], const float front[3], const float up[3], float out[16])
diff --git a/clraytracer_amd/skybox_dirs.py b/clraytracer_amd/skybox_dirs.py
--- /dev/null
+++ b/clraytracer_amd/skybox_dirs.py
@@ -0,0 +1,83 @@
+import ctypes as C
+from concurrent.futures import ThreadPoolExecutor
+
+import numpy as np
+
+from . import _lib
+
+SIZES = [(2048, 1024), (512, 256), (3, 7), (1, 1)]
+
+
+def _ulps(v, k):
+    v = np.asarray(v, np.float32).copy()
+    for _ in range(abs(k)):
+        v = np.nextafter(v, np.float32(np.inf if k > 0 else -np.inf), dtype=np.float32)
+    return v
+
+
+def structured(W, H):
+    out = []
+    k = np.arange(-(W // 2) - 1, W // 2 + 2, dtype=np.float64)
+    az = k * (2.0 * np.pi / W)
+    for y in (0.0, 0.3, -0.85):
+        s = np.sqrt(1.0 - y * y)
+        x, z = (np.sin(az) * s).astype(np.float32), (-np.cos(az) * s).astype(np.float32)
+        for u in range(-4, 5):
+            out.append(np.stack([_ulps(x, u), np.full_like(x, y), z], 1))
+            out.append(np.stack([x, np.full_like(x, y), _ulps(z, u)], 1))
+    k = np.arange(0, H + 1, dtype=np.float64)
+    y = np.cos(k * (np.pi / H)).astype(np.float32)
+    for a in (0.4, 2.5, -1.1):
+        s = np.sqrt(np.maximum(0.0, 1.0 - y.astype(np.float64) ** 2))
+        x, z = (np.sin(a) * s).astype(np.float32), (-np.cos(a) * s).astype(np.float32)
+        for u in range(-4, 5):
+            out.append(np.stack([x, _ulps(y, u), z], 1))
+    one = np.float32(1.0)
+    up1, up2 = _ulps([one], 1)[0], _ulps([one], 2)[0]
+    den, tiny = np.float32(1e-42), np.float32(1e-31)
+    nan, inf = np.float32(np.nan), np.float32(np.inf)
+    special = [
+        (0, 1, 0), (0, -1, 0), (-0.0, 1, -0.0), (0.0, -1, 0.0),
+        (0.1, up1, 0.2), (0.1, -up1, 0.2), (0.1, up2, 0.2), (0, -up2, 0), (0.3, 1, 0.1), (0.3, -1, -0.1), (0, 1.5, 1), (1, -2, 0),
+        (0.0, 0.2, 1.0), (-0.0, 0.2, 1.0), (0.0, -0.7, 0.5), (-0.0, 0.0, 1e-3),
+        (0.0, 0.2, -1.0), (-0.0, 0.2, -1.0),
+        (0, 0.5, 0), (-0.0, 0.5, 0.0), (0.0, 0.0, -0.0), (0, 0.999, 0),
+        (den, 0.5, 0), (0, 0.5, den), (den, 0.5, -den), (-den, -0.5, den), (tiny, 0.1, tiny), (den, 0.5, 1), (1, 0.5, den), (1, den, 1),
+        (-1, -den, -den), (1e-20, 0.3, 1), (1, 0.3, 1e-20), (1e-29, 0.3, 3e-30), (1e38, 0.3, 1e38), (3.2e38, 0.1, 1), (1, 0.1, -3.3e38),
+        (nan, 0.1, 1), (1, nan, 1), (1, 0.1, nan), (nan, nan, nan), (inf, 0.1, 1), (-inf, 0.1, 1), (1, inf, 1), (1, -inf, 1), (1, 0.1, inf),
+        (1, 0.1, -inf), (inf, 0.5, inf), (inf, inf, inf), (1, 1, 1), (-1, -1, -1), (0.6, 0.0, 0.8), (1, 0, 0), (-1, 0, 0), (0, 0, 1), (0, 0, -1),
+        (1, 0, 1), (1, 0, -1), (-1, 0, 1), (-1, 0, -1), (0.5, 0.70710678, 0.5), (0.5, -0.70710678, -0.5),
+    ]
+    out.append(np.asarray(special, np.float32))
+    return np.ascontiguousarray(np.concatenate(out, 0), np.float32)
+
+
+def seeded(n, seed):
+    rng = np.random.default_rng(seed)
+    d = rng.standard_normal((n, 3), dtype=np.float32)
+    d /= np.sqrt((d.astype(np.float64) ** 2).sum(1, keepdims=True)).astype(np.float32)
+    return np.ascontiguousarray(d, np.float32)
+
+
+def host_indices(dirs, W, H, angles=False, threads=8):
+    h = _lib.host()
+    n = len(dirs)
+    r = {k: np.empty(n, np.int32) for k in ("final", "double", "decided", "fast")}
+    if angles:
+        r["aHat"], r["cHat"] = np.empty(n, np.float32), np.empty(n, np.float32)
+
+    def run(lo, hi):
+        p = lambda a: a[lo:hi].ctypes.data_as(C.c_void_p)
+        h.crth_skybox_indices(dirs[lo:hi].ctypes.data_as(C.POINTER(C.c_float)), hi - lo, W, H, p(r["final"]), p(r["double"]), p(r["decided"]),
+                              p(r["fast"]), p(r["aHat"]) if angles else None, p(r["cHat"]) if angles else None)
+
+    cuts = np.linspace(0, n, (threads if n > 100000 else 1) + 1).astype(int)
+    with ThreadPoolExecutor(max_workers=threads) as ex:
+        list(ex.map(lambda i: run(cuts[i], cuts[i + 1]), range(len(cuts) - 1)))
+    return r
+
+
+def bounds():
+    b = (C.c_float * 4)()
+    _lib.host().crth_skybox_bounds(b)
+    return {"eps_a": float(b[0]), "eps_c": float(b[1]), "delta": float(b[2]), "min_xz": float(b[3])}
diff --git a/include/crt_debug.h b/include/crt_debug.h
--- a/include/crt_debug.h
+++ b/include/crt_debug.h
@@ -15,6 +15,9 @@
 int crt_debug_last_gather(uint64_t* bytes, int* bytesPerPixel);
 int crt_debug_build_stats(uint32_t* levels, uint32_t* launches);
 int crt_debug_tlas_stats(uint64_t* builds, uint32_t* refitsSinceBuild, uint32_t* nodes);
+int crt_debug_instance_bounds(float* dst, int n);
+int crt_debug_cull_counts(const float* origins, const float* dirs, int n, uint32_t numInstances, uint32_t* culledPerRay);
+int crt_debug_skybox_indices(const float* dirs, int n, int texW, int texH, int* idxFinal, int* idxDouble, int* decided, int* idxFast);
 
 #ifdef __cplusplus
 }
diff --git a/include/crt_host.h b/include/crt_host.h
--- a/include/crt_host.h
+++ b/include/crt_host.h
@@ -77,6 +77,9 @@
 void crth_inverse(const float in[16], float out[16]);
 void crth_perspective_fov_rh(float fovRad, float width, float height, float zNear, float zFar, float out[16]);
 void crth_look_at_rh(const float eye[3], const float front[3], const float up[3], float out[16]);
+void crth_skybox_indices(const float* dirs, size_t n, int texW, int texH, int* idxFinal, int* idxDouble, int* decided, int* idxFast,
+                         float* aHat, float* cHat);
+void crth_skybox_bounds(float out[4]);
 int crth_write_obj(const char* path, const float* positions, int numPositions, const float* uvs, int numUvs,
                    const float* normals, int numNormals, const int* faces, const int* faceMaterial, int numFaces,
                    const char* const* materialNames, int numMaterials);
diff --git a/include/crt_skybox_index.h b/include/crt_skybox_index.h
--- /dev/null
+++ b/include/crt_skybox_index.h
@@ -0,0 +1,82 @@
+#ifndef CRT_SKYBOX_INDEX_H
+#define CRT_SKYBOX_INDEX_H
+#include <math.h>
+#include <stdint.h>
+
+#if defined(__HIPCC__)
+#define CRT_SKY_FN __host__ __device__ static inline __attribute__((always_inline))
+#else
+#define CRT_SKY_FN static inline
+#endif
+
+#define CRT_SKY_EPS_A 2.6e-7f
+#define CRT_SKY_EPS_C 2.9e-7f
+#define CRT_SKY_DELTA 6.1e-8f
+#define CRT_SKY_GUARD_A 3.3e-7f
+#define CRT_SKY_GUARD_C 3.6e-7f
+#define CRT_SKY_MIN_XZ 1e-30f
+#define CRT_SKY_MAX_XZ 3.0e38f
+
+typedef struct CrtSkyIndex { int index; int decided; } CrtSkyIndex;
+
+CRT_SKY_FN int crt_sky_f2i(float x)
+{
+    if (!(x == x)) return 0;
+    if (x >= 2147483648.0f) return 2147483647;
+    if (x <= -2147483648.0f) return (-2147483647 - 1);
+    return (int)x;
+}
+
+CRT_SKY_FN float crt_sky_atan_pi(float mn, float mx)
+{
+    const float t = mn / mx;
+    const float s = t * t;
+    float p = -0x1.7c7b9cp-10f;
+    p = p * s + 0x1.f01462p-8f;
+    p = p * s + -0x1.32ceecp-6f;
+    p = p * s + 0x1.01570ap-5f;
+    p = p * s + -0x1.6d2628p-5f;
+    p = p * s + 0x1.045426p-4f;
+    p = p * s + -0x1.b2944cp-4f;
+    p = p * s + 0x1.45f304p-2f;
+    return t * p;
+}
+
+CRT_SKY_FN float crt_sky_azimuth(float x, float z)
+{
+    const float ax = fabsf(x), az = fabsf(z);
+    const int swap = ax > az;
+    float q = crt_sky_atan_pi(swap ? az : ax, swap ? ax : az);
+    if (swap) q = 0.5f - q;
+    if (z > 0.0f) q = 1.0f - q;
+    return copysignf(q, x);
+}
+
+CRT_SKY_FN float crt_sky_polar(float y)
+{
+    const float ay = fabsf(y);
+    const float sy = sqrtf((1.0f - y) * (1.0f + y));
+    const int swap = sy > ay;
+    float q = crt_sky_atan_pi(swap ? ay : sy, swap ? sy : ay);
+    if (swap) q = 0.5f - q;
+    if (y < 0.0f) q = 1.0f - q;
+    return q;
+}
+
+CRT_SKY_FN CrtSkyIndex crt_skybox_index_fast(float x, float y, float z, int texW, int texH)
+{
+    CrtSkyIndex r;
+    const float ax = fabsf(x), az = fabsf(z);
+    const int valid = (ax <= CRT_SKY_MAX_XZ) & (az <= CRT_SKY_MAX_XZ) & ((ax >= CRT_SKY_MIN_XZ) | (az >= CRT_SKY_MIN_XZ)) &
+                      (fabsf(y) < 1.0f) & (texW > 0) & (texH > 0);
+    if (!valid) { r.index = 0; r.decided = 0; return r; }
+    const float a = crt_sky_azimuth(x, z), c = crt_sky_polar(y);
+    const float w = (float)texW, h = (float)texH;
+    const int tl = crt_sky_f2i(((a - CRT_SKY_GUARD_A) * 0.5f) * w), th = crt_sky_f2i(((a + CRT_SKY_GUARD_A) * 0.5f) * w);
+    const int pl = crt_sky_f2i((c - CRT_SKY_GUARD_C) * h), ph = crt_sky_f2i((c + CRT_SKY_GUARD_C) * h);
+    r.index = (int)((uint32_t)pl * (uint32_t)texW + (uint32_t)(tl + 2));
+    r.decided = (tl == th) & (pl == ph);
+    return r;
+}
+
+#endif
```
